# osmocom/osmo-trx

Measured on AMD Instinct MI355X. Metric: Mbursts/s detect+demod (156.25 sym, 4 SPS), higher is better.
Workload: dtype f32

## Files before the change

osmo_trx_amd/csrc/trx_kernel_nb.hip:

```cpp
#include "trx_k4_common.h"
#include "trx_nb_asm.inc"

#define NB_D_LEN    160
#define NB_CZ_LEN   (TRX_CZ_PAD + TRX_CORR_NARROW + TRX_CZ_PAD)
#define NB_SLICE    (K4_XS + NB_D_LEN + NB_CZ_LEN)
#define NB_COMP_ROWS (TRX_DELAY_FILTS + 1)
#define NB_TABLES_FLOATS (TRX_SINCV_LDS + 16 * WAVE + NB_COMP_ROWS * 36 + 16 + 8 * 8 + 5 * WAVE + 5 * WAVE + 2 * 8 * 16)
#define NB_TABLES_BYTES (NB_TABLES_FLOATS * 4)
#define NB_WPB 16
#define NB_POOL_RING 64
#define NB_POOL_UNSET (-1)
#define NB_POOL_END (-2)
#define NB_NO_BURST 0xffffffffu
#define NB_LDS_TAIL (16 + 4 * NB_POOL_RING)
#define NB_LDS_BYTES (NB_TABLES_BYTES + NB_WPB * NB_SLICE * 8 + NB_LDS_TAIL)
#define NB_MAX_TOA 32



typedef float v3f __attribute__((ext_vector_type(3)));
typedef int v4i __attribute__((ext_vector_type(4)));

template <typename T>
__device__ __forceinline__ unsigned lds_addr(const T *p)
{
	return (unsigned)(uintptr_t)(const __attribute__((address_space(3))) T *)p;
}

__global__ void __launch_bounds__(NB_WPB * WAVE)
nb_pull4_kernel(const uint32_t *__restrict__ iq, const trxhip_burst_params *__restrict__ params,
		trxhip_burst_result *__restrict__ results, float *__restrict__ soft, const trx_tables *__restrict__ tab,
		unsigned n_bursts, float thresh, float full_scale, unsigned *__restrict__ pool_ctr, unsigned *__restrict__ redo,
		float gk5, float gk6, float gk7, float gk8)
{
	static_assert(NB_TABLES_BYTES % 16 == 0 && (NB_SLICE * 8) % 16 == 0 && (K4_XS * 8) % 16 == 0 && (NB_D_LEN * 8) % 16 == 0, "16-byte LDS accesses");
	static_assert(NB_LDS_BYTES <= 160 * 1024, "LDS");
	static_assert(NB_ASM_GDEC_OFF == (TRX_SINCV_LDS + 16 * WAVE + NB_COMP_ROWS * 36) * 4, "tools/gen_nb_asm.py: LDS offset of the decimator taps");
	static_assert(NB_ASM_LSEQ_OFF == (NB_TABLES_FLOATS - 2 * 8 * 16) * 4, "tools/gen_nb_asm.py: LDS offset of the training-sequence taps");
	constexpr int NLD = 10;
	extern __shared__ __attribute__((aligned(16))) char smem[];
	const int lane0 = threadIdx.x & (WAVE - 1);
	const int wave = uni((int)(threadIdx.x >> 6));

	float *const sincv = reinterpret_cast<float *>(smem);
	float *const wa4f = sincv + TRX_SINCV_LDS;
	const float4 *const wa4 = reinterpret_cast<const float4 *>(wa4f);
	float *const comp = wa4f + 16 * WAVE;
	float *const gdec = comp + NB_COMP_ROWS * 36;
	float *const lhdr = gdec + 16;
	int *const pkcl = reinterpret_cast<int *>(lhdr + 8 * 8);
	int *const lcn = pkcl + 5 * WAVE;
	c32 *const lseq = reinterpret_cast<c32 *>(lcn + 5 * WAVE);
	c32 *const wbase = reinterpret_cast<c32 *>(smem + NB_TABLES_BYTES) + (size_t)wave * NB_SLICE;
	int *const wg_next = reinterpret_cast<int *>(reinterpret_cast<c32 *>(smem + NB_TABLES_BYTES) + (size_t)NB_WPB * NB_SLICE);
	int *const pool_g = wg_next + 4;
	c32 *const P = wbase;
	c32 *const D = wbase + K4_XS;
	c32 *const cz = D + NB_D_LEN + TRX_CZ_PAD;

	for (int i = threadIdx.x; i < TRX_SINCV_LDS; i += blockDim.x)
		sincv[i] = (i < TRX_SINCV_LEN) ? tab->sincv[i] : 0.0f;
	for (int i = threadIdx.x; i < 16 * WAVE; i += blockDim.x) {
		const int l = i & (WAVE - 1), u = i >> 6;
		const PeakConst pcl = peak_const(l);
		const int q = (u < 8) ? pcl.loA + 512 * (7 - u) : pcl.hiA + 512 * (u - 8);
		wa4f[((u >> 2) * WAVE + l) * 4 + (u & 3)] = (q < TRX_SINCV_LEN) ? tab->sincv[q] : 0.0f;
	}
	for (int i = threadIdx.x; i < NB_COMP_ROWS * 36; i += blockDim.x) {
		const int f = i / 36, j = i % 36;
		comp[i] = (j >= TRX_FUSED_SH) ? tab->comp_filt[f][j - TRX_FUSED_SH] : 0.0f;
	}
	if (threadIdx.x < 16)
		gdec[threadIdx.x] = tab->dec_taps[threadIdx.x];
	if (threadIdx.x < 128)
		lseq[threadIdx.x] = make_float2(tab->seq[TRX_SEQ_TSC0 + (threadIdx.x >> 4)].taps[threadIdx.x & 15].re,
						tab->seq[TRX_SEQ_TSC0 + (threadIdx.x >> 4)].taps[threadIdx.x & 15].im);
	if (threadIdx.x < 64)
		lhdr[threadIdx.x] = reinterpret_cast<const float *>(&tab->seq[TRX_SEQ_TSC0 + (threadIdx.x >> 3)].gain)[threadIdx.x & 7];
	if (threadIdx.x < WAVE) {
		const PeakConst pc0 = peak_const(threadIdx.x);
		pkcl[0 * WAVE + threadIdx.x] = pc0.flA;
		pkcl[1 * WAVE + threadIdx.x] = pc0.loA;
		pkcl[2 * WAVE + threadIdx.x] = pc0.hiA;
		pkcl[3 * WAVE + threadIdx.x] = pc0.offB;
		pkcl[4 * WAVE + threadIdx.x] = pc0.ratio_off;
		lcn[0 * WAVE + threadIdx.x] = pc0.ratio_off * 8;
		lcn[1 * WAVE + threadIdx.x] = (pc0.flA - 8) * 8;
		lcn[2 * WAVE + threadIdx.x] = pc0.offB;
		const int l = threadIdx.x, e = (-l) & 3;
		const bool sp = l >= 52 && l < 60;
		lcn[3 * WAVE + l] = 8 * (sp ? (l < 56 ? e : e - 2) : (l < 48 ? 4 + 3 * l : 148));
		lcn[4 * WAVE + l] = sp ? (e + (l >= 56 ? 4 : 0)) * K4_NTP * 4 : -1;
	}
	for (int i = lane0; i < NB_SLICE; i += WAVE)
		wbase[i] = make_float2(0.0f, 0.0f);
	if (threadIdx.x == 0) {
		wg_next[0] = NB_WPB;
		wg_next[1] = 0;
	}
	if (threadIdx.x < NB_POOL_RING)
		pool_g[threadIdx.x] = NB_POOL_UNSET;
	__syncthreads();

	const float fs_db = 6.02059991f * __log2f(full_scale);
	const float thr2 = thresh * thresh;
	const float gc0 = thr2 * 1.0001e-5f;
	int t5pk = 0;
	bool t5_ok = true;
	for (int t = 0; t < 8; t++) {
		const int v = (int)(lhdr[8 * t + 5] * 512.0f);
		t5_ok = t5_ok && v >= -8 && v <= 7 && (float)v == lhdr[8 * t + 5] * 512.0f;
		t5pk |= (v & 15) << (4 * t);
	}
	t5pk = uni(t5pk);
	const unsigned long long e8_addr = reinterpret_cast<unsigned long long>(&tab->edge8[0][0][0]);
	const unsigned n_wg = gridDim.x;
	const unsigned n_groups = (n_bursts + 15u) >> 4;
	const bool pooled = pool_ctr != nullptr;
	const unsigned n_static_groups = pooled ? ((n_groups - (n_groups >> 3)) / n_wg) * n_wg : n_groups;
	const unsigned n_pool_groups = n_groups - n_static_groups;
	const unsigned gq = n_static_groups / n_wg, gr = n_static_groups % n_wg;
	const unsigned my_groups = gq + (blockIdx.x < gr ? 1u : 0u);
	const unsigned base16 = (blockIdx.x * gq + (blockIdx.x < gr ? blockIdx.x : gr)) << 4;
	unsigned items = my_groups << 4;
	if (base16 + items > n_bursts)
		items = (base16 < n_bursts) ? n_bursts - base16 : 0u;
	auto burst_of = [&](unsigned jj) -> unsigned {
		if (jj < items)
			return base16 + jj;
		if (!pooled)
			return NB_NO_BURST;
		const unsigned k = (jj - items) >> 4;
		volatile int *slot = pool_g + (k & (NB_POOL_RING - 1));
		int g;
		while ((g = *slot) == NB_POOL_UNSET)
			__builtin_amdgcn_s_sleep(2);
		g = uni(g);
		if (g < 0)
			return NB_NO_BURST;
		const unsigned bb = ((n_static_groups + (unsigned)g) << 4) + (jj & 15u);
		return bb < n_bursts ? bb : NB_NO_BURST;
	};
	auto pool_draw = [&](unsigned jj, bool ended, int lane) {
		const unsigned k = (jj + 16u - items) >> 4;
		int g = NB_POOL_END;
		if (!ended) {
			unsigned p = 0;
			if (lane == 0)
				p = __hip_atomic_fetch_add(pool_ctr, 1u, __ATOMIC_RELAXED, __HIP_MEMORY_SCOPE_AGENT);
			p = (unsigned)uni((int)p);
			g = (p < n_pool_groups) ? (int)p : NB_POOL_END;
		}
		if (lane == 0) {
			pool_g[(k + NB_POOL_RING / 2) & (NB_POOL_RING - 1)] = NB_POOL_UNSET;
			pool_g[k & (NB_POOL_RING - 1)] = g;
		}
	};

	uint32_t pre_i[NLD];
	uint32_t pre_prm = 0u;
	auto prefetch = [&](unsigned bb, int lane) {
		pre_prm = reinterpret_cast<const uint32_t *>(params)[2 * (size_t)bb];
		const uint32_t *src = iq + (size_t)bb * 625;
		const unsigned ul = (unsigned)lane & 63u;
#pragma unroll
		for (int r = 0; r < NLD - 1; r++)
			pre_i[r] = __builtin_nontemporal_load(src + (unsigned)(r * WAVE) + ul);
		pre_i[NLD - 1] = __builtin_nontemporal_load(src + (unsigned)((NLD - 1) * WAVE) + min(ul, 48u));
	};
	const unsigned b_first = burst_of((unsigned)wave);
	if (b_first != NB_NO_BURST)
		prefetch(b_first, lane0);

	v3f o = { 0.0f, 0.0f, 0.0f };
	int recw = 0;
	bool pend_any = false;
	bool pend_rec = false;
	unsigned pend_b = 0;
	bool left_any = false;
	int q_xr = 0, q_xi = 0, q_es = 0, q_toa = 0, q_s = 0, q_fl = 0, q_b = 0;
	int q_n = 0;
	auto flush_records = [&](const int lane) {
		if (lane < q_n) {
			const float *const h = lhdr + 8 * (q_fl & 0xff);
			const float xr = __int_as_float(q_xr), xi = __int_as_float(q_xi);
			const float a0 = xr * h[2], a1 = xr * h[3], a2 = xi * h[3], a3 = xi * h[2];
			const float amp_re = a0 - a2, amp_im = a1 + a3;
			const float toa = (float)q_toa * 0.001953125f;
			const float energy = __int_as_float(q_es) * 0.0125f;
			const float rssi = fs_db - 3.01029996f * __log2f(energy);
			const float p2 = xi * xi + xr * xr;
			const float C = p2 * h[7];
			const float S = __int_as_float(q_s);
			const float ci = 3.0103f * __log2f(C * __builtin_amdgcn_rcpf(S - C));
			const v4i r0 = { 1, __float_as_int(toa), __float_as_int(amp_re), __float_as_int(amp_im) };
			const v4i r1 = { __float_as_int(ci), __float_as_int(energy), __float_as_int(rssi), q_fl };
			asm volatile("global_store_dwordx4 %0, %1, off\n\t"
				     "global_store_dwordx4 %0, %2, off offset:16\n\t"
				     "s_nop 1"
				     :: "v"(results + (unsigned)q_b), "v"(r0), "v"(r1) : "memory");
		}
		q_n = 0;
	};

	auto demod_general = [&](const int nk, const c32 ampv, const int lane) -> bool {
		constexpr int L = 625, nwrite = 148;
		c32 *const dec = D;
		const trx_tables *tabc = tab;
		asm volatile("" : "+s"(tabc));
		const int w = nk >> 7, fr = nk & 127;
		const int fidx = (fr >= 2) ? (fr >> 1) : TRX_DELAY_FILTS;
		const float ian = __builtin_amdgcn_rcpf(norm2(ampv));
		const c32 scale = make_float2(ampv.x * ian, -ampv.y * ian);
		const int n_lo = w > 0 ? w : 0;
		const int n_hi = (L - 1 + w < 623) ? L - 1 + w : 623;
		const int i_full_lo = cdiv4(n_lo + 15), i_full_hi = fdiv4(n_hi);
		const int i0l = cdiv4(n_lo), i0h = i_full_hi + 1;
		const bool need_lo = (n_hi >= n_lo) && (i0l < i_full_lo) && (i0l < nwrite);
		const bool need_hi = (n_hi >= n_lo) && (i0h <= fdiv4(n_hi + 15)) && (i0h < nwrite);
		const bool lo_tab = need_lo && (n_hi >= 4 * (i_full_lo - 1));
		float ct0 = 0.0f, ct1 = 0.0f, ct2 = 0.0f;
		const int le = lane >> 4, lt = lane & 15;
		const int li = i0l + le;
		const int lt0 = n_lo + 15 - 4 * li;
		const bool lact = lt0 >= 1;
		if (lo_tab) {
			const float *row = &tabc->edge_lo[fidx][(lact ? lt0 : 1) - 1][lt];
			ct0 = row[0];
			ct1 = row[16];
			ct2 = (lt < 4) ? row[32] : 0.0f;
		}
		const bool hi_tab = need_hi && (w <= -2) && (n_lo <= 4 * i0h - 15);
		if ((need_lo && !lo_tab) || (need_hi && !hi_tab))
			return false;
		float ch0 = 0.0f, ch1 = 0.0f, ch2 = 0.0f;
		const int hi_i = i0h + le;
		const int htm = n_hi + 15 - 4 * hi_i;
		const bool hact = htm >= 0;
		if (hi_tab) {
			const float *row = &tabc->edge_hi[fidx][hact ? htm : 0][lt];
			ch0 = row[0];
			ch1 = row[16];
			ch2 = (lt < 4) ? row[32] : 0.0f;
		}
		{
			const int c_full = -24 - w;
			const int i_min = cdiv4(-36 - c_full), i_max = fdiv4(L + 1 - c_full);
			int ic = 3 * lane;
			if (ic < i_min) ic = i_min;
			if (ic > i_max - 2) ic = i_max - 2;
			v2f acc[3];
			asm volatile(NB_ASM_FIRG
				     : [a0] "=&v"(acc[0]), [a1] "=&v"(acc[1]), [a2] "=&v"(acc[2])
				     : [nk] "s"(nk), [pb] "s"(lds_addr(P)), [cb] "s"(lds_addr(comp) + 4u * (K4_U0 + TRX_FUSED_SH)), [kic] "v"(8 * ic)
				     : NB_ASM_CLOBBERS);
			if (n_lo == 0 && lo_tab && i_full_hi >= nwrite - 1) {
				if (lane < 52) {
#pragma unroll
					for (int j = 0; j < 3; j++)
						dec[3 * lane + j] = cmul(make_float2(acc[j].x, acc[j].y), scale);
				}
			} else {
#pragma unroll
				for (int j = 0; j < 3; j++) {
					const int i = 3 * lane + j;
					const bool full = (i >= i_full_lo) && (i <= i_full_hi);
					const c32 d = full ? cmul(make_float2(acc[j].x, acc[j].y), scale) : make_float2(0.0f, 0.0f);
					if (i < 156)
						dec[i] = d;
				}
			}
		}
		if (lo_tab) {
			const int s0 = 4 * li - 24 - w + lt;
			const c32 *pp = P + ((s0 & 3) * PH_A + PH_M0 + (s0 >> 2));
			const c32 x0 = lds_c32(pp), x1 = lds_c32(pp + 4), x2 = lds_c32(pp + 8);
			float ar = x0.x * ct0, ai = x0.y * ct0;
			ar = fmaf(x1.x, ct1, ar); ai = fmaf(x1.y, ct1, ai);
			ar = fmaf(x2.x, ct2, ar); ai = fmaf(x2.y, ct2, ai);
			const float sr = row_sum(ar), si = row_sum(ai);
			if (lt == 0 && lact)
				dec[li] = cmul(make_float2(sr, si), scale);
		}
		if (hi_tab) {
			const int s0 = 4 * hi_i - 24 - w + lt;
			const c32 *pp = P + ((s0 & 3) * PH_A + PH_M0 + (s0 >> 2));
			const c32 x0 = lds_c32(pp), x1 = lds_c32(pp + 4), x2 = lds_c32(pp + 8);
			float ar = x0.x * ch0, ai = x0.y * ch0;
			ar = fmaf(x1.x, ch1, ar); ai = fmaf(x1.y, ch1, ai);
			ar = fmaf(x2.x, ch2, ar); ai = fmaf(x2.y, ch2, ai);
			const float sr = row_sum(ar), si = row_sum(ai);
			if (lt == 0 && hact && hi_i < 156)
				dec[hi_i] = cmul(make_float2(sr, si), scale);
		}
		wave_sync();
		auto pick = [&](int i) {
			const float d = reinterpret_cast<const float *>(dec + i)[i & 1];
			return __builtin_amdgcn_fmed3f(fmaf((i & 2) ? -0.5f : 0.5f, d, 0.5f), 0.0f, 1.0f);
		};
		const int i0 = (lane < 48) ? 4 + 3 * lane : ((-lane) & 3);
		o.x = pick(i0);
		o.y = pick(lane < 48 ? i0 + 1 : 0);
		o.z = pick(lane < 48 ? i0 + 2 : 0);
		wave_sync();
		return true;
	};

	DIAG_DECL;
	unsigned j_next = 0, b_next = NB_NO_BURST;
	for (unsigned b = b_first; b != NB_NO_BURST; b = b_next) {
		int lane;
		asm volatile("v_mbcnt_lo_u32_b32 %0, -1, 0\n\tv_mbcnt_hi_u32_b32 %0, -1, %0" : "=v"(lane));
		const int ticket = claim_issue(wg_next);
		const unsigned prm0 = (unsigned)uni((int)pre_prm);
		const unsigned max_toa = prm0 >> 16;
		const int tsc = (prm0 >> 8) & 0xff;
		bool leave = ((prm0 & 0xf8ffu) != (unsigned)TRXHIP_TSC) || (max_toa > NB_MAX_TOA) || !t5_ok;

		c32 *const pload = P + (lane & 3) * PH_A + PH_M0 + (lane >> 2);
		float amax = 0.0f, epart = 0.0f;
#ifdef TRX_DIAG
		DIAG_MARK(12);
		asm volatile("s_waitcnt vmcnt(0)" ::: "memory");
		DIAG_MARK(13);
#endif
		if (!leave) {
#pragma unroll
			for (int r = 0; r < NLD; r++) {
				const int i = r * WAVE + lane;
				if (r < NLD - 1 || i < 625) {
					const c32 v = make_float2((float)(int16_t)(pre_i[r] & 0xffffu), (float)(int16_t)(pre_i[r] >> 16));
					pload[16 * r] = v;
					asm("v_max3_f32 %0, %0, |%1|, |%2|" : "+v"(amax) : "v"(v.x), "v"(v.y));
					if (r < 5)
						epart = fmaf(v.x, v.x, fmaf(v.y, v.y, epart));
				}
			}
		} else {
#pragma unroll
			for (int r = 0; r < NLD; r++)
				asm volatile("" :: "v"(pre_i[r]));
		}
		DIAG_MARK(14);
		if (pend_any) {
			float *const so = soft + (size_t)pend_b * 148;
			int *const rp = reinterpret_cast<int *>(results + pend_b);
			const float oe = o.x;
			asm volatile("s_bfm_b64 exec, 48, 0\n\t"
				     "global_store_dwordx3 %0, %1, %2 offset:16\n\t"
				     "s_bfm_b64 exec, 4, 52\n\t"
				     "global_store_dword %3, %4, %2\n\t"
				     "s_mov_b64 exec, %8\n\t"
				     "global_store_dword %5, %6, %7\n\t"
				     "s_mov_b64 exec, -1\n\t"
				     "s_nop 0"
				     :: "v"(lane * 12), "v"(o), "s"(so), "v"(((-lane) & 3) * 4), "v"(oe), "v"(lane * 4), "v"(recw), "s"(rp),
				        "s"(pend_rec ? 0xffull : 0ull)
				     : "memory");
		}
		pend_any = false;
		DIAG_MARK(16);
		j_next = (unsigned)(leave ? claim_take(ticket) : claim_take_behind<5>(ticket));
		b_next = burst_of(j_next);
		if (pooled && (j_next & 15u) == 0u && j_next + 16u >= items)
			pool_draw(j_next, b_next == NB_NO_BURST && j_next >= items, lane);
		DIAG_MARK(17);
		if (b_next != NB_NO_BURST)
			prefetch(b_next, lane);
		DIAG_MARK(15);

		int clip = 0;
		if (!leave) {
			clip = __ballot(amax > TRX_CLIP_THRESH) != 0ull;

			const int len = 16 + (int)max_toa;
			__builtin_assume(len >= 16 && len <= 16 + NB_MAX_TOA);
			const unsigned vd_addr = lds_addr(D) + 8u * (unsigned)lane, vcz_addr = lds_addr(cz) + 8u * (unsigned)lane;
			unsigned long long bad;
			asm volatile(NB_ASM_DEC
				     : [bad] "=s"(bad)
				     : [pd] "v"(lds_addr(P + PH_M0 + 52) + 8u * (unsigned)lane), [vd] "v"(vd_addr), [zero] "v"(0), [nact] "s"(15 + len)
				     : NB_ASM_CLOBBERS);
			DIAG_MARK(2);
			{
				float v;
				asm volatile(NB_ASM_CORR
					     : [nrm] "=&v"(v)
					     : [vd] "v"(vd_addr), [vcz] "v"(vcz_addr), [len] "s"(len), [tsc] "s"(tsc), [bad] "s"(bad)
					     : NB_ASM_CLOBBERS);
				DIAG_MARK(3);
				int m_bits, es_bits, bidx;
				int kr, ka, kb, kic, ktp;
				asm volatile(NB_ASM_AMAX("ds_read_b32 %[kr], %[l4] offset:%c[lc]", "ds_read_b32 %[ka], %[l4] offset:%c[lc]+256",
							 "ds_read_b32 %[kb], %[l4] offset:%c[lc]+512", "ds_read_b32 %[kic], %[l4] offset:%c[lc]+768",
							 "ds_read_b32 %[ktp], %[l4] offset:%c[lc]+1024", "s_nop 0", "s_nop 0", "s_nop 0")
					     "s_waitcnt lgkmcnt(0)"
					     : [m] "=s"(m_bits), [es] "=s"(es_bits), [bidx] "=s"(bidx), [kr] "=&v"(kr), [ka] "=&v"(ka), [kb] "=&v"(kb),
					       [kic] "=&v"(kic), [ktp] "=&v"(ktp)
					     : [nrm] "v"(v), [ep] "v"(epart), [l4] "v"(4 * lane),
					       [lc] "n"((TRX_SINCV_LDS + 16 * WAVE + NB_COMP_ROWS * 36 + 16 + 64 + 5 * WAVE) * 4)
					     : NB_ASM_CLOBBERS);
				DIAG_MARK(4);
				int hit = 0;
				int toa512 = 0;
				if (m_bits != 0) {
					int st, e512;
					float km;
					asm volatile(NB_ASM_DETA
						     : [st] "=&s"(st), [e] "=&s"(e512), [km] "=&v"(km)
						     : [bidx] "s"(bidx), [len] "s"(len), [czb] "s"(lds_addr(cz)), [kr] "v"(kr), [ka] "v"(ka), [l16] "v"(16 * lane),
						       [k5] "s"(gk5), [k6] "s"(gk6), [k7] "s"(gk7), [k8] "s"(gk8), [c0] "v"(gc0)
						     : NB_ASM_CLOBBERS);
					DIAG_MARK(5);
					int xr_bits = 0, xi_bits = 0;
					if (st == 1) {
						asm volatile(NB_ASM_DETB
							     : [st] "=&s"(st), [toa] "=&s"(toa512), [xr] "=&s"(xr_bits), [xi] "=&s"(xi_bits)
							     : [e] "s"(e512), [kb] "v"(kb), [czb] "s"(lds_addr(cz)), [km] "v"(km)
							     : NB_ASM_CLOBBERS);
						DIAG_MARK(6);
					}
					if (st == 3) {
						if (lane == 0)
							atomicAdd(&g_trx_fast_stats[0], 1ull);
						PeakConst pkc;
						pkc.flA = pkcl[0 * WAVE + lane]; pkc.loA = pkcl[1 * WAVE + lane]; pkc.hiA = pkcl[2 * WAVE + lane];
						pkc.offB = pkcl[3 * WAVE + lane]; pkc.ratio_off = pkcl[4 * WAVE + lane];
						c32 xcorr;
						peak_detect_spec(cz, bidx, sincv, pkc, lane, &toa512, &xcorr, wa4);
						toa512 = uni(toa512);
						xr_bits = uni(__float_as_int(xcorr.x));
						xi_bits = uni(__float_as_int(xcorr.y));
						st = 1;
					}
					if (st == 2) {
						leave = true;
						if (lane == 0) atomicAdd(&g_trx_fast_stats[2], 1ull);
					}
					if (st == 1) {
						hit = 1;
						int ok, s_bits;
						float d0, d1, d2;
						const int t5 = (t5pk << (28 - 4 * tsc)) >> 28;
						asm volatile("s_setprio 0");
						asm volatile(NB_ASM_TAIL
							     : [ok] "=&s"(ok), [ssum] "=&s"(s_bits), [d0] "=&v"(d0), [d1] "=&v"(d1), [d2] "=&v"(d2)
							     : [toa] "s"(toa512), [xr] "s"(xr_bits), [xi] "s"(xi_bits), [t5] "s"(t5), [hdrb] "s"(lds_addr(lhdr) + 32u * (unsigned)tsc),
							       [e8lo] "s"((unsigned)e8_addr), [e8hi] "s"((unsigned)(e8_addr >> 32)), [l16] "v"(16 * lane),
							       [vd] "v"(vd_addr), [pb] "s"(lds_addr(P)), [cb] "s"(lds_addr(comp) + 4u * (K4_U0 + TRX_FUSED_SH)), [db] "s"(lds_addr(D)),
							       [kic] "v"(kic), [ktp] "v"(ktp)
							     : NB_ASM_CLOBBERS);
						DIAG_MARK(10);
						asm volatile("s_setprio 2");
						if (!ok) {
							if (lane == 0) atomicAdd(&g_trx_fast_stats[3], 1ull);
							const float *const h = lhdr + 8 * tsc;
							const float xr = __int_as_float(xr_bits), xi = __int_as_float(xi_bits);
							const float a0 = xr * h[2], a1 = xr * h[3], a2 = xi * h[3], a3 = xi * h[2];
							const c32 ampv = make_float2(unif(a0 - a2), unif(a1 + a3));
							if (!demod_general(t5 + 10 * 512 - toa512, ampv, lane))
								leave = true;
						}
						if (!leave) {
							asm("s_lshl_b64 exec, 1, %[n]\n\t"
						    "v_mov_b32_e32 %[qxr], %[xr]\n\t"
						    "v_mov_b32_e32 %[qxi], %[xi]\n\t"
						    "v_mov_b32_e32 %[qes], %[es]\n\t"
						    "v_mov_b32_e32 %[qtoa], %[toa]\n\t"
						    "v_mov_b32_e32 %[qs], %[ss]\n\t"
						    "v_mov_b32_e32 %[qfl], %[fl]\n\t"
						    "v_mov_b32_e32 %[qb], %[b]\n\t"
						    "s_mov_b64 exec, -1"
						    : [qxr] "+v"(q_xr), [qxi] "+v"(q_xi), [qes] "+v"(q_es), [qtoa] "+v"(q_toa), [qs] "+v"(q_s), [qfl] "+v"(q_fl),
						      [qb] "+v"(q_b)
						    : [n] "s"(uni(q_n)), [xr] "s"(xr_bits), [xi] "s"(xi_bits), [es] "s"(es_bits), [toa] "s"(toa512 - t5 - 10 * 512),
						      [ss] "s"(s_bits), [fl] "s"((int)((uint32_t)tsc | ((uint32_t)clip << 8) | (37u << 24))), [b] "s"((int)b));
						q_n++;
						}
						if (ok) {
							o.x = __builtin_amdgcn_fmed3f(fmaf(0.5f, d0, 0.5f), 0.0f, 1.0f);
							o.y = __builtin_amdgcn_fmed3f(fmaf(0.5f, d1, 0.5f), 0.0f, 1.0f);
							o.z = __builtin_amdgcn_fmed3f(fmaf(0.5f, d2, 0.5f), 0.0f, 1.0f);
						}
					}
				}
				if (!hit && !leave) {
					const float energy = __int_as_float(es_bits) * 0.0125f;
					const float rssi = fs_db - 3.01029996f * __log2f(energy);
					const uint32_t flags = ((uint32_t)clip << 8) | (1u << 16);
					int word = clip ? -TRXHIP_SIGERR_CLIP : 0;
					word = put_lane<1>(word, 0.0f);
					word = put_lane<2>(word, 0.0f);
					word = put_lane<3>(word, 0.0f);
					word = put_lane<4>(word, 0.0f);
					word = put_lane<5>(word, energy);
					word = put_lane<6>(word, rssi);
					word = write_lane<7>(word, (int)flags);
					recw = word;
					o = (v3f){ 0.0f, 0.0f, 0.0f };
				}
				pend_rec = !hit;
			}
		}
		if (leave) {
			if (lane == 0) {
				reinterpret_cast<uint8_t *>(redo + TRX_REDO_HDR)[b] = 1;
				if (!left_any)
					__hip_atomic_store(redo, 1u, __ATOMIC_RELAXED, __HIP_MEMORY_SCOPE_AGENT);
			}
			left_any = true;
			continue;
		}
		pend_b = b;
		pend_any = true;
		if (q_n == WAVE)
			flush_records(lane);
		DIAG_MARK(11);
	}
	if (pend_any) {
		int lane;
		asm volatile("v_mbcnt_lo_u32_b32 %0, -1, 0\n\tv_mbcnt_hi_u32_b32 %0, -1, %0" : "=v"(lane));
		float *const so = soft + (size_t)pend_b * 148;
		int *const rp = reinterpret_cast<int *>(results + pend_b);
		const float oe = o.x;
		asm volatile("s_bfm_b64 exec, 48, 0\n\t"
			     "global_store_dwordx3 %0, %1, %2 offset:16\n\t"
			     "s_bfm_b64 exec, 4, 52\n\t"
			     "global_store_dword %3, %4, %2\n\t"
			     "s_mov_b64 exec, %8\n\t"
			     "global_store_dword %5, %6, %7\n\t"
			     "s_mov_b64 exec, -1\n\t"
			     "s_nop 0"
			     :: "v"(lane * 12), "v"(o), "s"(so), "v"(((-lane) & 3) * 4), "v"(oe), "v"(lane * 4), "v"(recw), "s"(rp),
			        "s"(pend_rec ? 0xffull : 0ull)
			     : "memory");
	}
	{
		int lane;
		asm volatile("v_mbcnt_lo_u32_b32 %0, -1, 0\n\tv_mbcnt_hi_u32_b32 %0, -1, %0" : "=v"(lane));
		flush_records(lane);
	}
	DIAG_FLUSH();
	if (pooled) {
		__syncthreads();
		int tid0;
		asm volatile("v_mbcnt_lo_u32_b32 %0, -1, 0\n\tv_mbcnt_hi_u32_b32 %0, -1, %0" : "=v"(tid0));
		if (tid0 == 0 && atomicAdd(wg_next + 1, 1) == 0) {
			const unsigned d = __hip_atomic_fetch_add(pool_ctr + 1, 1u, __ATOMIC_ACQ_REL, __HIP_MEMORY_SCOPE_AGENT);
			if (d == gridDim.x - 1u) {
				__hip_atomic_store(pool_ctr, 0u, __ATOMIC_RELAXED, __HIP_MEMORY_SCOPE_AGENT);
				__hip_atomic_store(pool_ctr + 1, 0u, __ATOMIC_RELEASE, __HIP_MEMORY_SCOPE_AGENT);
			}
		}
	}
}
```

osmo_trx_amd/csrc/trx_nb_asm.inc:

```
#define NB_ASM_GDEC_OFF 29968
#define NB_ASM_LSEQ_OFF 32848
#define NB_ASM_CLOBBERS "v64", "v65", "v66", "v67", "v68", "v69", "v70", "v71", "v72", "v73", "v74", "v75", "v76", "v77", "v78", "v79", "v80", "v81", "v82", "v83", "v84", "v85", "v86", "v87", "v88", "v89", "v90", "v91", "v92", "v93", "v94", "v95", "v96", "v97", "v98", "v99", "v100", "v101", "v102", "v103", "v104", "v105", "v106", "v107", "v108", "v109", "v110", "v111", "v112", "v113", "v114", "v115", "v116", "v117", "v118", "v119", "v120", "v121", "v122", "v123", "v124", "v125", "v126", "v127", "s87", "s88", "s89", "s90", "s91", "s92", "s93", "s94", "s95", "s96", "s97", "s98", "s99", "vcc", "scc", "memory"
#define NB_ASM_DEC \
	"s_bfm_b64 exec, %[nact], 0\n\t" \
	"ds_read_b128 v[120:123], %[zero] offset:29968\n\t" \
	"ds_read_b128 v[124:127], %[zero] offset:29984\n\t" \
	"ds_read_b64 v[88:89], %[pd] offset:1440\n\t" \
	"ds_read_b64 v[90:91], %[pd] offset:2880\n\t" \
	"ds_read_b64 v[92:93], %[pd] offset:4320\n\t" \
	"ds_read_b64 v[94:95], %[pd] offset:8\n\t" \
	"ds_read_b64 v[96:97], %[pd] offset:1448\n\t" \
	"ds_read_b64 v[98:99], %[pd] offset:2888\n\t" \
	"ds_read_b64 v[100:101], %[pd] offset:4328\n\t" \
	"ds_read_b64 v[102:103], %[pd] offset:16\n\t" \
	"ds_read_b64 v[104:105], %[pd] offset:1456\n\t" \
	"ds_read_b64 v[106:107], %[pd] offset:2896\n\t" \
	"ds_read_b64 v[108:109], %[pd] offset:4336\n\t" \
	"ds_read_b64 v[110:111], %[pd] offset:24\n\t" \
	"ds_read_b64 v[112:113], %[pd] offset:1464\n\t" \
	"ds_read_b64 v[114:115], %[pd] offset:2904\n\t" \
	"ds_read_b64 v[116:117], %[pd] offset:4344\n\t" \
	"ds_read_b64 v[118:119], %[pd] offset:32\n\t" \
	"s_waitcnt lgkmcnt(12)\n\t" \
	"v_pk_mul_f32 v[88:89], v[88:89], v[120:121] op_sel:[0,0] op_sel_hi:[1,0]\n\t" \
	"v_pk_mul_f32 v[90:91], v[90:91], v[120:121] op_sel:[0,1] op_sel_hi:[1,1]\n\t" \
	"v_pk_mul_f32 v[92:93], v[92:93], v[122:123] op_sel:[0,0] op_sel_hi:[1,0]\n\t" \
	"v_pk_add_f32 v[88:89], v[88:89], v[90:91]\n\t" \
	"v_pk_mul_f32 v[94:95], v[94:95], v[122:123] op_sel:[0,1] op_sel_hi:[1,1]\n\t" \
	"v_pk_add_f32 v[88:89], v[88:89], v[92:93]\n\t" \
	"s_waitcnt lgkmcnt(8)\n\t" \
	"v_pk_mul_f32 v[96:97], v[96:97], v[124:125] op_sel:[0,0] op_sel_hi:[1,0]\n\t" \
	"v_pk_add_f32 v[88:89], v[88:89], v[94:95]\n\t" \
	"v_pk_mul_f32 v[98:99], v[98:99], v[124:125] op_sel:[0,1] op_sel_hi:[1,1]\n\t" \
	"v_pk_add_f32 v[88:89], v[88:89], v[96:97]\n\t" \
	"v_pk_mul_f32 v[100:101], v[100:101], v[126:127] op_sel:[0,0] op_sel_hi:[1,0]\n\t" \
	"v_pk_add_f32 v[88:89], v[88:89], v[98:99]\n\t" \
	"v_pk_mul_f32 v[102:103], v[102:103], v[126:127] op_sel:[0,1] op_sel_hi:[1,1]\n\t" \
	"v_pk_add_f32 v[88:89], v[88:89], v[100:101]\n\t" \
	"s_waitcnt lgkmcnt(4)\n\t" \
	"v_pk_mul_f32 v[104:105], v[104:105], v[126:127] op_sel:[0,1] op_sel_hi:[1,1]\n\t" \
	"v_pk_add_f32 v[88:89], v[88:89], v[102:103]\n\t" \
	"v_pk_mul_f32 v[106:107], v[106:107], v[126:127] op_sel:[0,0] op_sel_hi:[1,0]\n\t" \
	"v_pk_add_f32 v[88:89], v[88:89], v[104:105]\n\t" \
	"v_pk_mul_f32 v[108:109], v[108:109], v[124:125] op_sel:[0,1] op_sel_hi:[1,1]\n\t" \
	"v_pk_add_f32 v[88:89], v[88:89], v[106:107]\n\t" \
	"v_pk_mul_f32 v[110:111], v[110:111], v[124:125] op_sel:[0,0] op_sel_hi:[1,0]\n\t" \
	"v_pk_add_f32 v[88:89], v[88:89], v[108:109]\n\t" \
	"s_waitcnt lgkmcnt(0)\n\t" \
	"v_pk_mul_f32 v[112:113], v[112:113], v[122:123] op_sel:[0,1] op_sel_hi:[1,1]\n\t" \
	"v_pk_add_f32 v[88:89], v[88:89], v[110:111]\n\t" \
	"v_pk_mul_f32 v[114:115], v[114:115], v[122:123] op_sel:[0,0] op_sel_hi:[1,0]\n\t" \
	"v_pk_add_f32 v[88:89], v[88:89], v[112:113]\n\t" \
	"v_pk_mul_f32 v[116:117], v[116:117], v[120:121] op_sel:[0,1] op_sel_hi:[1,1]\n\t" \
	"v_pk_add_f32 v[88:89], v[88:89], v[114:115]\n\t" \
	"v_pk_mul_f32 v[118:119], v[118:119], v[120:121] op_sel:[0,0] op_sel_hi:[1,0]\n\t" \
	"v_pk_add_f32 v[88:89], v[88:89], v[116:117]\n\t" \
	"s_nop 0\n\t" \
	"v_pk_add_f32 v[88:89], v[88:89], v[118:119]\n\t" \
	"ds_write_b64 %[vd], v[88:89]\n\t" \
	"v_min_f32_e64 v90, |v88|, |v89|\n\t" \
	"v_max_f32_e64 v91, |v88|, |v89|\n\t" \
	"v_ldexp_f32 v90, v90, 17\n\t" \
	"v_cmp_lt_f32_e32 vcc, v90, v91\n\t" \
	"s_mov_b64 exec, -1\n\t" \
	"s_mov_b64 %[bad], vcc\n\t" \
	"s_waitcnt lgkmcnt(0)\n\t"
#define NB_ASM_CORR \
	"v_mov_b64_e32 v[120:121], 0\n\t" \
	"s_bfm_b64 exec, %[len], 0\n\t" \
	"ds_read_b64 v[88:89], %[vd] offset:0\n\t" \
	"ds_read_b64 v[90:91], %[vd] offset:8\n\t" \
	"ds_read_b64 v[92:93], %[vd] offset:16\n\t" \
	"ds_read_b64 v[94:95], %[vd] offset:24\n\t" \
	"ds_read_b64 v[96:97], %[vd] offset:32\n\t" \
	"ds_read_b64 v[98:99], %[vd] offset:40\n\t" \
	"ds_read_b64 v[100:101], %[vd] offset:48\n\t" \
	"ds_read_b64 v[102:103], %[vd] offset:56\n\t" \
	"ds_read_b64 v[104:105], %[vd] offset:64\n\t" \
	"ds_read_b64 v[106:107], %[vd] offset:72\n\t" \
	"ds_read_b64 v[108:109], %[vd] offset:80\n\t" \
	"ds_read_b64 v[110:111], %[vd] offset:88\n\t" \
	"ds_read_b64 v[112:113], %[vd] offset:96\n\t" \
	"ds_read_b64 v[114:115], %[vd] offset:104\n\t" \
	"ds_read_b64 v[116:117], %[vd] offset:112\n\t" \
	"ds_read_b64 v[118:119], %[vd] offset:120\n\t" \
	"s_cmp_lg_u64 %[bad], 0\n\t" \
	"s_cbranch_scc1 .Lnb_corr_mul\n\t" \
	"s_getpc_b64 s[88:89]\n\t" \
	".Lnb_corr_pc:\n\t" \
	"s_mul_i32 s90, %[tsc], .Lnb_corr_v1-.Lnb_corr_v0\n\t" \
	"s_add_u32 s88, s88, s90\n\t" \
	"s_addc_u32 s89, s89, 0\n\t" \
	"s_add_u32 s88, s88, .Lnb_corr_v0-.Lnb_corr_pc\n\t" \
	"s_addc_u32 s89, s89, 0\n\t" \
	"s_setpc_b64 s[88:89]\n\t" \
	".Lnb_corr_v0:\n\t" \
	"s_waitcnt lgkmcnt(15)\n\t" \
	"v_pk_add_f32 v[120:121], v[120:121], v[88:89] neg_lo:[0,1] neg_hi:[0,1]\n\t" \
	"s_waitcnt lgkmcnt(14)\n\t" \
	"v_pk_add_f32 v[120:121], v[120:121], v[90:91] op_sel:[0,1] op_sel_hi:[1,0] neg_lo:[0,0] neg_hi:[0,1]\n\t" \
	"s_waitcnt lgkmcnt(13)\n\t" \
	"v_pk_add_f32 v[120:121], v[120:121], v[92:93]\n\t" \
	"s_waitcnt lgkmcnt(12)\n\t" \
	"v_pk_add_f32 v[120:121], v[120:121], v[94:95] op_sel:[0,1] op_sel_hi:[1,0] neg_lo:[0,0] neg_hi:[0,1]\n\t" \
	"s_waitcnt lgkmcnt(11)\n\t" \
	"v_pk_add_f32 v[120:121], v[120:121], v[96:97] neg_lo:[0,1] neg_hi:[0,1]\n\t" \
	"s_waitcnt lgkmcnt(10)\n\t" \
	"v_pk_add_f32 v[120:121], v[120:121], v[98:99] op_sel:[0,1] op_sel_hi:[1,0] neg_lo:[0,0] neg_hi:[0,1]\n\t" \
	"s_waitcnt lgkmcnt(9)\n\t" \
	"v_pk_add_f32 v[120:121], v[120:121], v[100:101] neg_lo:[0,1] neg_hi:[0,1]\n\t" \
	"s_waitcnt lgkmcnt(8)\n\t" \
	"v_pk_add_f32 v[120:121], v[120:121], v[102:103] op_sel:[0,1] op_sel_hi:[1,0] neg_lo:[0,1] neg_hi:[0,0]\n\t" \
	"s_waitcnt lgkmcnt(7)\n\t" \
	"v_pk_add_f32 v[120:121], v[120:121], v[104:105]\n\t" \
	"s_waitcnt lgkmcnt(6)\n\t" \
	"v_pk_add_f32 v[120:121], v[120:121], v[106:107] op_sel:[0,1] op_sel_hi:[1,0] neg_lo:[0,1] neg_hi:[0,0]\n\t" \
	"s_waitcnt lgkmcnt(5)\n\t" \
	"v_pk_add_f32 v[120:121], v[120:121], v[108:109] neg_lo:[0,1] neg_hi:[0,1]\n\t" \
	"s_waitcnt lgkmcnt(4)\n\t" \
	"v_pk_add_f32 v[120:121], v[120:121], v[110:111] op_sel:[0,1] op_sel_hi:[1,0] neg_lo:[0,1] neg_hi:[0,0]\n\t" \
	"s_waitcnt lgkmcnt(3)\n\t" \
	"v_pk_add_f32 v[120:121], v[120:121], v[112:113]\n\t" \
	"s_waitcnt lgkmcnt(2)\n\t" \
	"v_pk_add_f32 v[120:121], v[120:121], v[114:115] op_sel:[0,1] op_sel_hi:[1,0] neg_lo:[0,1] neg_hi:[0,0]\n\t" \
	"s_waitcnt lgkmcnt(1)\n\t" \
	"v_pk_add_f32 v[120:121], v[120:121], v[116:117] neg_lo:[0,1] neg_hi:[0,1]\n\t" \
	"s_waitcnt lgkmcnt(0)\n\t" \
	"v_pk_add_f32 v[120:121], v[120:121], v[118:119] op_sel:[0,1] op_sel_hi:[1,0] neg_lo:[0,1] neg_hi:[0,0]\n\t" \
	"s_branch .Lnb_corr_join\n\t" \
	".Lnb_corr_v1:\n\t" \
	"s_waitcnt lgkmcnt(15)\n\t" \
	"v_pk_add_f32 v[120:121], v[120:121], v[88:89] neg_lo:[0,1] neg_hi:[0,1]\n\t" \
	"s_waitcnt lgkmcnt(14)\n\t" \
	"v_pk_add_f32 v[120:121], v[120:121], v[90:91] op_sel:[0,1] op_sel_hi:[1,0] neg_lo:[0,0] neg_hi:[0,1]\n\t" \
	"s_waitcnt lgkmcnt(13)\n\t" \
	"v_pk_add_f32 v[120:121], v[120:121], v[92:93]\n\t" \
	"s_waitcnt lgkmcnt(12)\n\t" \
	"v_pk_add_f32 v[120:121], v[120:121], v[94:95] op_sel:[0,1] op_sel_hi:[1,0] neg_lo:[0,0] neg_hi:[0,1]\n\t" \
	"s_waitcnt lgkmcnt(11)\n\t" \
	"v_pk_add_f32 v[120:121], v[120:121], v[96:97] neg_lo:[0,1] neg_hi:[0,1]\n\t" \
	"s_waitcnt lgkmcnt(10)\n\t" \
	"v_pk_add_f32 v[120:121], v[120:121], v[98:99] op_sel:[0,1] op_sel_hi:[1,0] neg_lo:[0,0] neg_hi:[0,1]\n\t" \
	"s_waitcnt lgkmcnt(9)\n\t" \
	"v_pk_add_f32 v[120:121], v[120:121], v[100:101]\n\t" \
	"s_waitcnt lgkmcnt(8)\n\t" \
	"v_pk_add_f32 v[120:121], v[120:121], v[102:103] op_sel:[0,1] op_sel_hi:[1,0] neg_lo:[0,0] neg_hi:[0,1]\n\t" \
	"s_waitcnt lgkmcnt(7)\n\t" \
	"v_pk_add_f32 v[120:121], v[120:121], v[104:105] neg_lo:[0,1] neg_hi:[0,1]\n\t" \
	"s_waitcnt lgkmcnt(6)\n\t" \
	"v_pk_add_f32 v[120:121], v[120:121], v[106:107] op_sel:[0,1] op_sel_hi:[1,0] neg_lo:[0,1] neg_hi:[0,0]\n\t" \
	"s_waitcnt lgkmcnt(5)\n\t" \
	"v_pk_add_f32 v[120:121], v[120:121], v[108:109] neg_lo:[0,1] neg_hi:[0,1]\n\t" \
	"s_waitcnt lgkmcnt(4)\n\t" \
	"v_pk_add_f32 v[120:121], v[120:121], v[110:111] op_sel:[0,1] op_sel_hi:[1,0] neg_lo:[0,1] neg_hi:[0,0]\n\t" \
	"s_waitcnt lgkmcnt(3)\n\t" \
	"v_pk_add_f32 v[120:121], v[120:121], v[112:113]\n\t" \
	"s_waitcnt lgkmcnt(2)\n\t" \
	"v_pk_add_f32 v[120:121], v[120:121], v[114:115] op_sel:[0,1] op_sel_hi:[1,0] neg_lo:[0,1] neg_hi:[0,0]\n\t" \
	"s_waitcnt lgkmcnt(1)\n\t" \
	"v_pk_add_f32 v[120:121], v[120:121], v[116:117] neg_lo:[0,1] neg_hi:[0,1]\n\t" \
	"s_waitcnt lgkmcnt(0)\n\t" \
	"v_pk_add_f32 v[120:121], v[120:121], v[118:119] op_sel:[0,1] op_sel_hi:[1,0] neg_lo:[0,0] neg_hi:[0,1]\n\t" \
	"s_branch .Lnb_corr_join\n\t" \
	".Lnb_corr_v2:\n\t" \
	"s_waitcnt lgkmcnt(15)\n\t" \
	"v_pk_add_f32 v[120:121], v[120:121], v[88:89]\n\t" \
	"s_waitcnt lgkmcnt(14)\n\t" \
	"v_pk_add_f32 v[120:121], v[120:121], v[90:91] op_sel:[0,1] op_sel_hi:[1,0] neg_lo:[0,1] neg_hi:[0,0]\n\t" \
	"s_waitcnt lgkmcnt(13)\n\t" \
	"v_pk_add_f32 v[120:121], v[120:121], v[92:93]\n\t" \
	"s_waitcnt lgkmcnt(12)\n\t" \
	"v_pk_add_f32 v[120:121], v[120:121], v[94:95] op_sel:[0,1] op_sel_hi:[1,0] neg_lo:[0,0] neg_hi:[0,1]\n\t" \
	"s_waitcnt lgkmcnt(11)\n\t" \
	"v_pk_add_f32 v[120:121], v[120:121], v[96:97]\n\t" \
	"s_waitcnt lgkmcnt(10)\n\t" \
	"v_pk_add_f32 v[120:121], v[120:121], v[98:99] op_sel:[0,1] op_sel_hi:[1,0] neg_lo:[0,1] neg_hi:[0,0]\n\t" \
	"s_waitcnt lgkmcnt(9)\n\t" \
	"v_pk_add_f32 v[120:121], v[120:121], v[100:101]\n\t" \
	"s_waitcnt lgkmcnt(8)\n\t" \
	"v_pk_add_f32 v[120:121], v[120:121], v[102:103] op_sel:[0,1] op_sel_hi:[1,0] neg_lo:[0,0] neg_hi:[0,1]\n\t" \
	"s_waitcnt lgkmcnt(7)\n\t" \
	"v_pk_add_f32 v[120:121], v[120:121], v[104:105]\n\t" \
	"s_waitcnt lgkmcnt(6)\n\t" \
	"v_pk_add_f32 v[120:121], v[120:121], v[106:107] op_sel:[0,1] op_sel_hi:[1,0] neg_lo:[0,1] neg_hi:[0,0]\n\t" \
	"s_waitcnt lgkmcnt(5)\n\t" \
	"v_pk_add_f32 v[120:121], v[120:121], v[108:109] neg_lo:[0,1] neg_hi:[0,1]\n\t" \
	"s_waitcnt lgkmcnt(4)\n\t" \
	"v_pk_add_f32 v[120:121], v[120:121], v[110:111] op_sel:[0,1] op_sel_hi:[1,0] neg_lo:[0,1] neg_hi:[0,0]\n\t" \
	"s_waitcnt lgkmcnt(3)\n\t" \
	"v_pk_add_f32 v[120:121], v[120:121], v[112:113] neg_lo:[0,1] neg_hi:[0,1]\n\t" \
	"s_waitcnt lgkmcnt(2)\n\t" \
	"v_pk_add_f32 v[120:121], v[120:121], v[114:115] op_sel:[0,1] op_sel_hi:[1,0] neg_lo:[0,0] neg_hi:[0,1]\n\t" \
	"s_waitcnt lgkmcnt(1)\n\t" \
	"v_pk_add_f32 v[120:121], v[120:121], v[116:117] neg_lo:[0,1] neg_hi:[0,1]\n\t" \
	"s_waitcnt lgkmcnt(0)\n\t" \
	"v_pk_add_f32 v[120:121], v[120:121], v[118:119] op_sel:[0,1] op_sel_hi:[1,0] neg_lo:[0,1] neg_hi:[0,0]\n\t" \
	"s_branch .Lnb_corr_join\n\t" \
	".Lnb_corr_v3:\n\t" \
	"s_waitcnt lgkmcnt(15)\n\t" \
	"v_pk_add_f32 v[120:121], v[120:121], v[88:89] neg_lo:[0,1] neg_hi:[0,1]\n\t" \
	"s_waitcnt lgkmcnt(14)\n\t" \
	"v_pk_add_f32 v[120:121], v[120:121], v[90:91] op_sel:[0,1] op_sel_hi:[1,0] neg_lo:[0,1] neg_hi:[0,0]\n\t" \
	"s_waitcnt lgkmcnt(13)\n\t" \
	"v_pk_add_f32 v[120:121], v[120:121], v[92:93]\n\t" \
	"s_waitcnt lgkmcnt(12)\n\t" \
	"v_pk_add_f32 v[120:121], v[120:121], v[94:95] op_sel:[0,1] op_sel_hi:[1,0] neg_lo:[0,0] neg_hi:[0,1]\n\t" \
	"s_waitcnt lgkmcnt(11)\n\t" \
	"v_pk_add_f32 v[120:121], v[120:121], v[96:97]\n\t" \
	"s_waitcnt lgkmcnt(10)\n\t" \
	"v_pk_add_f32 v[120:121], v[120:121], v[98:99] op_sel:[0,1] op_sel_hi:[1,0] neg_lo:[0,1] neg_hi:[0,0]\n\t" \
	"s_waitcnt lgkmcnt(9)\n\t" \
	"v_pk_add_f32 v[120:121], v[120:121], v[100:101]\n\t" \
	"s_waitcnt lgkmcnt(8)\n\t" \
	"v_pk_add_f32 v[120:121], v[120:121], v[102:103] op_sel:[0,1] op_sel_hi:[1,0] neg_lo:[0,1] neg_hi:[0,0]\n\t" \
	"s_waitcnt lgkmcnt(7)\n\t" \
	"v_pk_add_f32 v[120:121], v[120:121], v[104:105] neg_lo:[0,1] neg_hi:[0,1]\n\t" \
	"s_waitcnt lgkmcnt(6)\n\t" \
	"v_pk_add_f32 v[120:121], v[120:121], v[106:107] op_sel:[0,1] op_sel_hi:[1,0] neg_lo:[0,0] neg_hi:[0,1]\n\t" \
	"s_waitcnt lgkmcnt(5)\n\t" \
	"v_pk_add_f32 v[120:121], v[120:121], v[108:109] neg_lo:[0,1] neg_hi:[0,1]\n\t" \
	"s_waitcnt lgkmcnt(4)\n\t" \
	"v_pk_add_f32 v[120:121], v[120:121], v[110:111] op_sel:[0,1] op_sel_hi:[1,0] neg_lo:[0,1] neg_hi:[0,0]\n\t" \
	"s_waitcnt lgkmcnt(3)\n\t" \
	"v_pk_add_f32 v[120:121], v[120:121], v[112:113] neg_lo:[0,1] neg_hi:[0,1]\n\t" \
	"s_waitcnt lgkmcnt(2)\n\t" \
	"v_pk_add_f32 v[120:121], v[120:121], v[114:115] op_sel:[0,1] op_sel_hi:[1,0] neg_lo:[0,0] neg_hi:[0,1]\n\t" \
	"s_waitcnt lgkmcnt(1)\n\t" \
	"v_pk_add_f32 v[120:121], v[120:121], v[116:117] neg_lo:[0,1] neg_hi:[0,1]\n\t" \
	"s_waitcnt lgkmcnt(0)\n\t" \
	"v_pk_add_f32 v[120:121], v[120:121], v[118:119] op_sel:[0,1] op_sel_hi:[1,0] neg_lo:[0,1] neg_hi:[0,0]\n\t" \
	"s_branch .Lnb_corr_join\n\t" \
	".Lnb_corr_v4:\n\t" \
	"s_waitcnt lgkmcnt(15)\n\t" \
	"v_pk_add_f32 v[120:121], v[120:121], v[88:89]\n\t" \
	"s_waitcnt lgkmcnt(14)\n\t" \
	"v_pk_add_f32 v[120:121], v[120:121], v[90:91] op_sel:[0,1] op_sel_hi:[1,0] neg_lo:[0,1] neg_hi:[0,0]\n\t" \
	"s_waitcnt lgkmcnt(13)\n\t" \
	"v_pk_add_f32 v[120:121], v[120:121], v[92:93] neg_lo:[0,1] neg_hi:[0,1]\n\t" \
	"s_waitcnt lgkmcnt(12)\n\t" \
	"v_pk_add_f32 v[120:121], v[120:121], v[94:95] op_sel:[0,1] op_sel_hi:[1,0] neg_lo:[0,0] neg_hi:[0,1]\n\t" \
	"s_waitcnt lgkmcnt(11)\n\t" \
	"v_pk_add_f32 v[120:121], v[120:121], v[96:97] neg_lo:[0,1] neg_hi:[0,1]\n\t" \
	"s_waitcnt lgkmcnt(10)\n\t" \
	"v_pk_add_f32 v[120:121], v[120:121], v[98:99] op_sel:[0,1] op_sel_hi:[1,0] neg_lo:[0,1] neg_hi:[0,0]\n\t" \
	"s_waitcnt lgkmcnt(9)\n\t" \
	"v_pk_add_f32 v[120:121], v[120:121], v[100:101] neg_lo:[0,1] neg_hi:[0,1]\n\t" \
	"s_waitcnt lgkmcnt(8)\n\t" \
	"v_pk_add_f32 v[120:121], v[120:121], v[102:103] op_sel:[0,1] op_sel_hi:[1,0] neg_lo:[0,1] neg_hi:[0,0]\n\t" \
	"s_waitcnt lgkmcnt(7)\n\t" \
	"v_pk_add_f32 v[120:121], v[120:121], v[104:105] neg_lo:[0,1] neg_hi:[0,1]\n\t" \
	"s_waitcnt lgkmcnt(6)\n\t" \
	"v_pk_add_f32 v[120:121], v[120:121], v[106:107] op_sel:[0,1] op_sel_hi:[1,0] neg_lo:[0,0] neg_hi:[0,1]\n\t" \
	"s_waitcnt lgkmcnt(5)\n\t" \
	"v_pk_add_f32 v[120:121], v[120:121], v[108:109] neg_lo:[0,1] neg_hi:[0,1]\n\t" \
	"s_waitcnt lgkmcnt(4)\n\t" \
	"v_pk_add_f32 v[120:121], v[120:121], v[110:111] op_sel:[0,1] op_sel_hi:[1,0] neg_lo:[0,1] neg_hi:[0,0]\n\t" \
	"s_waitcnt lgkmcnt(3)\n\t" \
	"v_pk_add_f32 v[120:121], v[120:121], v[112:113]\n\t" \
	"s_waitcnt lgkmcnt(2)\n\t" \
	"v_pk_add_f32 v[120:121], v[120:121], v[114:115] op_sel:[0,1] op_sel_hi:[1,0] neg_lo:[0,0] neg_hi:[0,1]\n\t" \
	"s_waitcnt lgkmcnt(1)\n\t" \
	"v_pk_add_f32 v[120:121], v[120:121], v[116:117]\n\t" \
	"s_waitcnt lgkmcnt(0)\n\t" \
	"v_pk_add_f32 v[120:121], v[120:121], v[118:119] op_sel:[0,1] op_sel_hi:[1,0] neg_lo:[0,0] neg_hi:[0,1]\n\t" \
	"s_branch .Lnb_corr_join\n\t" \
	".Lnb_corr_v5:\n\t" \
	"s_waitcnt lgkmcnt(15)\n\t" \
	"v_pk_add_f32 v[120:121], v[120:121], v[88:89] neg_lo:[0,1] neg_hi:[0,1]\n\t" \
	"s_waitcnt lgkmcnt(14)\n\t" \
	"v_pk_add_f32 v[120:121], v[120:121], v[90:91] op_sel:[0,1] op_sel_hi:[1,0] neg_lo:[0,1] neg_hi:[0,0]\n\t" \
	"s_waitcnt lgkmcnt(13)\n\t" \
	"v_pk_add_f32 v[120:121], v[120:121], v[92:93] neg_lo:[0,1] neg_hi:[0,1]\n\t" \
	"s_waitcnt lgkmcnt(12)\n\t" \
	"v_pk_add_f32 v[120:121], v[120:121], v[94:95] op_sel:[0,1] op_sel_hi:[1,0] neg_lo:[0,0] neg_hi:[0,1]\n\t" \
	"s_waitcnt lgkmcnt(11)\n\t" \
	"v_pk_add_f32 v[120:121], v[120:121], v[96:97]\n\t" \
	"s_waitcnt lgkmcnt(10)\n\t" \
	"v_pk_add_f32 v[120:121], v[120:121], v[98:99] op_sel:[0,1] op_sel_hi:[1,0] neg_lo:[0,1] neg_hi:[0,0]\n\t" \
	"s_waitcnt lgkmcnt(9)\n\t" \
	"v_pk_add_f32 v[120:121], v[120:121], v[100:101]\n\t" \
	"s_waitcnt lgkmcnt(8)\n\t" \
	"v_pk_add_f32 v[120:121], v[120:121], v[102:103] op_sel:[0,1] op_sel_hi:[1,0] neg_lo:[0,1] neg_hi:[0,0]\n\t" \
	"s_waitcnt lgkmcnt(7)\n\t" \
	"v_pk_add_f32 v[120:121], v[120:121], v[104:105]\n\t" \
	"s_waitcnt lgkmcnt(6)\n\t" \
	"v_pk_add_f32 v[120:121], v[120:121], v[106:107] op_sel:[0,1] op_sel_hi:[1,0] neg_lo:[0,0] neg_hi:[0,1]\n\t" \
	"s_waitcnt lgkmcnt(5)\n\t" \
	"v_pk_add_f32 v[120:121], v[120:121], v[108:109] neg_lo:[0,1] neg_hi:[0,1]\n\t" \
	"s_waitcnt lgkmcnt(4)\n\t" \
	"v_pk_add_f32 v[120:121], v[120:121], v[110:111] op_sel:[0,1] op_sel_hi:[1,0] neg_lo:[0,1] neg_hi:[0,0]\n\t" \
	"s_waitcnt lgkmcnt(3)\n\t" \
	"v_pk_add_f32 v[120:121], v[120:121], v[112:113] neg_lo:[0,1] neg_hi:[0,1]\n\t" \
	"s_waitcnt lgkmcnt(2)\n\t" \
	"v_pk_add_f32 v[120:121], v[120:121], v[114:115] op_sel:[0,1] op_sel_hi:[1,0] neg_lo:[0,0] neg_hi:[0,1]\n\t" \
	"s_waitcnt lgkmcnt(1)\n\t" \
	"v_pk_add_f32 v[120:121], v[120:121], v[116:117] neg_lo:[0,1] neg_hi:[0,1]\n\t" \
	"s_waitcnt lgkmcnt(0)\n\t" \
	"v_pk_add_f32 v[120:121], v[120:121], v[118:119] op_sel:[0,1] op_sel_hi:[1,0] neg_lo:[0,0] neg_hi:[0,1]\n\t" \
	"s_branch .Lnb_corr_join\n\t" \
	".Lnb_corr_v6:\n\t" \
	"s_waitcnt lgkmcnt(15)\n\t" \
	"v_pk_add_f32 v[120:121], v[120:121], v[88:89] neg_lo:[0,1] neg_hi:[0,1]\n\t" \
	"s_waitcnt lgkmcnt(14)\n\t" \
	"v_pk_add_f32 v[120:121], v[120:121], v[90:91] op_sel:[0,1] op_sel_hi:[1,0] neg_lo:[0,1] neg_hi:[0,0]\n\t" \
	"s_waitcnt lgkmcnt(13)\n\t" \
	"v_pk_add_f32 v[120:121], v[120:121], v[92:93]\n\t" \
	"s_waitcnt lgkmcnt(12)\n\t" \
	"v_pk_add_f32 v[120:121], v[120:121], v[94:95] op_sel:[0,1] op_sel_hi:[1,0] neg_lo:[0,0] neg_hi:[0,1]\n\t" \
	"s_waitcnt lgkmcnt(11)\n\t" \
	"v_pk_add_f32 v[120:121], v[120:121], v[96:97] neg_lo:[0,1] neg_hi:[0,1]\n\t" \
	"s_waitcnt lgkmcnt(10)\n\t" \
	"v_pk_add_f32 v[120:121], v[120:121], v[98:99] op_sel:[0,1] op_sel_hi:[1,0] neg_lo:[0,0] neg_hi:[0,1]\n\t" \
	"s_waitcnt lgkmcnt(9)\n\t" \
	"v_pk_add_f32 v[120:121], v[120:121], v[100:101]\n\t" \
	"s_waitcnt lgkmcnt(8)\n\t" \
	"v_pk_add_f32 v[120:121], v[120:121], v[102:103] op_sel:[0,1] op_sel_hi:[1,0] neg_lo:[0,0] neg_hi:[0,1]\n\t" \
	"s_waitcnt lgkmcnt(7)\n\t" \
	"v_pk_add_f32 v[120:121], v[120:121], v[104:105]\n\t" \
	"s_waitcnt lgkmcnt(6)\n\t" \
	"v_pk_add_f32 v[120:121], v[120:121], v[106:107] op_sel:[0,1] op_sel_hi:[1,0] neg_lo:[0,0] neg_hi:[0,1]\n\t" \
	"s_waitcnt lgkmcnt(5)\n\t" \
	"v_pk_add_f32 v[120:121], v[120:121], v[108:109] neg_lo:[0,1] neg_hi:[0,1]\n\t" \
	"s_waitcnt lgkmcnt(4)\n\t" \
	"v_pk_add_f32 v[120:121], v[120:121], v[110:111] op_sel:[0,1] op_sel_hi:[1,0] neg_lo:[0,0] neg_hi:[0,1]\n\t" \
	"s_waitcnt lgkmcnt(3)\n\t" \
	"v_pk_add_f32 v[120:121], v[120:121], v[112:113]\n\t" \
	"s_waitcnt lgkmcnt(2)\n\t" \
	"v_pk_add_f32 v[120:121], v[120:121], v[114:115] op_sel:[0,1] op_sel_hi:[1,0] neg_lo:[0,1] neg_hi:[0,0]\n\t" \
	"s_waitcnt lgkmcnt(1)\n\t" \
	"v_pk_add_f32 v[120:121], v[120:121], v[116:117] neg_lo:[0,1] neg_hi:[0,1]\n\t" \
	"s_waitcnt lgkmcnt(0)\n\t" \
	"v_pk_add_f32 v[120:121], v[120:121], v[118:119] op_sel:[0,1] op_sel_hi:[1,0] neg_lo:[0,1] neg_hi:[0,0]\n\t" \
	"s_branch .Lnb_corr_join\n\t" \
	".Lnb_corr_v7:\n\t" \
	"s_waitcnt lgkmcnt(15)\n\t" \
	"v_pk_add_f32 v[120:121], v[120:121], v[88:89] neg_lo:[0,1] neg_hi:[0,1]\n\t" \
	"s_waitcnt lgkmcnt(14)\n\t" \
	"v_pk_add_f32 v[120:121], v[120:121], v[90:91] op_sel:[0,1] op_sel_hi:[1,0] neg_lo:[0,1] neg_hi:[0,0]\n\t" \
	"s_waitcnt lgkmcnt(13)\n\t" \
	"v_pk_add_f32 v[120:121], v[120:121], v[92:93]\n\t" \
	"s_waitcnt lgkmcnt(12)\n\t" \
	"v_pk_add_f32 v[120:121], v[120:121], v[94:95] op_sel:[0,1] op_sel_hi:[1,0] neg_lo:[0,1] neg_hi:[0,0]\n\t" \
	"s_waitcnt lgkmcnt(11)\n\t" \
	"v_pk_add_f32 v[120:121], v[120:121], v[96:97]\n\t" \
	"s_waitcnt lgkmcnt(10)\n\t" \
	"v_pk_add_f32 v[120:121], v[120:121], v[98:99] op_sel:[0,1] op_sel_hi:[1,0] neg_lo:[0,0] neg_hi:[0,1]\n\t" \
	"s_waitcnt lgkmcnt(9)\n\t" \
	"v_pk_add_f32 v[120:121], v[120:121], v[100:101]\n\t" \
	"s_waitcnt lgkmcnt(8)\n\t" \
	"v_pk_add_f32 v[120:121], v[120:121], v[102:103] op_sel:[0,1] op_sel_hi:[1,0] neg_lo:[0,1] neg_hi:[0,0]\n\t" \
	"s_waitcnt lgkmcnt(7)\n\t" \
	"v_pk_add_f32 v[120:121], v[120:121], v[104:105]\n\t" \
	"s_waitcnt lgkmcnt(6)\n\t" \
	"v_pk_add_f32 v[120:121], v[120:121], v[106:107] op_sel:[0,1] op_sel_hi:[1,0] neg_lo:[0,1] neg_hi:[0,0]\n\t" \
	"s_waitcnt lgkmcnt(5)\n\t" \
	"v_pk_add_f32 v[120:121], v[120:121], v[108:109] neg_lo:[0,1] neg_hi:[0,1]\n\t" \
	"s_waitcnt lgkmcnt(4)\n\t" \
	"v_pk_add_f32 v[120:121], v[120:121], v[110:111] op_sel:[0,1] op_sel_hi:[1,0] neg_lo:[0,0] neg_hi:[0,1]\n\t" \
	"s_waitcnt lgkmcnt(3)\n\t" \
	"v_pk_add_f32 v[120:121], v[120:121], v[112:113] neg_lo:[0,1] neg_hi:[0,1]\n\t" \
	"s_waitcnt lgkmcnt(2)\n\t" \
	"v_pk_add_f32 v[120:121], v[120:121], v[114:115] op_sel:[0,1] op_sel_hi:[1,0] neg_lo:[0,1] neg_hi:[0,0]\n\t" \
	"s_waitcnt lgkmcnt(1)\n\t" \
	"v_pk_add_f32 v[120:121], v[120:121], v[116:117] neg_lo:[0,1] neg_hi:[0,1]\n\t" \
	"s_waitcnt lgkmcnt(0)\n\t" \
	"v_pk_add_f32 v[120:121], v[120:121], v[118:119] op_sel:[0,1] op_sel_hi:[1,0] neg_lo:[0,0] neg_hi:[0,1]\n\t" \
	"s_branch .Lnb_corr_join\n\t" \
	".Lnb_corr_join:\n\t" \
	"s_add_u32 s90, %[len], 12\n\t" \
	"s_bfm_b64 exec, s90, 0\n\t" \
	"ds_write_b64 %[vcz], v[120:121]\n\t" \
	"s_mov_b64 exec, -1\n\t" \
	"v_pk_mul_f32 v[122:123], v[120:121], v[120:121]\n\t" \
	"s_waitcnt lgkmcnt(0)\n\t" \
	"v_add_f32_e32 %[nrm], v123, v122\n\t" \
	"s_branch .Lnb_corr_end\n\t" \
	".Lnb_corr_mul:\n\t" \
	"s_lshl_b32 s90, %[tsc], 7\n\t" \
	"v_mov_b32_e32 v64, s90\n\t" \
	"ds_read_b128 v[66:69], v64 offset:32848\n\t" \
	"ds_read_b128 v[70:73], v64 offset:32864\n\t" \
	"ds_read_b128 v[74:77], v64 offset:32880\n\t" \
	"ds_read_b128 v[78:81], v64 offset:32896\n\t" \
	"s_waitcnt lgkmcnt(0)\n\t" \
	"v_pk_mul_f32 v[82:83], v[88:89], v[66:67] op_sel:[0,0] op_sel_hi:[0,1]\n\t" \
	"v_pk_mul_f32 v[84:85], v[88:89], v[66:67] op_sel:[1,1] op_sel_hi:[1,0]\n\t" \
	"s_nop 0\n\t" \
	"v_pk_add_f32 v[86:87], v[82:83], v[84:85] neg_lo:[0,1] neg_hi:[0,0]\n\t" \
	"s_nop 0\n\t" \
	"v_pk_add_f32 v[120:121], v[120:121], v[86:87]\n\t" \
	"v_pk_mul_f32 v[82:83], v[90:91], v[68:69] op_sel:[0,0] op_sel_hi:[0,1]\n\t" \
	"v_pk_mul_f32 v[84:85], v[90:91], v[68:69] op_sel:[1,1] op_sel_hi:[1,0]\n\t" \
	"s_nop 0\n\t" \
	"v_pk_add_f32 v[86:87], v[82:83], v[84:85] neg_lo:[0,1] neg_hi:[0,0]\n\t" \
	"s_nop 0\n\t" \
	"v_pk_add_f32 v[120:121], v[120:121], v[86:87]\n\t" \
	"v_pk_mul_f32 v[82:83], v[92:93], v[70:71] op_sel:[0,0] op_sel_hi:[0,1]\n\t" \
	"v_pk_mul_f32 v[84:85], v[92:93], v[70:71] op_sel:[1,1] op_sel_hi:[1,0]\n\t" \
	"s_nop 0\n\t" \
	"v_pk_add_f32 v[86:87], v[82:83], v[84:85] neg_lo:[0,1] neg_hi:[0,0]\n\t" \
	"s_nop 0\n\t" \
	"v_pk_add_f32 v[120:121], v[120:121], v[86:87]\n\t" \
	"v_pk_mul_f32 v[82:83], v[94:95], v[72:73] op_sel:[0,0] op_sel_hi:[0,1]\n\t" \
	"v_pk_mul_f32 v[84:85], v[94:95], v[72:73] op_sel:[1,1] op_sel_hi:[1,0]\n\t" \
	"s_nop 0\n\t" \
	"v_pk_add_f32 v[86:87], v[82:83], v[84:85] neg_lo:[0,1] neg_hi:[0,0]\n\t" \
	"s_nop 0\n\t" \
	"v_pk_add_f32 v[120:121], v[120:121], v[86:87]\n\t" \
	"v_pk_mul_f32 v[82:83], v[96:97], v[74:75] op_sel:[0,0] op_sel_hi:[0,1]\n\t" \
	"v_pk_mul_f32 v[84:85], v[96:97], v[74:75] op_sel:[1,1] op_sel_hi:[1,0]\n\t" \
	"s_nop 0\n\t" \
	"v_pk_add_f32 v[86:87], v[82:83], v[84:85] neg_lo:[0,1] neg_hi:[0,0]\n\t" \
	"s_nop 0\n\t" \
	"v_pk_add_f32 v[120:121], v[120:121], v[86:87]\n\t" \
	"v_pk_mul_f32 v[82:83], v[98:99], v[76:77] op_sel:[0,0] op_sel_hi:[0,1]\n\t" \
	"v_pk_mul_f32 v[84:85], v[98:99], v[76:77] op_sel:[1,1] op_sel_hi:[1,0]\n\t" \
	"s_nop 0\n\t" \
	"v_pk_add_f32 v[86:87], v[82:83], v[84:85] neg_lo:[0,1] neg_hi:[0,0]\n\t" \
	"s_nop 0\n\t" \
	"v_pk_add_f32 v[120:121], v[120:121], v[86:87]\n\t" \
	"v_pk_mul_f32 v[82:83], v[100:101], v[78:79] op_sel:[0,0] op_sel_hi:[0,1]\n\t" \
	"v_pk_mul_f32 v[84:85], v[100:101], v[78:79] op_sel:[1,1] op_sel_hi:[1,0]\n\t" \
	"s_nop 0\n\t" \
	"v_pk_add_f32 v[86:87], v[82:83], v[84:85] neg_lo:[0,1] neg_hi:[0,0]\n\t" \
	"s_nop 0\n\t" \
	"v_pk_add_f32 v[120:121], v[120:121], v[86:87]\n\t" \
	"v_pk_mul_f32 v[82:83], v[102:103], v[80:81] op_sel:[0,0] op_sel_hi:[0,1]\n\t" \
	"v_pk_mul_f32 v[84:85], v[102:103], v[80:81] op_sel:[1,1] op_sel_hi:[1,0]\n\t" \
	"s_nop 0\n\t" \
	"v_pk_add_f32 v[86:87], v[82:83], v[84:85] neg_lo:[0,1] neg_hi:[0,0]\n\t" \
	"s_nop 0\n\t" \
	"v_pk_add_f32 v[120:121], v[120:121], v[86:87]\n\t" \
	"ds_read_b128 v[66:69], v64 offset:32912\n\t" \
	"ds_read_b128 v[70:73], v64 offset:32928\n\t" \
	"ds_read_b128 v[74:77], v64 offset:32944\n\t" \
	"ds_read_b128 v[78:81], v64 offset:32960\n\t" \
	"s_waitcnt lgkmcnt(0)\n\t" \
	"v_pk_mul_f32 v[82:83], v[104:105], v[66:67] op_sel:[0,0] op_sel_hi:[0,1]\n\t" \
	"v_pk_mul_f32 v[84:85], v[104:105], v[66:67] op_sel:[1,1] op_sel_hi:[1,0]\n\t" \
	"s_nop 0\n\t" \
	"v_pk_add_f32 v[86:87], v[82:83], v[84:85] neg_lo:[0,1] neg_hi:[0,0]\n\t" \
	"s_nop 0\n\t" \
	"v_pk_add_f32 v[120:121], v[120:121], v[86:87]\n\t" \
	"v_pk_mul_f32 v[82:83], v[106:107], v[68:69] op_sel:[0,0] op_sel_hi:[0,1]\n\t" \
	"v_pk_mul_f32 v[84:85], v[106:107], v[68:69] op_sel:[1,1] op_sel_hi:[1,0]\n\t" \
	"s_nop 0\n\t" \
	"v_pk_add_f32 v[86:87], v[82:83], v[84:85] neg_lo:[0,1] neg_hi:[0,0]\n\t" \
	"s_nop 0\n\t" \
	"v_pk_add_f32 v[120:121], v[120:121], v[86:87]\n\t" \
	"v_pk_mul_f32 v[82:83], v[108:109], v[70:71] op_sel:[0,0] op_sel_hi:[0,1]\n\t" \
	"v_pk_mul_f32 v[84:85], v[108:109], v[70:71] op_sel:[1,1] op_sel_hi:[1,0]\n\t" \
	"s_nop 0\n\t" \
	"v_pk_add_f32 v[86:87], v[82:83], v[84:85] neg_lo:[0,1] neg_hi:[0,0]\n\t" \
	"s_nop 0\n\t" \
	"v_pk_add_f32 v[120:121], v[120:121], v[86:87]\n\t" \
	"v_pk_mul_f32 v[82:83], v[110:111], v[72:73] op_sel:[0,0] op_sel_hi:[0,1]\n\t" \
	"v_pk_mul_f32 v[84:85], v[110:111], v[72:73] op_sel:[1,1] op_sel_hi:[1,0]\n\t" \
	"s_nop 0\n\t" \
	"v_pk_add_f32 v[86:87], v[82:83], v[84:85] neg_lo:[0,1] neg_hi:[0,0]\n\t" \
	"s_nop 0\n\t" \
	"v_pk_add_f32 v[120:121], v[120:121], v[86:87]\n\t" \
	"v_pk_mul_f32 v[82:83], v[112:113], v[74:75] op_sel:[0,0] op_sel_hi:[0,1]\n\t" \
	"v_pk_mul_f32 v[84:85], v[112:113], v[74:75] op_sel:[1,1] op_sel_hi:[1,0]\n\t" \
	"s_nop 0\n\t" \
	"v_pk_add_f32 v[86:87], v[82:83], v[84:85] neg_lo:[0,1] neg_hi:[0,0]\n\t" \
	"s_nop 0\n\t" \
	"v_pk_add_f32 v[120:121], v[120:121], v[86:87]\n\t" \
	"v_pk_mul_f32 v[82:83], v[114:115], v[76:77] op_sel:[0,0] op_sel_hi:[0,1]\n\t" \
	"v_pk_mul_f32 v[84:85], v[114:115], v[76:77] op_sel:[1,1] op_sel_hi:[1,0]\n\t" \
	"s_nop 0\n\t" \
	"v_pk_add_f32 v[86:87], v[82:83], v[84:85] neg_lo:[0,1] neg_hi:[0,0]\n\t" \
	"s_nop 0\n\t" \
	"v_pk_add_f32 v[120:121], v[120:121], v[86:87]\n\t" \
	"v_pk_mul_f32 v[82:83], v[116:117], v[78:79] op_sel:[0,0] op_sel_hi:[0,1]\n\t" \
	"v_pk_mul_f32 v[84:85], v[116:117], v[78:79] op_sel:[1,1] op_sel_hi:[1,0]\n\t" \
	"s_nop 0\n\t" \
	"v_pk_add_f32 v[86:87], v[82:83], v[84:85] neg_lo:[0,1] neg_hi:[0,0]\n\t" \
	"s_nop 0\n\t" \
	"v_pk_add_f32 v[120:121], v[120:121], v[86:87]\n\t" \
	"v_pk_mul_f32 v[82:83], v[118:119], v[80:81] op_sel:[0,0] op_sel_hi:[0,1]\n\t" \
	"v_pk_mul_f32 v[84:85], v[118:119], v[80:81] op_sel:[1,1] op_sel_hi:[1,0]\n\t" \
	"s_nop 0\n\t" \
	"v_pk_add_f32 v[86:87], v[82:83], v[84:85] neg_lo:[0,1] neg_hi:[0,0]\n\t" \
	"s_nop 0\n\t" \
	"v_pk_add_f32 v[120:121], v[120:121], v[86:87]\n\t" \
	"s_branch .Lnb_corr_join\n\t" \
	".Lnb_corr_end:\n\t"
#define NB_ASM_DETA \
	"s_mov_b32 %[st], 0\n\t" \
	"s_cmp_lt_i32 %[bidx], 3\n\t" \
	"s_cbranch_scc1 .Lnb_da_end\n\t" \
	"s_sub_u32 s88, %[len], 3\n\t" \
	"s_cmp_gt_i32 %[bidx], s88\n\t" \
	"s_cbranch_scc1 .Lnb_da_end\n\t" \
	"s_lshl3_add_u32 s89, %[bidx], %[czb]\n\t" \
	"s_add_u32 s90, %[len], -1\n\t" \
	"v_mov_b32_e32 v64, s89\n\t" \
	"v_add_u32_e32 v65, s89, %[kr]\n\t" \
	"s_lshl3_add_u32 s90, s90, %[czb]\n\t" \
	"v_add_u32_e32 v66, s89, %[ka]\n\t" \
	"ds_read_b64 v[68:69], v64\n\t" \
	"v_mov_b32_e32 v67, s90\n\t" \
	"v_mov_b64_e32 v[72:73], 0\n\t" \
	"s_bfm_b64 exec, 8, 0\n\t" \
	"ds_read_b64 v[70:71], v65\n\t" \
	"s_mov_b64 exec, 1\n\t" \
	"ds_write_b64 v67, v[72:73]\n\t" \
	"s_mov_b64 exec, -1\n\t" \
	"ds_read_b128 v[76:79], %[l16] offset:16512\n\t" \
	"ds_read_b128 v[80:83], %[l16] offset:17536\n\t" \
	"ds_read_b64 v[88:89], v66 offset:0\n\t" \
	"ds_read_b64 v[90:91], v66 offset:8\n\t" \
	"ds_read_b64 v[92:93], v66 offset:16\n\t" \
	"ds_read_b64 v[94:95], v66 offset:24\n\t" \
	"ds_read_b64 v[96:97], v66 offset:32\n\t" \
	"ds_read_b64 v[98:99], v66 offset:40\n\t" \
	"ds_read_b64 v[100:101], v66 offset:48\n\t" \
	"ds_read_b64 v[102:103], v66 offset:56\n\t" \
	"v_mov_b64_e32 v[84:85], 0\n\t" \
	"v_mov_b64_e32 v[86:87], 0\n\t" \
	"s_add_u32 s91, %[bidx], -1\n\t" \
	"s_sub_u32 s92, %[len], %[bidx]\n\t" \
	"s_min_u32 s91, s91, 4\n\t" \
	"s_waitcnt lgkmcnt(11)\n\t" \
	"v_pk_mul_f32 v[68:69], v[68:69], v[68:69]\n\t" \
	"s_add_u32 s92, s92, -2\n\t" \
	"v_add_f32_e32 v74, v69, v68\n\t" \
	"v_mul_f32_e32 %[km], 0x36c9539c, v74\n\t" \
	"s_bfm_b64 exec, 8, 0\n\t" \
	"v_pk_mul_f32 v[70:71], v[70:71], v[70:71]\n\t" \
	"s_min_u32 s92, s92, 4\n\t" \
	"v_add_f32_e32 v75, v71, v70\n\t" \
	"s_add_u32 s91, s91, s92\n\t" \
	"s_cmp_eq_u32 s91, 8\n\t" \
	"v_add_f32_dpp v75, v75, v75 quad_perm:[1,0,3,2] row_mask:0xf bank_mask:0xf\n\t" \
	"s_cselect_b32 s92, %[k8], %[k7]\n\t" \
	"s_cmp_eq_u32 s91, 6\n\t" \
	"v_add_f32_dpp v75, v75, v75 quad_perm:[2,3,0,1] row_mask:0xf bank_mask:0xf\n\t" \
	"s_cselect_b32 s93, %[k6], %[k5]\n\t" \
	"s_cmp_ge_u32 s91, 7\n\t" \
	"v_add_f32_dpp v75, v75, v75 row_half_mirror row_mask:0xf bank_mask:0xf\n\t" \
	"s_cselect_b32 s92, s92, s93\n\t" \
	"v_mul_f32_e32 v112, s92, v75\n\t" \
	"v_mul_f32_e32 v113, 0x3f7fff37, v112\n\t" \
	"v_fmamk_f32 v114, v112, 0x3f8000c9, %[c0]\n\t" \
	"v_cmp_lt_f32_e32 vcc, v74, v113\n\t" \
	"s_cbranch_vccnz .Lnb_da_wait_end\n\t" \
	"v_cmp_gt_f32_e32 vcc, v74, v114\n\t" \
	"s_mov_b32 %[st], 2\n\t" \
	"s_cbranch_vccz .Lnb_da_wait_end\n\t" \
	"s_mov_b64 exec, -1\n\t" \
	"ds_read_b128 v[104:107], %[l16] offset:18560\n\t" \
	"ds_read_b128 v[108:111], %[l16] offset:19584\n\t" \
	"ds_read_b64 v[112:113], v66 offset:64\n\t" \
	"ds_read_b64 v[114:115], v66 offset:72\n\t" \
	"ds_read_b64 v[116:117], v66 offset:80\n\t" \
	"ds_read_b64 v[118:119], v66 offset:88\n\t" \
	"ds_read_b64 v[120:121], v66 offset:96\n\t" \
	"ds_read_b64 v[122:123], v66 offset:104\n\t" \
	"ds_read_b64 v[124:125], v66 offset:112\n\t" \
	"ds_read_b64 v[126:127], v66 offset:120\n\t" \
	"s_waitcnt lgkmcnt(10)\n\t" \
	"v_pk_fma_f32 v[84:85], v[88:89], v[76:77], v[84:85] op_sel:[0,0,0] op_sel_hi:[1,0,1]\n\t" \
	"v_pk_fma_f32 v[86:87], v[90:91], v[76:77], v[86:87] op_sel:[0,1,0] op_sel_hi:[1,1,1]\n\t" \
	"v_pk_fma_f32 v[84:85], v[92:93], v[78:79], v[84:85] op_sel:[0,0,0] op_sel_hi:[1,0,1]\n\t" \
	"v_pk_fma_f32 v[86:87], v[94:95], v[78:79], v[86:87] op_sel:[0,1,0] op_sel_hi:[1,1,1]\n\t" \
	"v_pk_fma_f32 v[84:85], v[96:97], v[80:81], v[84:85] op_sel:[0,0,0] op_sel_hi:[1,0,1]\n\t" \
	"v_pk_fma_f32 v[86:87], v[98:99], v[80:81], v[86:87] op_sel:[0,1,0] op_sel_hi:[1,1,1]\n\t" \
	"v_pk_fma_f32 v[84:85], v[100:101], v[82:83], v[84:85] op_sel:[0,0,0] op_sel_hi:[1,0,1]\n\t" \
	"v_pk_fma_f32 v[86:87], v[102:103], v[82:83], v[86:87] op_sel:[0,1,0] op_sel_hi:[1,1,1]\n\t" \
	"s_waitcnt lgkmcnt(0)\n\t" \
	"v_pk_fma_f32 v[84:85], v[112:113], v[104:105], v[84:85] op_sel:[0,0,0] op_sel_hi:[1,0,1]\n\t" \
	"v_pk_fma_f32 v[86:87], v[114:115], v[104:105], v[86:87] op_sel:[0,1,0] op_sel_hi:[1,1,1]\n\t" \
	"v_pk_fma_f32 v[84:85], v[116:117], v[106:107], v[84:85] op_sel:[0,0,0] op_sel_hi:[1,0,1]\n\t" \
	"v_pk_fma_f32 v[86:87], v[118:119], v[106:107], v[86:87] op_sel:[0,1,0] op_sel_hi:[1,1,1]\n\t" \
	"v_pk_fma_f32 v[84:85], v[120:121], v[108:109], v[84:85] op_sel:[0,0,0] op_sel_hi:[1,0,1]\n\t" \
	"v_pk_fma_f32 v[86:87], v[122:123], v[108:109], v[86:87] op_sel:[0,1,0] op_sel_hi:[1,1,1]\n\t" \
	"v_pk_fma_f32 v[84:85], v[124:125], v[110:111], v[84:85] op_sel:[0,0,0] op_sel_hi:[1,0,1]\n\t" \
	"v_pk_fma_f32 v[86:87], v[126:127], v[110:111], v[86:87] op_sel:[0,1,0] op_sel_hi:[1,1,1]\n\t" \
	"s_nop 0\n\t" \
	"v_pk_add_f32 v[84:85], v[84:85], v[86:87]\n\t" \
	"s_nop 0\n\t" \
	"v_pk_mul_f32 v[84:85], v[84:85], v[84:85]\n\t" \
	"s_nop 0\n\t" \
	"v_add_f32_e32 v88, v85, v84\n\t" \
	"v_fmamk_f32 v89, v88, 0x36c9539c, %[km]\n\t" \
	"v_sub_f32_e32 v90, v88, v89\n\t" \
	"v_add_f32_e32 v91, v88, v89\n\t" \
	"s_lshl_b32 s94, %[bidx], 9\n\t" \
	"v_mov_b32_dpp v90, v90 quad_perm:[1,0,3,2] row_mask:0xf bank_mask:0xf\n\t" \
	"v_cmp_lt_f32_e64 s[88:89], v91, v90\n\t" \
	"s_mov_b32 %[st], 1\n\t" \
	"s_lshr_b64 s[90:91], s[88:89], 1\n\t" \
	"s_or_b64 s[90:91], s[90:91], s[88:89]\n\t" \
	"s_mov_b32 s96, 0x55555555\n\t" \
	"s_mov_b32 s97, 0x15555555\n\t" \
	"s_and_b64 s[92:93], s[90:91], s[96:97]\n\t" \
	"s_cmp_eq_u64 s[92:93], s[96:97]\n\t" \
	"s_cbranch_scc0 .Lnb_da_careful\n\t" \
	"s_mov_b32 s95, 0\n\t" \
	"s_lshl1_add_u32 s96, s95, 0\n\t" \
	"s_bitcmp1_b64 s[88:89], s96\n\t" \
	"s_addc_u32 s95, s95, s95\n\t" \
	"s_lshl1_add_u32 s96, s95, 2\n\t" \
	"s_bitcmp1_b64 s[88:89], s96\n\t" \
	"s_addc_u32 s95, s95, s95\n\t" \
	"s_lshl1_add_u32 s96, s95, 6\n\t" \
	"s_bitcmp1_b64 s[88:89], s96\n\t" \
	"s_addc_u32 s95, s95, s95\n\t" \
	"s_lshl1_add_u32 s96, s95, 14\n\t" \
	"s_bitcmp1_b64 s[88:89], s96\n\t" \
	"s_addc_u32 s95, s95, s95\n\t" \
	"s_lshl1_add_u32 s96, s95, 30\n\t" \
	"s_bitcmp1_b64 s[88:89], s96\n\t" \
	"s_addc_u32 s95, s95, s95\n\t" \
	".Lnb_da_walked:\n\t" \
	"s_lshl_b32 s95, s95, 5\n\t" \
	"s_add_u32 s94, s94, s95\n\t" \
	"s_add_u32 %[e], s94, -1008\n\t" \
	"s_branch .Lnb_da_end\n\t" \
	".Lnb_da_careful:\n\t" \
	"s_mov_b32 s95, 0\n\t" \
	"s_lshl1_add_u32 s96, s95, 0\n\t" \
	"s_bitcmp0_b64 s[90:91], s96\n\t" \
	"s_cbranch_scc1 .Lnb_da_unsure\n\t" \
	"s_bitcmp1_b64 s[88:89], s96\n\t" \
	"s_addc_u32 s95, s95, s95\n\t" \
	"s_lshl1_add_u32 s96, s95, 2\n\t" \
	"s_bitcmp0_b64 s[90:91], s96\n\t" \
	"s_cbranch_scc1 .Lnb_da_unsure\n\t" \
	"s_bitcmp1_b64 s[88:89], s96\n\t" \
	"s_addc_u32 s95, s95, s95\n\t" \
	"s_lshl1_add_u32 s96, s95, 6\n\t" \
	"s_bitcmp0_b64 s[90:91], s96\n\t" \
	"s_cbranch_scc1 .Lnb_da_unsure\n\t" \
	"s_bitcmp1_b64 s[88:89], s96\n\t" \
	"s_addc_u32 s95, s95, s95\n\t" \
	"s_lshl1_add_u32 s96, s95, 14\n\t" \
	"s_bitcmp0_b64 s[90:91], s96\n\t" \
	"s_cbranch_scc1 .Lnb_da_unsure\n\t" \
	"s_bitcmp1_b64 s[88:89], s96\n\t" \
	"s_addc_u32 s95, s95, s95\n\t" \
	"s_lshl1_add_u32 s96, s95, 30\n\t" \
	"s_bitcmp0_b64 s[90:91], s96\n\t" \
	"s_cbranch_scc1 .Lnb_da_unsure\n\t" \
	"s_bitcmp1_b64 s[88:89], s96\n\t" \
	"s_addc_u32 s95, s95, s95\n\t" \
	"s_branch .Lnb_da_walked\n\t" \
	".Lnb_da_unsure:\n\t" \
	"s_mov_b32 %[st], 3\n\t" \
	"s_branch .Lnb_da_end\n\t" \
	".Lnb_da_wait_end:\n\t" \
	"s_mov_b64 exec, -1\n\t" \
	"s_waitcnt lgkmcnt(0)\n\t" \
	".Lnb_da_end:\n\t"
#define NB_ASM_DETB \
	"v_mov_b64_e32 v[64:65], 0\n\t" \
	"v_mov_b64_e32 v[66:67], 0\n\t" \
	"v_add_u32_e32 v68, %[e], %[kb]\n\t" \
	"s_add_u32 s88, %[czb], -56\n\t" \
	"s_mov_b32 exec_lo, 0x3fffffff\n\t" \
	"s_mov_b32 exec_hi, 0xffff\n\t" \
	"v_ashrrev_i32_e32 v69, 9, v68\n\t" \
	"v_and_b32_e32 v70, 0x1ff, v68\n\t" \
	"v_lshl_add_u32 v69, v69, 3, s88\n\t" \
	"v_bfe_u32 v71, v70, 4, 5\n\t" \
	"v_sub_u32_e32 v72, 0x200, v70\n\t" \
	"v_xor_b32_e32 v71, v71, v70\n\t" \
	"v_bfe_u32 v73, v72, 4, 5\n\t" \
	"v_lshlrev_b32_e32 v71, 2, v71\n\t" \
	"v_xor_b32_e32 v72, v73, v72\n\t" \
	"v_lshlrev_b32_e32 v72, 2, v72\n\t" \
	"ds_read_b64 v[80:81], v69 offset:0\n\t" \
	"ds_read_b32 v96, v71 offset:14336\n\t" \
	"ds_read_b64 v[82:83], v69 offset:8\n\t" \
	"ds_read_b32 v97, v71 offset:12288\n\t" \
	"ds_read_b64 v[84:85], v69 offset:16\n\t" \
	"ds_read_b32 v98, v71 offset:10240\n\t" \
	"ds_read_b64 v[86:87], v69 offset:24\n\t" \
	"ds_read_b32 v99, v71 offset:8192\n\t" \
	"ds_read_b64 v[88:89], v69 offset:32\n\t" \
	"ds_read_b32 v100, v71 offset:6144\n\t" \
	"ds_read_b64 v[90:91], v69 offset:40\n\t" \
	"ds_read_b32 v101, v71 offset:4096\n\t" \
	"ds_read_b64 v[92:93], v69 offset:48\n\t" \
	"ds_read_b32 v102, v71 offset:2048\n\t" \
	"ds_read_b64 v[94:95], v69 offset:56\n\t" \
	"ds_read_b32 v103, v71 offset:0\n\t" \
	"s_waitcnt lgkmcnt(12)\n\t" \
	"v_pk_fma_f32 v[64:65], v[80:81], v[96:97], v[64:65] op_sel:[0,0,0] op_sel_hi:[1,0,1]\n\t" \
	"v_pk_fma_f32 v[66:67], v[82:83], v[96:97], v[66:67] op_sel:[0,1,0] op_sel_hi:[1,1,1]\n\t" \
	"ds_read_b64 v[104:105], v69 offset:64\n\t" \
	"ds_read_b32 v120, v72 offset:0\n\t" \
	"ds_read_b64 v[106:107], v69 offset:72\n\t" \
	"ds_read_b32 v121, v72 offset:2048\n\t" \
	"s_waitcnt lgkmcnt(12)\n\t" \
	"v_pk_fma_f32 v[64:65], v[84:85], v[98:99], v[64:65] op_sel:[0,0,0] op_sel_hi:[1,0,1]\n\t" \
	"v_pk_fma_f32 v[66:67], v[86:87], v[98:99], v[66:67] op_sel:[0,1,0] op_sel_hi:[1,1,1]\n\t" \
	"ds_read_b64 v[108:109], v69 offset:80\n\t" \
	"ds_read_b32 v122, v72 offset:4096\n\t" \
	"ds_read_b64 v[110:111], v69 offset:88\n\t" \
	"ds_read_b32 v123, v72 offset:6144\n\t" \
	"s_waitcnt lgkmcnt(12)\n\t" \
	"v_pk_fma_f32 v[64:65], v[88:89], v[100:101], v[64:65] op_sel:[0,0,0] op_sel_hi:[1,0,1]\n\t" \
	"v_pk_fma_f32 v[66:67], v[90:91], v[100:101], v[66:67] op_sel:[0,1,0] op_sel_hi:[1,1,1]\n\t" \
	"ds_read_b64 v[112:113], v69 offset:96\n\t" \
	"ds_read_b32 v124, v72 offset:8192\n\t" \
	"ds_read_b64 v[114:115], v69 offset:104\n\t" \
	"ds_read_b32 v125, v72 offset:10240\n\t" \
	"s_waitcnt lgkmcnt(12)\n\t" \
	"v_pk_fma_f32 v[64:65], v[92:93], v[102:103], v[64:65] op_sel:[0,0,0] op_sel_hi:[1,0,1]\n\t" \
	"v_pk_fma_f32 v[66:67], v[94:95], v[102:103], v[66:67] op_sel:[0,1,0] op_sel_hi:[1,1,1]\n\t" \
	"ds_read_b64 v[116:117], v69 offset:112\n\t" \
	"ds_read_b32 v126, v72 offset:12288\n\t" \
	"ds_read_b64 v[118:119], v69 offset:120\n\t" \
	"ds_read_b32 v127, v72 offset:14336\n\t" \
	"s_waitcnt lgkmcnt(12)\n\t" \
	"v_pk_fma_f32 v[64:65], v[104:105], v[120:121], v[64:65] op_sel:[0,0,0] op_sel_hi:[1,0,1]\n\t" \
	"v_pk_fma_f32 v[66:67], v[106:107], v[120:121], v[66:67] op_sel:[0,1,0] op_sel_hi:[1,1,1]\n\t" \
	"s_waitcnt lgkmcnt(8)\n\t" \
	"v_pk_fma_f32 v[64:65], v[108:109], v[122:123], v[64:65] op_sel:[0,0,0] op_sel_hi:[1,0,1]\n\t" \
	"v_pk_fma_f32 v[66:67], v[110:111], v[122:123], v[66:67] op_sel:[0,1,0] op_sel_hi:[1,1,1]\n\t" \
	"s_waitcnt lgkmcnt(4)\n\t" \
	"v_pk_fma_f32 v[64:65], v[112:113], v[124:125], v[64:65] op_sel:[0,0,0] op_sel_hi:[1,0,1]\n\t" \
	"v_pk_fma_f32 v[66:67], v[114:115], v[124:125], v[66:67] op_sel:[0,1,0] op_sel_hi:[1,1,1]\n\t" \
	"s_waitcnt lgkmcnt(0)\n\t" \
	"v_pk_fma_f32 v[64:65], v[116:117], v[126:127], v[64:65] op_sel:[0,0,0] op_sel_hi:[1,0,1]\n\t" \
	"v_pk_fma_f32 v[66:67], v[118:119], v[126:127], v[66:67] op_sel:[0,1,0] op_sel_hi:[1,1,1]\n\t" \
	"s_mov_b64 exec, -1\n\t" \
	"v_pk_add_f32 v[74:75], v[64:65], v[66:67]\n\t" \
	"s_add_u32 s92, %[e], 497\n\t" \
	"v_pk_mul_f32 v[76:77], v[74:75], v[74:75]\n\t" \
	"s_mov_b32 %[st], 1\n\t" \
	"v_add_f32_e32 v78, v77, v76\n\t" \
	"v_fmamk_f32 v79, v78, 0x36c9539c, %[km]\n\t" \
	"v_sub_f32_e32 v96, v78, v79\n\t" \
	"v_add_f32_e32 v97, v78, v79\n\t" \
	"s_nop 0\n\t" \
	"v_mov_b32_dpp v96, v96 quad_perm:[1,0,3,2] row_mask:0xf bank_mask:0xf\n\t" \
	"v_cmp_lt_f32_e64 s[88:89], v97, v96\n\t" \
	"s_lshr_b32 s90, s88, 1\n\t" \
	"s_or_b32 s90, s90, s88\n\t" \
	"s_and_b32 s91, s90, 0x15555555\n\t" \
	"s_cmp_eq_u32 s91, 0x15555555\n\t" \
	"s_cbranch_scc0 .Lnb_db_careful\n\t" \
	"s_mov_b32 s94, 0\n\t" \
	"s_lshl1_add_u32 s95, s94, 0\n\t" \
	"s_bitcmp1_b32 s88, s95\n\t" \
	"s_addc_u32 s94, s94, s94\n\t" \
	"s_lshl1_add_u32 s95, s94, 2\n\t" \
	"s_bitcmp1_b32 s88, s95\n\t" \
	"s_addc_u32 s94, s94, s94\n\t" \
	"s_lshl1_add_u32 s95, s94, 6\n\t" \
	"s_bitcmp1_b32 s88, s95\n\t" \
	"s_addc_u32 s94, s94, s94\n\t" \
	"s_lshl1_add_u32 s95, s94, 14\n\t" \
	"s_bitcmp1_b32 s88, s95\n\t" \
	"s_addc_u32 s94, s94, s94\n\t" \
	".Lnb_db_walked:\n\t" \
	"s_add_u32 s93, s94, 32\n\t" \
	"s_lshl1_add_u32 %[toa], s94, s92\n\t" \
	"v_readlane_b32 %[xr], v74, s93\n\t" \
	"v_readlane_b32 %[xi], v75, s93\n\t" \
	"s_branch .Lnb_db_end\n\t" \
	".Lnb_db_careful:\n\t" \
	"s_mov_b32 s94, 0\n\t" \
	"s_lshl1_add_u32 s95, s94, 0\n\t" \
	"s_bitcmp0_b32 s90, s95\n\t" \
	"s_cbranch_scc1 .Lnb_db_unsure\n\t" \
	"s_bitcmp1_b32 s88, s95\n\t" \
	"s_addc_u32 s94, s94, s94\n\t" \
	"s_lshl1_add_u32 s95, s94, 2\n\t" \
	"s_bitcmp0_b32 s90, s95\n\t" \
	"s_cbranch_scc1 .Lnb_db_unsure\n\t" \
	"s_bitcmp1_b32 s88, s95\n\t" \
	"s_addc_u32 s94, s94, s94\n\t" \
	"s_lshl1_add_u32 s95, s94, 6\n\t" \
	"s_bitcmp0_b32 s90, s95\n\t" \
	"s_cbranch_scc1 .Lnb_db_unsure\n\t" \
	"s_bitcmp1_b32 s88, s95\n\t" \
	"s_addc_u32 s94, s94, s94\n\t" \
	"s_lshl1_add_u32 s95, s94, 14\n\t" \
	"s_bitcmp0_b32 s90, s95\n\t" \
	"s_cbranch_scc1 .Lnb_db_unsure\n\t" \
	"s_bitcmp1_b32 s88, s95\n\t" \
	"s_addc_u32 s94, s94, s94\n\t" \
	"s_branch .Lnb_db_walked\n\t" \
	".Lnb_db_unsure:\n\t" \
	"s_mov_b32 %[st], 3\n\t" \
	".Lnb_db_end:\n\t"
#define NB_ASM_TAIL \
	"v_mov_b32_e32 v65, %[hdrb]\n\t" \
	"ds_read_b128 v[68:71], v65\n\t" \
	"s_sub_u32 s88, %[t5], %[toa]\n\t" \
	"s_add_u32 s87, s88, 5120\n\t" \
	"s_mov_b32 %[ok], 0\n\t" \
	"s_and_b32 s91, s87, 127\n\t" \
	"s_lshr_b32 s92, s91, 1\n\t" \
	"s_cmp_ge_u32 s91, 2\n\t" \
	"s_cselect_b32 s92, s92, 64\n\t" \
	"s_mul_i32 s93, s92, 768\n\t" \
	"s_add_u32 s94, %[e8lo], s93\n\t" \
	"s_addc_u32 s95, %[e8hi], 0\n\t" \
	"s_abs_i32 s96, %[toa]\n\t" \
	"s_add_u32 s96, s96, 256\n\t" \
	"global_load_dwordx4 v[120:123], %[l16], s[94:95]\n\t" \
	"s_lshr_b32 s96, s96, 9\n\t" \
	"s_sub_u32 s97, 0, s96\n\t" \
	"s_cmp_lt_i32 %[toa], 0\n\t" \
	"s_cselect_b32 s96, s97, s96\n\t" \
	"s_lshl_b32 s96, s96, 3\n\t" \
	"v_add_u32_e32 v64, s96, %[vd]\n\t" \
	"s_bfm_b64 exec, 16, 0\n\t" \
	"ds_read_b64 v[66:67], v64\n\t" \
	"s_mov_b64 exec, -1\n\t" \
	"s_waitcnt lgkmcnt(1)\n\t" \
	"v_mul_f32_e32 v82, %[xr], v70\n\t" \
	"v_mul_f32_e32 v83, %[xr], v71\n\t" \
	"v_mul_f32_e32 v84, %[xi], v71\n\t" \
	"v_mul_f32_e32 v85, %[xi], v70\n\t" \
	"v_sub_f32_e32 v86, v82, v84\n\t" \
	"v_add_f32_e32 v87, v83, v85\n\t" \
	"v_mul_f32_e32 v90, v86, v86\n\t" \
	"v_mul_f32_e32 v89, v87, v87\n\t" \
	"v_add_f32_e32 v89, v89, v90\n\t" \
	"v_rcp_f32_e32 v89, v89\n\t" \
	"s_mov_b32 s88, 0xaaaaaaaa\n\t" \
	"s_mov_b32 s89, 0xaaaaaaaa\n\t" \
	"v_mul_f32_e32 v91, v86, v89\n\t" \
	"v_mul_f32_e64 v92, -v87, v89\n\t" \
	"v_cndmask_b32_e64 v119, v91, v92, s[88:89]\n\t" \
	"s_mov_b32 s88, 0xcccccccc\n\t" \
	"s_mov_b32 s89, 0xcccccccc\n\t" \
	"v_cndmask_b32_e64 v119, v119, -v119, s[88:89]\n\t" \
	"s_bfm_b64 exec, 16, 0\n\t" \
	"s_waitcnt lgkmcnt(0)\n\t" \
	"v_pk_mul_f32 v[66:67], v[66:67], v[66:67]\n\t" \
	"s_ashr_i32 s88, s87, 7\n\t" \
	"v_add_f32_e32 v81, v67, v66\n\t" \
	"s_and_b32 s89, s87, 127\n\t" \
	"s_lshr_b32 s90, s89, 1\n\t" \
	"v_add_f32_dpp v81, v81, v81 quad_perm:[1,0,3,2] row_mask:0xf bank_mask:0xf\n\t" \
	"s_cmp_ge_u32 s89, 2\n\t" \
	"s_cselect_b32 s90, s90, 64\n\t" \
	"v_add_f32_dpp v81, v81, v81 quad_perm:[2,3,0,1] row_mask:0xf bank_mask:0xf\n\t" \
	"s_sub_u32 s91, -18, s88\n\t" \
	"s_and_b32 s92, s91, 3\n\t" \
	"v_add_f32_dpp v81, v81, v81 row_half_mirror row_mask:0xf bank_mask:0xf\n\t" \
	"s_ashr_i32 s93, s91, 2\n\t" \
	"s_mul_i32 s94, s92, 180\n\t" \
	"v_add_f32_dpp v81, v81, v81 row_mirror row_mask:0xf bank_mask:0xf\n\t" \
	"s_add_u32 s94, s94, s93\n\t" \
	"s_lshl3_add_u32 s94, s94, %[pb]\n\t" \
	"v_mul_f32_e32 v81, 0x3d800000, v81\n\t" \
	"s_mul_i32 s95, s90, 144\n\t" \
	"s_add_u32 s95, s95, %[cb]\n\t" \
	"v_readlane_b32 %[ssum], v81, 0\n\t" \
	"s_mov_b64 exec, -1\n\t" \
	"s_sub_u32 s96, 0, s88\n\t" \
	"s_cmp_gt_u32 s96, 36\n\t" \
	"s_cbranch_scc1 .Lnb_tl_wait_end\n\t" \
	"s_mov_b32 %[ok], 1\n\t" \
	"v_add_u32_e32 v112, s94, %[kic]\n\t" \
	"s_add_u32 s96, s92, 1\n\t" \
	"s_lshr_b32 s96, s96, 2\n\t" \
	"s_mul_i32 s96, s96, -5752\n\t" \
	"s_add_u32 s96, s96, 1440\n\t" \
	"v_add_u32_e32 v113, s96, v112\n\t" \
	"s_add_u32 s96, s92, 2\n\t" \
	"s_lshr_b32 s96, s96, 2\n\t" \
	"s_mul_i32 s96, s96, -5752\n\t" \
	"s_add_u32 s96, s96, 2880\n\t" \
	"v_add_u32_e32 v114, s96, v112\n\t" \
	"s_add_u32 s96, s92, 3\n\t" \
	"s_lshr_b32 s96, s96, 2\n\t" \
	"s_mul_i32 s96, s96, -5752\n\t" \
	"s_add_u32 s96, s96, 4320\n\t" \
	"v_add_u32_e32 v115, s96, v112\n\t" \
	"s_mov_b32 exec_hi, 0x0ff0ffff\n\t" \
	"ds_read_b64 v[72:73], v112 offset:96\n\t" \
	"ds_read_b64 v[74:75], v113 offset:96\n\t" \
	"ds_read_b64 v[76:77], v114 offset:96\n\t" \
	"ds_read_b64 v[78:79], v115 offset:96\n\t" \
	"ds_read_b64 v[80:81], v112 offset:104\n\t" \
	"ds_read_b64 v[82:83], v113 offset:104\n\t" \
	"ds_read_b64 v[84:85], v114 offset:104\n\t" \
	"ds_read_b64 v[86:87], v115 offset:104\n\t" \
	"ds_read_b64 v[88:89], v112 offset:112\n\t" \
	"ds_read_b64 v[90:91], v113 offset:112\n\t" \
	"ds_read_b64 v[92:93], v114 offset:112\n\t" \
	"ds_read_b64 v[94:95], v115 offset:112\n\t" \
	"v_add_u32_e32 v116, %[db], %[l16]\n\t" \
	"v_cmp_lt_i32_e32 vcc, -1, %[ktp]\n\t" \
	"v_add_u32_e32 v117, %[db], %[ktp]\n\t" \
	"v_mov_b32_e32 v118, s95\n\t" \
	"v_mov_b64_e32 v[64:65], 0\n\t" \
	"v_mov_b64_e32 v[66:67], 0\n\t" \
	"v_mov_b64_e32 v[68:69], 0\n\t" \
	"v_cndmask_b32_e32 v117, v118, v117, vcc\n\t" \
	"s_waitcnt vmcnt(0)\n\t" \
	"ds_write_b128 v116, v[120:123]\n\t" \
	"ds_read_b128 v[104:107], v117\n\t" \
	"ds_read_b128 v[108:111], v117 offset:16\n\t" \
	"ds_read_b64 v[96:97], v112 offset:120\n\t" \
	"ds_read_b64 v[98:99], v113 offset:120\n\t" \
	"ds_read_b64 v[100:101], v114 offset:120\n\t" \
	"ds_read_b64 v[102:103], v115 offset:120\n\t" \
	"s_waitcnt lgkmcnt(5)\n\t" \
	"v_pk_fma_f32 v[64:65], v[72:73], v[104:105], v[64:65] op_sel:[0,0,0] op_sel_hi:[1,0,1]\n\t" \
	"v_pk_fma_f32 v[66:67], v[80:81], v[104:105], v[66:67] op_sel:[0,0,0] op_sel_hi:[1,0,1]\n\t" \
	"v_pk_fma_f32 v[68:69], v[88:89], v[104:105], v[68:69] op_sel:[0,0,0] op_sel_hi:[1,0,1]\n\t" \
	"v_pk_fma_f32 v[64:65], v[74:75], v[104:105], v[64:65] op_sel:[0,1,0] op_sel_hi:[1,1,1]\n\t" \
	"v_pk_fma_f32 v[66:67], v[82:83], v[104:105], v[66:67] op_sel:[0,1,0] op_sel_hi:[1,1,1]\n\t" \
	"v_pk_fma_f32 v[68:69], v[90:91], v[104:105], v[68:69] op_sel:[0,1,0] op_sel_hi:[1,1,1]\n\t" \
	"v_pk_fma_f32 v[64:65], v[76:77], v[106:107], v[64:65] op_sel:[0,0,0] op_sel_hi:[1,0,1]\n\t" \
	"v_pk_fma_f32 v[66:67], v[84:85], v[106:107], v[66:67] op_sel:[0,0,0] op_sel_hi:[1,0,1]\n\t" \
	"v_pk_fma_f32 v[68:69], v[92:93], v[106:107], v[68:69] op_sel:[0,0,0] op_sel_hi:[1,0,1]\n\t" \
	"v_pk_fma_f32 v[64:65], v[78:79], v[106:107], v[64:65] op_sel:[0,1,0] op_sel_hi:[1,1,1]\n\t" \
	"v_pk_fma_f32 v[66:67], v[86:87], v[106:107], v[66:67] op_sel:[0,1,0] op_sel_hi:[1,1,1]\n\t" \
	"v_pk_fma_f32 v[68:69], v[94:95], v[106:107], v[68:69] op_sel:[0,1,0] op_sel_hi:[1,1,1]\n\t" \
	"ds_read_b128 v[104:107], v117 offset:32\n\t" \
	"ds_read_b64 v[72:73], v112 offset:128\n\t" \
	"ds_read_b64 v[74:75], v113 offset:128\n\t" \
	"ds_read_b64 v[76:77], v114 offset:128\n\t" \
	"ds_read_b64 v[78:79], v115 offset:128\n\t" \
	"s_waitcnt lgkmcnt(5)\n\t" \
	"v_pk_fma_f32 v[64:65], v[80:81], v[108:109], v[64:65] op_sel:[0,0,0] op_sel_hi:[1,0,1]\n\t" \
	"v_pk_fma_f32 v[66:67], v[88:89], v[108:109], v[66:67] op_sel:[0,0,0] op_sel_hi:[1,0,1]\n\t" \
	"v_pk_fma_f32 v[68:69], v[96:97], v[108:109], v[68:69] op_sel:[0,0,0] op_sel_hi:[1,0,1]\n\t" \
	"v_pk_fma_f32 v[64:65], v[82:83], v[108:109], v[64:65] op_sel:[0,1,0] op_sel_hi:[1,1,1]\n\t" \
	"v_pk_fma_f32 v[66:67], v[90:91], v[108:109], v[66:67] op_sel:[0,1,0] op_sel_hi:[1,1,1]\n\t" \
	"v_pk_fma_f32 v[68:69], v[98:99], v[108:109], v[68:69] op_sel:[0,1,0] op_sel_hi:[1,1,1]\n\t" \
	"v_pk_fma_f32 v[64:65], v[84:85], v[110:111], v[64:65] op_sel:[0,0,0] op_sel_hi:[1,0,1]\n\t" \
	"v_pk_fma_f32 v[66:67], v[92:93], v[110:111], v[66:67] op_sel:[0,0,0] op_sel_hi:[1,0,1]\n\t" \
	"v_pk_fma_f32 v[68:69], v[100:101], v[110:111], v[68:69] op_sel:[0,0,0] op_sel_hi:[1,0,1]\n\t" \
	"v_pk_fma_f32 v[64:65], v[86:87], v[110:111], v[64:65] op_sel:[0,1,0] op_sel_hi:[1,1,1]\n\t" \
	"v_pk_fma_f32 v[66:67], v[94:95], v[110:111], v[66:67] op_sel:[0,1,0] op_sel_hi:[1,1,1]\n\t" \
	"v_pk_fma_f32 v[68:69], v[102:103], v[110:111], v[68:69] op_sel:[0,1,0] op_sel_hi:[1,1,1]\n\t" \
	"ds_read_b128 v[108:111], v117 offset:48\n\t" \
	"ds_read_b64 v[80:81], v112 offset:136\n\t" \
	"ds_read_b64 v[82:83], v113 offset:136\n\t" \
	"ds_read_b64 v[84:85], v114 offset:136\n\t" \
	"ds_read_b64 v[86:87], v115 offset:136\n\t" \
	"s_waitcnt lgkmcnt(5)\n\t" \
	"v_pk_fma_f32 v[64:65], v[88:89], v[104:105], v[64:65] op_sel:[0,0,0] op_sel_hi:[1,0,1]\n\t" \
	"v_pk_fma_f32 v[66:67], v[96:97], v[104:105], v[66:67] op_sel:[0,0,0] op_sel_hi:[1,0,1]\n\t" \
	"v_pk_fma_f32 v[68:69], v[72:73], v[104:105], v[68:69] op_sel:[0,0,0] op_sel_hi:[1,0,1]\n\t" \
	"v_pk_fma_f32 v[64:65], v[90:91], v[104:105], v[64:65] op_sel:[0,1,0] op_sel_hi:[1,1,1]\n\t" \
	"v_pk_fma_f32 v[66:67], v[98:99], v[104:105], v[66:67] op_sel:[0,1,0] op_sel_hi:[1,1,1]\n\t" \
	"v_pk_fma_f32 v[68:69], v[74:75], v[104:105], v[68:69] op_sel:[0,1,0] op_sel_hi:[1,1,1]\n\t" \
	"v_pk_fma_f32 v[64:65], v[92:93], v[106:107], v[64:65] op_sel:[0,0,0] op_sel_hi:[1,0,1]\n\t" \
	"v_pk_fma_f32 v[66:67], v[100:101], v[106:107], v[66:67] op_sel:[0,0,0] op_sel_hi:[1,0,1]\n\t" \
	"v_pk_fma_f32 v[68:69], v[76:77], v[106:107], v[68:69] op_sel:[0,0,0] op_sel_hi:[1,0,1]\n\t" \
	"v_pk_fma_f32 v[64:65], v[94:95], v[106:107], v[64:65] op_sel:[0,1,0] op_sel_hi:[1,1,1]\n\t" \
	"v_pk_fma_f32 v[66:67], v[102:103], v[106:107], v[66:67] op_sel:[0,1,0] op_sel_hi:[1,1,1]\n\t" \
	"v_pk_fma_f32 v[68:69], v[78:79], v[106:107], v[68:69] op_sel:[0,1,0] op_sel_hi:[1,1,1]\n\t" \
	"ds_read_b128 v[104:107], v117 offset:64\n\t" \
	"ds_read_b64 v[88:89], v112 offset:144\n\t" \
	"ds_read_b64 v[90:91], v113 offset:144\n\t" \
	"ds_read_b64 v[92:93], v114 offset:144\n\t" \
	"ds_read_b64 v[94:95], v115 offset:144\n\t" \
	"s_waitcnt lgkmcnt(5)\n\t" \
	"v_pk_fma_f32 v[64:65], v[96:97], v[108:109], v[64:65] op_sel:[0,0,0] op_sel_hi:[1,0,1]\n\t" \
	"v_pk_fma_f32 v[66:67], v[72:73], v[108:109], v[66:67] op_sel:[0,0,0] op_sel_hi:[1,0,1]\n\t" \
	"v_pk_fma_f32 v[68:69], v[80:81], v[108:109], v[68:69] op_sel:[0,0,0] op_sel_hi:[1,0,1]\n\t" \
	"v_pk_fma_f32 v[64:65], v[98:99], v[108:109], v[64:65] op_sel:[0,1,0] op_sel_hi:[1,1,1]\n\t" \
	"v_pk_fma_f32 v[66:67], v[74:75], v[108:109], v[66:67] op_sel:[0,1,0] op_sel_hi:[1,1,1]\n\t" \
	"v_pk_fma_f32 v[68:69], v[82:83], v[108:109], v[68:69] op_sel:[0,1,0] op_sel_hi:[1,1,1]\n\t" \
	"v_pk_fma_f32 v[64:65], v[100:101], v[110:111], v[64:65] op_sel:[0,0,0] op_sel_hi:[1,0,1]\n\t" \
	"v_pk_fma_f32 v[66:67], v[76:77], v[110:111], v[66:67] op_sel:[0,0,0] op_sel_hi:[1,0,1]\n\t" \
	"v_pk_fma_f32 v[68:69], v[84:85], v[110:111], v[68:69] op_sel:[0,0,0] op_sel_hi:[1,0,1]\n\t" \
	"v_pk_fma_f32 v[64:65], v[102:103], v[110:111], v[64:65] op_sel:[0,1,0] op_sel_hi:[1,1,1]\n\t" \
	"v_pk_fma_f32 v[66:67], v[78:79], v[110:111], v[66:67] op_sel:[0,1,0] op_sel_hi:[1,1,1]\n\t" \
	"v_pk_fma_f32 v[68:69], v[86:87], v[110:111], v[68:69] op_sel:[0,1,0] op_sel_hi:[1,1,1]\n\t" \
	"ds_read_b128 v[108:111], v117 offset:80\n\t" \
	"ds_read_b64 v[96:97], v112 offset:152\n\t" \
	"ds_read_b64 v[98:99], v113 offset:152\n\t" \
	"ds_read_b64 v[100:101], v114 offset:152\n\t" \
	"ds_read_b64 v[102:103], v115 offset:152\n\t" \
	"s_waitcnt lgkmcnt(5)\n\t" \
	"v_pk_fma_f32 v[64:65], v[72:73], v[104:105], v[64:65] op_sel:[0,0,0] op_sel_hi:[1,0,1]\n\t" \
	"v_pk_fma_f32 v[66:67], v[80:81], v[104:105], v[66:67] op_sel:[0,0,0] op_sel_hi:[1,0,1]\n\t" \
	"v_pk_fma_f32 v[68:69], v[88:89], v[104:105], v[68:69] op_sel:[0,0,0] op_sel_hi:[1,0,1]\n\t" \
	"v_pk_fma_f32 v[64:65], v[74:75], v[104:105], v[64:65] op_sel:[0,1,0] op_sel_hi:[1,1,1]\n\t" \
	"v_pk_fma_f32 v[66:67], v[82:83], v[104:105], v[66:67] op_sel:[0,1,0] op_sel_hi:[1,1,1]\n\t" \
	"v_pk_fma_f32 v[68:69], v[90:91], v[104:105], v[68:69] op_sel:[0,1,0] op_sel_hi:[1,1,1]\n\t" \
	"v_pk_fma_f32 v[64:65], v[76:77], v[106:107], v[64:65] op_sel:[0,0,0] op_sel_hi:[1,0,1]\n\t" \
	"v_pk_fma_f32 v[66:67], v[84:85], v[106:107], v[66:67] op_sel:[0,0,0] op_sel_hi:[1,0,1]\n\t" \
	"v_pk_fma_f32 v[68:69], v[92:93], v[106:107], v[68:69] op_sel:[0,0,0] op_sel_hi:[1,0,1]\n\t" \
	"v_pk_fma_f32 v[64:65], v[78:79], v[106:107], v[64:65] op_sel:[0,1,0] op_sel_hi:[1,1,1]\n\t" \
	"v_pk_fma_f32 v[66:67], v[86:87], v[106:107], v[66:67] op_sel:[0,1,0] op_sel_hi:[1,1,1]\n\t" \
	"v_pk_fma_f32 v[68:69], v[94:95], v[106:107], v[68:69] op_sel:[0,1,0] op_sel_hi:[1,1,1]\n\t" \
	"s_waitcnt lgkmcnt(0)\n\t" \
	"v_pk_fma_f32 v[64:65], v[80:81], v[108:109], v[64:65] op_sel:[0,0,0] op_sel_hi:[1,0,1]\n\t" \
	"v_pk_fma_f32 v[66:67], v[88:89], v[108:109], v[66:67] op_sel:[0,0,0] op_sel_hi:[1,0,1]\n\t" \
	"v_pk_fma_f32 v[68:69], v[96:97], v[108:109], v[68:69] op_sel:[0,0,0] op_sel_hi:[1,0,1]\n\t" \
	"v_pk_fma_f32 v[64:65], v[82:83], v[108:109], v[64:65] op_sel:[0,1,0] op_sel_hi:[1,1,1]\n\t" \
	"v_pk_fma_f32 v[66:67], v[90:91], v[108:109], v[66:67] op_sel:[0,1,0] op_sel_hi:[1,1,1]\n\t" \
	"v_pk_fma_f32 v[68:69], v[98:99], v[108:109], v[68:69] op_sel:[0,1,0] op_sel_hi:[1,1,1]\n\t" \
	"v_pk_fma_f32 v[64:65], v[84:85], v[110:111], v[64:65] op_sel:[0,0,0] op_sel_hi:[1,0,1]\n\t" \
	"v_pk_fma_f32 v[66:67], v[92:93], v[110:111], v[66:67] op_sel:[0,0,0] op_sel_hi:[1,0,1]\n\t" \
	"v_pk_fma_f32 v[68:69], v[100:101], v[110:111], v[68:69] op_sel:[0,0,0] op_sel_hi:[1,0,1]\n\t" \
	"v_pk_fma_f32 v[64:65], v[86:87], v[110:111], v[64:65] op_sel:[0,1,0] op_sel_hi:[1,1,1]\n\t" \
	"v_pk_fma_f32 v[66:67], v[94:95], v[110:111], v[66:67] op_sel:[0,1,0] op_sel_hi:[1,1,1]\n\t" \
	"v_pk_fma_f32 v[68:69], v[102:103], v[110:111], v[68:69] op_sel:[0,1,0] op_sel_hi:[1,1,1]\n\t" \
	"s_nop 0\n\t" \
	"v_add_f32_dpp v64, v64, v64 row_shl:4 row_mask:0x8 bank_mask:0xf\n\t" \
	"v_add_f32_dpp v65, v65, v65 row_shl:4 row_mask:0x8 bank_mask:0xf\n\t" \
	"v_mul_f32_dpp %[d1], v119, v66 quad_perm:[1,0,3,2] row_mask:0xf bank_mask:0xf\n\t" \
	"v_mul_f32_dpp %[d2], v119, v68 quad_perm:[2,1,0,3] row_mask:0xf bank_mask:0xf\n\t" \
	"v_mul_f32_dpp %[d0], v119, v64 quad_perm:[0,3,2,1] row_mask:0xf bank_mask:0xf\n\t" \
	"v_fmac_f32_dpp %[d1], v119, v67 quad_perm:[0,3,2,1] row_mask:0xf bank_mask:0xf\n\t" \
	"v_fmac_f32_dpp %[d2], v119, v69 quad_perm:[1,0,3,2] row_mask:0xf bank_mask:0xf\n\t" \
	"v_fmac_f32_dpp %[d0], v119, v65 quad_perm:[3,2,1,0] row_mask:0xf bank_mask:0xf\n\t" \
	"s_mov_b64 exec, -1\n\t" \
	"s_branch .Lnb_tl_end\n\t" \
	".Lnb_tl_wait_end:\n\t" \
	"s_waitcnt vmcnt(0)\n\t" \
	".Lnb_tl_end:\n\t"
#define NB_ASM_FIRG \
	"s_ashr_i32 s88, %[nk], 7\n\t" \
	"s_and_b32 s89, %[nk], 127\n\t" \
	"s_lshr_b32 s90, s89, 1\n\t" \
	"s_cmp_ge_u32 s89, 2\n\t" \
	"s_cselect_b32 s90, s90, 64\n\t" \
	"s_sub_u32 s91, -18, s88\n\t" \
	"s_and_b32 s92, s91, 3\n\t" \
	"s_ashr_i32 s93, s91, 2\n\t" \
	"s_mul_i32 s94, s92, 180\n\t" \
	"s_add_u32 s94, s94, s93\n\t" \
	"s_lshl3_add_u32 s94, s94, %[pb]\n\t" \
	"s_mul_i32 s95, s90, 144\n\t" \
	"s_add_u32 s95, s95, %[cb]\n\t" \
	"v_add_u32_e32 v112, s94, %[kic]\n\t" \
	"s_add_u32 s96, s92, 1\n\t" \
	"s_lshr_b32 s96, s96, 2\n\t" \
	"s_mul_i32 s96, s96, -5752\n\t" \
	"s_add_u32 s96, s96, 1440\n\t" \
	"v_add_u32_e32 v113, s96, v112\n\t" \
	"s_add_u32 s96, s92, 2\n\t" \
	"s_lshr_b32 s96, s96, 2\n\t" \
	"s_mul_i32 s96, s96, -5752\n\t" \
	"s_add_u32 s96, s96, 2880\n\t" \
	"v_add_u32_e32 v114, s96, v112\n\t" \
	"s_add_u32 s96, s92, 3\n\t" \
	"s_lshr_b32 s96, s96, 2\n\t" \
	"s_mul_i32 s96, s96, -5752\n\t" \
	"s_add_u32 s96, s96, 4320\n\t" \
	"v_add_u32_e32 v115, s96, v112\n\t" \
	"v_mov_b64_e32 %[a0], 0\n\t" \
	"v_mov_b64_e32 %[a1], 0\n\t" \
	"v_mov_b64_e32 %[a2], 0\n\t" \
	"v_mov_b32_e32 v117, s95\n\t" \
	"s_bfm_b64 exec, 52, 0\n\t" \
	"ds_read_b64 v[72:73], v112 offset:96\n\t" \
	"ds_read_b64 v[74:75], v113 offset:96\n\t" \
	"ds_read_b64 v[76:77], v114 offset:96\n\t" \
	"ds_read_b64 v[78:79], v115 offset:96\n\t" \
	"ds_read_b64 v[80:81], v112 offset:104\n\t" \
	"ds_read_b64 v[82:83], v113 offset:104\n\t" \
	"ds_read_b64 v[84:85], v114 offset:104\n\t" \
	"ds_read_b64 v[86:87], v115 offset:104\n\t" \
	"ds_read_b64 v[88:89], v112 offset:112\n\t" \
	"ds_read_b64 v[90:91], v113 offset:112\n\t" \
	"ds_read_b64 v[92:93], v114 offset:112\n\t" \
	"ds_read_b64 v[94:95], v115 offset:112\n\t" \
	"ds_read_b128 v[104:107], v117\n\t" \
	"ds_read_b128 v[108:111], v117 offset:16\n\t" \
	"ds_read_b64 v[96:97], v112 offset:120\n\t" \
	"ds_read_b64 v[98:99], v113 offset:120\n\t" \
	"ds_read_b64 v[100:101], v114 offset:120\n\t" \
	"ds_read_b64 v[102:103], v115 offset:120\n\t" \
	"s_waitcnt lgkmcnt(5)\n\t" \
	"v_pk_fma_f32 %[a0], v[72:73], v[104:105], %[a0] op_sel:[0,0,0] op_sel_hi:[1,0,1]\n\t" \
	"v_pk_fma_f32 %[a1], v[80:81], v[104:105], %[a1] op_sel:[0,0,0] op_sel_hi:[1,0,1]\n\t" \
	"v_pk_fma_f32 %[a2], v[88:89], v[104:105], %[a2] op_sel:[0,0,0] op_sel_hi:[1,0,1]\n\t" \
	"v_pk_fma_f32 %[a0], v[74:75], v[104:105], %[a0] op_sel:[0,1,0] op_sel_hi:[1,1,1]\n\t" \
	"v_pk_fma_f32 %[a1], v[82:83], v[104:105], %[a1] op_sel:[0,1,0] op_sel_hi:[1,1,1]\n\t" \
	"v_pk_fma_f32 %[a2], v[90:91], v[104:105], %[a2] op_sel:[0,1,0] op_sel_hi:[1,1,1]\n\t" \
	"v_pk_fma_f32 %[a0], v[76:77], v[106:107], %[a0] op_sel:[0,0,0] op_sel_hi:[1,0,1]\n\t" \
	"v_pk_fma_f32 %[a1], v[84:85], v[106:107], %[a1] op_sel:[0,0,0] op_sel_hi:[1,0,1]\n\t" \
	"v_pk_fma_f32 %[a2], v[92:93], v[106:107], %[a2] op_sel:[0,0,0] op_sel_hi:[1,0,1]\n\t" \
	"v_pk_fma_f32 %[a0], v[78:79], v[106:107], %[a0] op_sel:[0,1,0] op_sel_hi:[1,1,1]\n\t" \
	"v_pk_fma_f32 %[a1], v[86:87], v[106:107], %[a1] op_sel:[0,1,0] op_sel_hi:[1,1,1]\n\t" \
	"v_pk_fma_f32 %[a2], v[94:95], v[106:107], %[a2] op_sel:[0,1,0] op_sel_hi:[1,1,1]\n\t" \
	"ds_read_b128 v[104:107], v117 offset:32\n\t" \
	"ds_read_b64 v[72:73], v112 offset:128\n\t" \
	"ds_read_b64 v[74:75], v113 offset:128\n\t" \
	"ds_read_b64 v[76:77], v114 offset:128\n\t" \
	"ds_read_b64 v[78:79], v115 offset:128\n\t" \
	"s_waitcnt lgkmcnt(5)\n\t" \
	"v_pk_fma_f32 %[a0], v[80:81], v[108:109], %[a0] op_sel:[0,0,0] op_sel_hi:[1,0,1]\n\t" \
	"v_pk_fma_f32 %[a1], v[88:89], v[108:109], %[a1] op_sel:[0,0,0] op_sel_hi:[1,0,1]\n\t" \
	"v_pk_fma_f32 %[a2], v[96:97], v[108:109], %[a2] op_sel:[0,0,0] op_sel_hi:[1,0,1]\n\t" \
	"v_pk_fma_f32 %[a0], v[82:83], v[108:109], %[a0] op_sel:[0,1,0] op_sel_hi:[1,1,1]\n\t" \
	"v_pk_fma_f32 %[a1], v[90:91], v[108:109], %[a1] op_sel:[0,1,0] op_sel_hi:[1,1,1]\n\t" \
	"v_pk_fma_f32 %[a2], v[98:99], v[108:109], %[a2] op_sel:[0,1,0] op_sel_hi:[1,1,1]\n\t" \
	"v_pk_fma_f32 %[a0], v[84:85], v[110:111], %[a0] op_sel:[0,0,0] op_sel_hi:[1,0,1]\n\t" \
	"v_pk_fma_f32 %[a1], v[92:93], v[110:111], %[a1] op_sel:[0,0,0] op_sel_hi:[1,0,1]\n\t" \
	"v_pk_fma_f32 %[a2], v[100:101], v[110:111], %[a2] op_sel:[0,0,0] op_sel_hi:[1,0,1]\n\t" \
	"v_pk_fma_f32 %[a0], v[86:87], v[110:111], %[a0] op_sel:[0,1,0] op_sel_hi:[1,1,1]\n\t" \
	"v_pk_fma_f32 %[a1], v[94:95], v[110:111], %[a1] op_sel:[0,1,0] op_sel_hi:[1,1,1]\n\t" \
	"v_pk_fma_f32 %[a2], v[102:103], v[110:111], %[a2] op_sel:[0,1,0] op_sel_hi:[1,1,1]\n\t" \
	"ds_read_b128 v[108:111], v117 offset:48\n\t" \
	"ds_read_b64 v[80:81], v112 offset:136\n\t" \
	"ds_read_b64 v[82:83], v113 offset:136\n\t" \
	"ds_read_b64 v[84:85], v114 offset:136\n\t" \
	"ds_read_b64 v[86:87], v115 offset:136\n\t" \
	"s_waitcnt lgkmcnt(5)\n\t" \
	"v_pk_fma_f32 %[a0], v[88:89], v[104:105], %[a0] op_sel:[0,0,0] op_sel_hi:[1,0,1]\n\t" \
	"v_pk_fma_f32 %[a1], v[96:97], v[104:105], %[a1] op_sel:[0,0,0] op_sel_hi:[1,0,1]\n\t" \
	"v_pk_fma_f32 %[a2], v[72:73], v[104:105], %[a2] op_sel:[0,0,0] op_sel_hi:[1,0,1]\n\t" \
	"v_pk_fma_f32 %[a0], v[90:91], v[104:105], %[a0] op_sel:[0,1,0] op_sel_hi:[1,1,1]\n\t" \
	"v_pk_fma_f32 %[a1], v[98:99], v[104:105], %[a1] op_sel:[0,1,0] op_sel_hi:[1,1,1]\n\t" \
	"v_pk_fma_f32 %[a2], v[74:75], v[104:105], %[a2] op_sel:[0,1,0] op_sel_hi:[1,1,1]\n\t" \
	"v_pk_fma_f32 %[a0], v[92:93], v[106:107], %[a0] op_sel:[0,0,0] op_sel_hi:[1,0,1]\n\t" \
	"v_pk_fma_f32 %[a1], v[100:101], v[106:107], %[a1] op_sel:[0,0,0] op_sel_hi:[1,0,1]\n\t" \
	"v_pk_fma_f32 %[a2], v[76:77], v[106:107], %[a2] op_sel:[0,0,0] op_sel_hi:[1,0,1]\n\t" \
	"v_pk_fma_f32 %[a0], v[94:95], v[106:107], %[a0] op_sel:[0,1,0] op_sel_hi:[1,1,1]\n\t" \
	"v_pk_fma_f32 %[a1], v[102:103], v[106:107], %[a1] op_sel:[0,1,0] op_sel_hi:[1,1,1]\n\t" \
	"v_pk_fma_f32 %[a2], v[78:79], v[106:107], %[a2] op_sel:[0,1,0] op_sel_hi:[1,1,1]\n\t" \
	"ds_read_b128 v[104:107], v117 offset:64\n\t" \
	"ds_read_b64 v[88:89], v112 offset:144\n\t" \
	"ds_read_b64 v[90:91], v113 offset:144\n\t" \
	"ds_read_b64 v[92:93], v114 offset:144\n\t" \
	"ds_read_b64 v[94:95], v115 offset:144\n\t" \
	"s_waitcnt lgkmcnt(5)\n\t" \
	"v_pk_fma_f32 %[a0], v[96:97], v[108:109], %[a0] op_sel:[0,0,0] op_sel_hi:[1,0,1]\n\t" \
	"v_pk_fma_f32 %[a1], v[72:73], v[108:109], %[a1] op_sel:[0,0,0] op_sel_hi:[1,0,1]\n\t" \
	"v_pk_fma_f32 %[a2], v[80:81], v[108:109], %[a2] op_sel:[0,0,0] op_sel_hi:[1,0,1]\n\t" \
	"v_pk_fma_f32 %[a0], v[98:99], v[108:109], %[a0] op_sel:[0,1,0] op_sel_hi:[1,1,1]\n\t" \
	"v_pk_fma_f32 %[a1], v[74:75], v[108:109], %[a1] op_sel:[0,1,0] op_sel_hi:[1,1,1]\n\t" \
	"v_pk_fma_f32 %[a2], v[82:83], v[108:109], %[a2] op_sel:[0,1,0] op_sel_hi:[1,1,1]\n\t" \
	"v_pk_fma_f32 %[a0], v[100:101], v[110:111], %[a0] op_sel:[0,0,0] op_sel_hi:[1,0,1]\n\t" \
	"v_pk_fma_f32 %[a1], v[76:77], v[110:111], %[a1] op_sel:[0,0,0] op_sel_hi:[1,0,1]\n\t" \
	"v_pk_fma_f32 %[a2], v[84:85], v[110:111], %[a2] op_sel:[0,0,0] op_sel_hi:[1,0,1]\n\t" \
	"v_pk_fma_f32 %[a0], v[102:103], v[110:111], %[a0] op_sel:[0,1,0] op_sel_hi:[1,1,1]\n\t" \
	"v_pk_fma_f32 %[a1], v[78:79], v[110:111], %[a1] op_sel:[0,1,0] op_sel_hi:[1,1,1]\n\t" \
	"v_pk_fma_f32 %[a2], v[86:87], v[110:111], %[a2] op_sel:[0,1,0] op_sel_hi:[1,1,1]\n\t" \
	"ds_read_b128 v[108:111], v117 offset:80\n\t" \
	"ds_read_b64 v[96:97], v112 offset:152\n\t" \
	"ds_read_b64 v[98:99], v113 offset:152\n\t" \
	"ds_read_b64 v[100:101], v114 offset:152\n\t" \
	"ds_read_b64 v[102:103], v115 offset:152\n\t" \
	"s_waitcnt lgkmcnt(5)\n\t" \
	"v_pk_fma_f32 %[a0], v[72:73], v[104:105], %[a0] op_sel:[0,0,0] op_sel_hi:[1,0,1]\n\t" \
	"v_pk_fma_f32 %[a1], v[80:81], v[104:105], %[a1] op_sel:[0,0,0] op_sel_hi:[1,0,1]\n\t" \
	"v_pk_fma_f32 %[a2], v[88:89], v[104:105], %[a2] op_sel:[0,0,0] op_sel_hi:[1,0,1]\n\t" \
	"v_pk_fma_f32 %[a0], v[74:75], v[104:105], %[a0] op_sel:[0,1,0] op_sel_hi:[1,1,1]\n\t" \
	"v_pk_fma_f32 %[a1], v[82:83], v[104:105], %[a1] op_sel:[0,1,0] op_sel_hi:[1,1,1]\n\t" \
	"v_pk_fma_f32 %[a2], v[90:91], v[104:105], %[a2] op_sel:[0,1,0] op_sel_hi:[1,1,1]\n\t" \
	"v_pk_fma_f32 %[a0], v[76:77], v[106:107], %[a0] op_sel:[0,0,0] op_sel_hi:[1,0,1]\n\t" \
	"v_pk_fma_f32 %[a1], v[84:85], v[106:107], %[a1] op_sel:[0,0,0] op_sel_hi:[1,0,1]\n\t" \
	"v_pk_fma_f32 %[a2], v[92:93], v[106:107], %[a2] op_sel:[0,0,0] op_sel_hi:[1,0,1]\n\t" \
	"v_pk_fma_f32 %[a0], v[78:79], v[106:107], %[a0] op_sel:[0,1,0] op_sel_hi:[1,1,1]\n\t" \
	"v_pk_fma_f32 %[a1], v[86:87], v[106:107], %[a1] op_sel:[0,1,0] op_sel_hi:[1,1,1]\n\t" \
	"v_pk_fma_f32 %[a2], v[94:95], v[106:107], %[a2] op_sel:[0,1,0] op_sel_hi:[1,1,1]\n\t" \
	"s_waitcnt lgkmcnt(0)\n\t" \
	"v_pk_fma_f32 %[a0], v[80:81], v[108:109], %[a0] op_sel:[0,0,0] op_sel_hi:[1,0,1]\n\t" \
	"v_pk_fma_f32 %[a1], v[88:89], v[108:109], %[a1] op_sel:[0,0,0] op_sel_hi:[1,0,1]\n\t" \
	"v_pk_fma_f32 %[a2], v[96:97], v[108:109], %[a2] op_sel:[0,0,0] op_sel_hi:[1,0,1]\n\t" \
	"v_pk_fma_f32 %[a0], v[82:83], v[108:109], %[a0] op_sel:[0,1,0] op_sel_hi:[1,1,1]\n\t" \
	"v_pk_fma_f32 %[a1], v[90:91], v[108:109], %[a1] op_sel:[0,1,0] op_sel_hi:[1,1,1]\n\t" \
	"v_pk_fma_f32 %[a2], v[98:99], v[108:109], %[a2] op_sel:[0,1,0] op_sel_hi:[1,1,1]\n\t" \
	"v_pk_fma_f32 %[a0], v[84:85], v[110:111], %[a0] op_sel:[0,0,0] op_sel_hi:[1,0,1]\n\t" \
	"v_pk_fma_f32 %[a1], v[92:93], v[110:111], %[a1] op_sel:[0,0,0] op_sel_hi:[1,0,1]\n\t" \
	"v_pk_fma_f32 %[a2], v[100:101], v[110:111], %[a2] op_sel:[0,0,0] op_sel_hi:[1,0,1]\n\t" \
	"v_pk_fma_f32 %[a0], v[86:87], v[110:111], %[a0] op_sel:[0,1,0] op_sel_hi:[1,1,1]\n\t" \
	"v_pk_fma_f32 %[a1], v[94:95], v[110:111], %[a1] op_sel:[0,1,0] op_sel_hi:[1,1,1]\n\t" \
	"v_pk_fma_f32 %[a2], v[102:103], v[110:111], %[a2] op_sel:[0,1,0] op_sel_hi:[1,1,1]\n\t" \
	"s_mov_b64 exec, -1\n\t"
#define NB_ASM_AMAX(FILL0, FILL1, FILL2, FILL3, FILL4, FILL5, FILL6, FILL7) \
	"v_mov_b32_e32 v88, %[nrm]\n\t" \
	"v_mov_b32_dpp v89, %[ep] quad_perm:[0,0,0,0] row_mask:0xf bank_mask:0xf\n\t" \
	FILL0 "\n\t" \
	"v_max_f32_dpp v88, v88, v88 quad_perm:[1,0,3,2] row_mask:0xf bank_mask:0xf\n\t" \
	"v_add_f32_dpp v89, v89, v89 row_half_mirror row_mask:0xf bank_mask:0xf\n\t" \
	FILL1 "\n\t" \
	"v_max_f32_dpp v88, v88, v88 quad_perm:[2,3,0,1] row_mask:0xf bank_mask:0xf\n\t" \
	"v_add_f32_dpp v89, v89, v89 row_mirror row_mask:0xf bank_mask:0xf\n\t" \
	FILL2 "\n\t" \
	"v_max_f32_dpp v88, v88, v88 row_half_mirror row_mask:0xf bank_mask:0xf\n\t" \
	"v_add_f32_dpp v89, v89, v89 row_bcast:15 row_mask:0xa bank_mask:0xf\n\t" \
	FILL3 "\n\t" \
	"v_max_f32_dpp v88, v88, v88 row_mirror row_mask:0xf bank_mask:0xf\n\t" \
	"v_add_f32_dpp v89, v89, v89 row_bcast:31 row_mask:0xc bank_mask:0xf\n\t" \
	FILL4 "\n\t" \
	"v_max_f32_dpp v88, v88, v88 row_bcast:15 row_mask:0xa bank_mask:0xf\n\t" \
	FILL5 "\n\t" \
	"v_readlane_b32 %[es], v89, 63\n\t" \
	"v_max_f32_dpp v88, v88, v88 row_bcast:31 row_mask:0xc bank_mask:0xf\n\t" \
	FILL6 "\n\t" \
	FILL7 "\n\t" \
	"v_readlane_b32 %[m], v88, 63\n\t" \
	"s_nop 1\n\t" \
	"v_cmp_eq_f32_e32 vcc, %[m], %[nrm]\n\t" \
	"s_ff1_i32_b64 %[bidx], vcc\n\t"
```

Baseline: 1048.

## Keep decimated samples in registers and correlate via DPP lane shifts for short windows

For search windows up to a fixed length, the decimator now works on shifted lanes and combines taps with DPP wave shifts. It hands its outputs to the correlator in registers instead of having the correlator reload them from LDS. The correlator runs the training-sequence correlation as a chain of DPP-shifted adds with a lane offset, and the peak index is corrected by that offset afterwards. Longer windows keep the original LDS-based path. This removes LDS reads and waitcnt stalls on the hot path, but adds much larger unrolled code, a data-dependent branch, and a tight lane-indexing scheme that must match the old output exactly.

```diff
diff --git a/osmo_trx_amd/csrc/trx_kernel_nb.hip b/osmo_trx_amd/csrc/trx_kernel_nb.hip
--- a/osmo_trx_amd/csrc/trx_kernel_nb.hip
+++ b/osmo_trx_amd/csrc/trx_kernel_nb.hip
@@ -36,6 +36,7 @@
 	static_assert(NB_TABLES_BYTES % 16 == 0 && (NB_SLICE * 8) % 16 == 0 && (K4_XS * 8) % 16 == 0 && (NB_D_LEN * 8) % 16 == 0, "16-byte LDS accesses");
 	static_assert(NB_LDS_BYTES <= 160 * 1024, "LDS");
 	static_assert(NB_ASM_GDEC_OFF == (TRX_SINCV_LDS + 16 * WAVE + NB_COMP_ROWS * 36) * 4, "tools/gen_nb_asm.py: LDS offset of the decimator taps");
+	static_assert(NB_ASM_DEC_MAX_NACT == 15 + NB_ASM_CORR_MAX_LEN, "tools/gen_nb_asm.py: DEC and CORR change form at the same window");
 	static_assert(NB_ASM_LSEQ_OFF == (NB_TABLES_FLOATS - 2 * 8 * 16) * 4, "tools/gen_nb_asm.py: LDS offset of the training-sequence taps");
 	constexpr int NLD = 10;
 	extern __shared__ __attribute__((aligned(16))) char smem[];
@@ -377,16 +378,20 @@
 			__builtin_assume(len >= 16 && len <= 16 + NB_MAX_TOA);
 			const unsigned vd_addr = lds_addr(D) + 8u * (unsigned)lane, vcz_addr = lds_addr(cz) + 8u * (unsigned)lane;
 			unsigned long long bad;
+			float dr, di;
 			asm volatile(NB_ASM_DEC
-				     : [bad] "=s"(bad)
-				     : [pd] "v"(lds_addr(P + PH_M0 + 52) + 8u * (unsigned)lane), [vd] "v"(vd_addr), [zero] "v"(0), [nact] "s"(15 + len)
+				     : [bad] "=s"(bad), [dr] "=&v"(dr), [di] "=&v"(di)
+				     : [pd] "v"(lds_addr(P + PH_M0 + 52) + 8u * (unsigned)lane), [vd] "v"(vd_addr), [vd4] "v"(vd_addr - 32u), [zero] "v"(0),
+				       [nact] "s"(15 + len)
 				     : NB_ASM_CLOBBERS);
 			DIAG_MARK(2);
 			{
 				float v;
+				const int lag0 = (len <= NB_ASM_CORR_MAX_LEN) ? NB_ASM_CORR_LANE0 : 0;
 				asm volatile(NB_ASM_CORR
 					     : [nrm] "=&v"(v)
-					     : [vd] "v"(vd_addr), [vcz] "v"(vcz_addr), [len] "s"(len), [tsc] "s"(tsc), [bad] "s"(bad)
+					     : [vd] "v"(vd_addr), [vcz] "v"(vcz_addr), [vdm] "v"(vd_addr - 8u * NB_ASM_CORR_LANE0),
+					       [vczm] "v"(vcz_addr - 8u * NB_ASM_CORR_LANE0), [dr] "v"(dr), [di] "v"(di), [len] "s"(len), [tsc] "s"(tsc), [bad] "s"(bad)
 					     : NB_ASM_CLOBBERS);
 				DIAG_MARK(3);
 				int m_bits, es_bits, bidx;
@@ -394,10 +399,11 @@
 				asm volatile(NB_ASM_AMAX("ds_read_b32 %[kr], %[l4] offset:%c[lc]", "ds_read_b32 %[ka], %[l4] offset:%c[lc]+256",
 							 "ds_read_b32 %[kb], %[l4] offset:%c[lc]+512", "ds_read_b32 %[kic], %[l4] offset:%c[lc]+768",
 							 "ds_read_b32 %[ktp], %[l4] offset:%c[lc]+1024", "s_nop 0", "s_nop 0", "s_nop 0")
+					     "s_sub_u32 %[bidx], %[bidx], %[lag0]\n\t"
 					     "s_waitcnt lgkmcnt(0)"
-					     : [m] "=s"(m_bits), [es] "=s"(es_bits), [bidx] "=s"(bidx), [kr] "=&v"(kr), [ka] "=&v"(ka), [kb] "=&v"(kb),
+					     : [m] "=&s"(m_bits), [es] "=&s"(es_bits), [bidx] "=&s"(bidx), [kr] "=&v"(kr), [ka] "=&v"(ka), [kb] "=&v"(kb),
 					       [kic] "=&v"(kic), [ktp] "=&v"(ktp)
-					     : [nrm] "v"(v), [ep] "v"(epart), [l4] "v"(4 * lane),
+					     : [nrm] "v"(v), [ep] "v"(epart), [l4] "v"(4 * lane), [lag0] "s"(lag0),
 					       [lc] "n"((TRX_SINCV_LDS + 16 * WAVE + NB_COMP_ROWS * 36 + 16 + 64 + 5 * WAVE) * 4)
 					     : NB_ASM_CLOBBERS);
 				DIAG_MARK(4);
diff --git a/osmo_trx_amd/csrc/trx_nb_asm.inc b/osmo_trx_amd/csrc/trx_nb_asm.inc
--- a/osmo_trx_amd/csrc/trx_nb_asm.inc
+++ b/osmo_trx_amd/csrc/trx_nb_asm.inc
@@ -1,7 +1,73 @@
 #define NB_ASM_GDEC_OFF 29968
 #define NB_ASM_LSEQ_OFF 32848
+#define NB_ASM_DEC_MAX_NACT 60
+#define NB_ASM_CORR_LANE0 19
+#define NB_ASM_CORR_MAX_LEN 45
 #define NB_ASM_CLOBBERS "v64", "v65", "v66", "v67", "v68", "v69", "v70", "v71", "v72", "v73", "v74", "v75", "v76", "v77", "v78", "v79", "v80", "v81", "v82", "v83", "v84", "v85", "v86", "v87", "v88", "v89", "v90", "v91", "v92", "v93", "v94", "v95", "v96", "v97", "v98", "v99", "v100", "v101", "v102", "v103", "v104", "v105", "v106", "v107", "v108", "v109", "v110", "v111", "v112", "v113", "v114", "v115", "v116", "v117", "v118", "v119", "v120", "v121", "v122", "v123", "v124", "v125", "v126", "v127", "s87", "s88", "s89", "s90", "s91", "s92", "s93", "s94", "s95", "s96", "s97", "s98", "s99", "vcc", "scc", "memory"
 #define NB_ASM_DEC \
+	"s_cmp_gt_u32 %[nact], 60\n\t" \
+	"s_cbranch_scc1 .Lnb_dec_wide\n\t" \
+	"s_sub_u32 s88, 60, %[nact]\n\t" \
+	"s_lshr_b64 exec, -1, s88\n\t" \
+	"ds_read_b128 v[120:123], %[zero] offset:29968\n\t" \
+	"ds_read_b128 v[124:127], %[zero] offset:29984\n\t" \
+	"ds_read_b64 v[98:99], %[pd] offset:1440\n\t" \
+	"ds_read_b64 v[100:101], %[pd] offset:2880\n\t" \
+	"ds_read_b64 v[102:103], %[pd] offset:4320\n\t" \
+	"ds_read_b64 v[96:97], %[pd] offset:0\n\t" \
+	"s_waitcnt lgkmcnt(3)\n\t" \
+	"v_pk_mul_f32 v[64:65], v[98:99], v[120:121] op_sel:[0,0] op_sel_hi:[1,0]\n\t" \
+	"s_waitcnt lgkmcnt(2)\n\t" \
+	"v_pk_mul_f32 v[66:67], v[100:101], v[120:121] op_sel:[0,1] op_sel_hi:[1,1]\n\t" \
+	"s_waitcnt lgkmcnt(1)\n\t" \
+	"v_pk_mul_f32 v[68:69], v[102:103], v[122:123] op_sel:[0,0] op_sel_hi:[1,0]\n\t" \
+	"v_pk_add_f32 v[104:105], v[64:65], v[66:67]\n\t" \
+	"s_waitcnt lgkmcnt(0)\n\t" \
+	"v_pk_mul_f32 v[70:71], v[96:97], v[122:123] op_sel:[0,1] op_sel_hi:[1,1]\n\t" \
+	"v_pk_add_f32 v[104:105], v[104:105], v[68:69]\n\t" \
+	"v_pk_mul_f32 v[72:73], v[98:99], v[124:125] op_sel:[0,0] op_sel_hi:[1,0]\n\t" \
+	"v_pk_mul_f32 v[74:75], v[100:101], v[124:125] op_sel:[0,1] op_sel_hi:[1,1]\n\t" \
+	"v_add_f32_dpp v104, v104, v70 wave_shr:1 row_mask:0xf bank_mask:0xf bound_ctrl:0\n\t" \
+	"v_add_f32_dpp v105, v105, v71 wave_shr:1 row_mask:0xf bank_mask:0xf bound_ctrl:0\n\t" \
+	"v_pk_mul_f32 v[76:77], v[102:103], v[126:127] op_sel:[0,0] op_sel_hi:[1,0]\n\t" \
+	"v_pk_add_f32 v[104:105], v[104:105], v[72:73]\n\t" \
+	"v_pk_mul_f32 v[78:79], v[96:97], v[126:127] op_sel:[0,1] op_sel_hi:[1,1]\n\t" \
+	"v_pk_add_f32 v[104:105], v[104:105], v[74:75]\n\t" \
+	"v_pk_mul_f32 v[80:81], v[98:99], v[126:127] op_sel:[0,1] op_sel_hi:[1,1]\n\t" \
+	"v_pk_add_f32 v[104:105], v[104:105], v[76:77]\n\t" \
+	"v_pk_mul_f32 v[82:83], v[100:101], v[126:127] op_sel:[0,0] op_sel_hi:[1,0]\n\t" \
+	"v_pk_mul_f32 v[84:85], v[102:103], v[124:125] op_sel:[0,1] op_sel_hi:[1,1]\n\t" \
+	"v_add_f32_dpp v104, v104, v78 wave_shr:1 row_mask:0xf bank_mask:0xf bound_ctrl:0\n\t" \
+	"v_add_f32_dpp v105, v105, v79 wave_shr:1 row_mask:0xf bank_mask:0xf bound_ctrl:0\n\t" \
+	"v_pk_mul_f32 v[86:87], v[96:97], v[124:125] op_sel:[0,0] op_sel_hi:[1,0]\n\t" \
+	"v_pk_add_f32 v[104:105], v[104:105], v[80:81]\n\t" \
+	"v_pk_mul_f32 v[88:89], v[98:99], v[122:123] op_sel:[0,1] op_sel_hi:[1,1]\n\t" \
+	"v_pk_add_f32 v[104:105], v[104:105], v[82:83]\n\t" \
+	"v_pk_mul_f32 v[90:91], v[100:101], v[122:123] op_sel:[0,0] op_sel_hi:[1,0]\n\t" \
+	"v_pk_add_f32 v[104:105], v[104:105], v[84:85]\n\t" \
+	"v_pk_mul_f32 v[92:93], v[102:103], v[120:121] op_sel:[0,1] op_sel_hi:[1,1]\n\t" \
+	"v_pk_mul_f32 v[94:95], v[96:97], v[120:121] op_sel:[0,0] op_sel_hi:[1,0]\n\t" \
+	"v_add_f32_dpp v104, v104, v86 wave_shr:1 row_mask:0xf bank_mask:0xf bound_ctrl:0\n\t" \
+	"v_add_f32_dpp v105, v105, v87 wave_shr:1 row_mask:0xf bank_mask:0xf bound_ctrl:0\n\t" \
+	"v_pk_add_f32 v[104:105], v[104:105], v[88:89]\n\t" \
+	"s_nop 0\n\t" \
+	"v_pk_add_f32 v[104:105], v[104:105], v[90:91]\n\t" \
+	"s_nop 0\n\t" \
+	"v_pk_add_f32 v[104:105], v[104:105], v[92:93]\n\t" \
+	"s_nop 1\n\t" \
+	"v_add_f32_dpp %[dr], v104, v94 wave_shr:1 row_mask:0xf bank_mask:0xf bound_ctrl:0\n\t" \
+	"v_add_f32_dpp %[di], v105, v95 wave_shr:1 row_mask:0xf bank_mask:0xf bound_ctrl:0\n\t" \
+	"s_bfm_b64 exec, %[nact], 4\n\t" \
+	"ds_write2_b32 %[vd4], %[dr], %[di] offset1:1\n\t" \
+	"v_min_f32_e64 v106, |%[dr]|, |%[di]|\n\t" \
+	"v_max_f32_e64 v107, |%[dr]|, |%[di]|\n\t" \
+	"v_ldexp_f32 v106, v106, 17\n\t" \
+	"v_cmp_lt_f32_e32 vcc, v106, v107\n\t" \
+	"s_mov_b64 exec, -1\n\t" \
+	"s_mov_b64 %[bad], vcc\n\t" \
+	"s_waitcnt lgkmcnt(0)\n\t" \
+	"s_branch .Lnb_dec_end\n\t" \
+	".Lnb_dec_wide:\n\t" \
 	"s_bfm_b64 exec, %[nact], 0\n\t" \
 	"ds_read_b128 v[120:123], %[zero] offset:29968\n\t" \
 	"ds_read_b128 v[124:127], %[zero] offset:29984\n\t" \
@@ -64,8 +130,559 @@
 	"v_cmp_lt_f32_e32 vcc, v90, v91\n\t" \
 	"s_mov_b64 exec, -1\n\t" \
 	"s_mov_b64 %[bad], vcc\n\t" \
-	"s_waitcnt lgkmcnt(0)\n\t"
+	"s_waitcnt lgkmcnt(0)\n\t" \
+	".Lnb_dec_end:\n\t"
 #define NB_ASM_CORR \
+	"s_cmp_gt_u32 %[len], 45\n\t" \
+	"s_cbranch_scc1 .Lnb_corr_wide\n\t" \
+	"v_mov_b64_e32 v[120:121], 0\n\t" \
+	"v_mov_b64_e32 v[122:123], 0\n\t" \
+	"v_mov_b32_e32 %[nrm], 0\n\t" \
+	"s_lshl_b32 s90, %[len], 3\n\t" \
+	"s_sub_u32 s91, 45, %[len]\n\t" \
+	"v_add_u32_e32 v64, s90, %[vcz]\n\t" \
+	"s_lshr_b64 exec, -1, s91\n\t" \
+	"s_cmp_lg_u64 %[bad], 0\n\t" \
+	"s_cbranch_scc1 .Lnb_corrr_mul\n\t" \
+	"s_getpc_b64 s[88:89]\n\t" \
+	".Lnb_corrr_pc:\n\t" \
+	"s_mul_i32 s90, %[tsc], .Lnb_corrr_v1-.Lnb_corrr_v0\n\t" \
+	"s_add_u32 s88, s88, s90\n\t" \
+	"s_addc_u32 s89, s89, 0\n\t" \
+	"s_add_u32 s88, s88, .Lnb_corrr_v0-.Lnb_corrr_pc\n\t" \
+	"s_addc_u32 s89, s89, 0\n\t" \
+	"s_setpc_b64 s[88:89]\n\t" \
+	".Lnb_corrr_v0:\n\t" \
+	"v_sub_f32_e32 v120, 0, %[dr]\n\t" \
+	"v_sub_f32_e32 v121, 0, %[di]\n\t" \
+	"s_nop 0\n\t" \
+	"v_add_f32_dpp v120, v120, %[di] wave_shr:1 row_mask:0xf bank_mask:0xf bound_ctrl:0\n\t" \
+	"v_sub_f32_dpp v121, v121, %[dr] wave_shr:1 row_mask:0xf bank_mask:0xf bound_ctrl:0\n\t" \
+	"s_nop 0\n\t" \
+	"v_add_f32_dpp v120, v120, %[dr] wave_shr:1 row_mask:0xf bank_mask:0xf bound_ctrl:0\n\t" \
+	"v_add_f32_dpp v121, v121, %[di] wave_shr:1 row_mask:0xf bank_mask:0xf bound_ctrl:0\n\t" \
+	"s_nop 0\n\t" \
+	"v_add_f32_dpp v120, v120, %[di] wave_shr:1 row_mask:0xf bank_mask:0xf bound_ctrl:0\n\t" \
+	"v_sub_f32_dpp v121, v121, %[dr] wave_shr:1 row_mask:0xf bank_mask:0xf bound_ctrl:0\n\t" \
+	"s_nop 0\n\t" \
+	"v_sub_f32_dpp v120, v120, %[dr] wave_shr:1 row_mask:0xf bank_mask:0xf bound_ctrl:0\n\t" \
+	"v_sub_f32_dpp v121, v121, %[di] wave_shr:1 row_mask:0xf bank_mask:0xf bound_ctrl:0\n\t" \
+	"s_nop 0\n\t" \
+	"v_add_f32_dpp v120, v120, %[di] wave_shr:1 row_mask:0xf bank_mask:0xf bound_ctrl:0\n\t" \
+	"v_sub_f32_dpp v121, v121, %[dr] wave_shr:1 row_mask:0xf bank_mask:0xf bound_ctrl:0\n\t" \
+	"s_nop 0\n\t" \
+	"v_sub_f32_dpp v120, v120, %[dr] wave_shr:1 row_mask:0xf bank_mask:0xf bound_ctrl:0\n\t" \
+	"v_sub_f32_dpp v121, v121, %[di] wave_shr:1 row_mask:0xf bank_mask:0xf bound_ctrl:0\n\t" \
+	"s_nop 0\n\t" \
+	"v_sub_f32_dpp v120, v120, %[di] wave_shr:1 row_mask:0xf bank_mask:0xf bound_ctrl:0\n\t" \
+	"v_add_f32_dpp v121, v121, %[dr] wave_shr:1 row_mask:0xf bank_mask:0xf bound_ctrl:0\n\t" \
+	"s_nop 0\n\t" \
+	"v_add_f32_dpp v120, v120, %[dr] wave_shr:1 row_mask:0xf bank_mask:0xf bound_ctrl:0\n\t" \
+	"v_add_f32_dpp v121, v121, %[di] wave_shr:1 row_mask:0xf bank_mask:0xf bound_ctrl:0\n\t" \
+	"s_nop 0\n\t" \
+	"v_sub_f32_dpp v120, v120, %[di] wave_shr:1 row_mask:0xf bank_mask:0xf bound_ctrl:0\n\t" \
+	"v_add_f32_dpp v121, v121, %[dr] wave_shr:1 row_mask:0xf bank_mask:0xf bound_ctrl:0\n\t" \
+	"s_nop 0\n\t" \
+	"v_sub_f32_dpp v120, v120, %[dr] wave_shr:1 row_mask:0xf bank_mask:0xf bound_ctrl:0\n\t" \
+	"v_sub_f32_dpp v121, v121, %[di] wave_shr:1 row_mask:0xf bank_mask:0xf bound_ctrl:0\n\t" \
+	"s_nop 0\n\t" \
+	"v_sub_f32_dpp v120, v120, %[di] wave_shr:1 row_mask:0xf bank_mask:0xf bound_ctrl:0\n\t" \
+	"v_add_f32_dpp v121, v121, %[dr] wave_shr:1 row_mask:0xf bank_mask:0xf bound_ctrl:0\n\t" \
+	"s_nop 0\n\t" \
+	"v_add_f32_dpp v120, v120, %[dr] wave_shr:1 row_mask:0xf bank_mask:0xf bound_ctrl:0\n\t" \
+	"v_add_f32_dpp v121, v121, %[di] wave_shr:1 row_mask:0xf bank_mask:0xf bound_ctrl:0\n\t" \
+	"s_nop 0\n\t" \
+	"v_sub_f32_dpp v120, v120, %[di] wave_shr:1 row_mask:0xf bank_mask:0xf bound_ctrl:0\n\t" \
+	"v_add_f32_dpp v121, v121, %[dr] wave_shr:1 row_mask:0xf bank_mask:0xf bound_ctrl:0\n\t" \
+	"s_nop 0\n\t" \
+	"v_sub_f32_dpp v120, v120, %[dr] wave_shr:1 row_mask:0xf bank_mask:0xf bound_ctrl:0\n\t" \
+	"v_sub_f32_dpp v121, v121, %[di] wave_shr:1 row_mask:0xf bank_mask:0xf bound_ctrl:0\n\t" \
+	"s_nop 0\n\t" \
+	"v_sub_f32_dpp v120, v120, %[di] wave_shr:1 row_mask:0xf bank_mask:0xf bound_ctrl:0\n\t" \
+	"v_add_f32_dpp v121, v121, %[dr] wave_shr:1 row_mask:0xf bank_mask:0xf bound_ctrl:0\n\t" \
+	"s_branch .Lnb_corrr_join\n\t" \
+	".Lnb_corrr_v1:\n\t" \
+	"v_sub_f32_e32 v120, 0, %[dr]\n\t" \
+	"v_sub_f32_e32 v121, 0, %[di]\n\t" \
+	"s_nop 0\n\t" \
+	"v_add_f32_dpp v120, v120, %[di] wave_shr:1 row_mask:0xf bank_mask:0xf bound_ctrl:0\n\t" \
+	"v_sub_f32_dpp v121, v121, %[dr] wave_shr:1 row_mask:0xf bank_mask:0xf bound_ctrl:0\n\t" \
+	"s_nop 0\n\t" \
+	"v_add_f32_dpp v120, v120, %[dr] wave_shr:1 row_mask:0xf bank_mask:0xf bound_ctrl:0\n\t" \
+	"v_add_f32_dpp v121, v121, %[di] wave_shr:1 row_mask:0xf bank_mask:0xf bound_ctrl:0\n\t" \
+	"s_nop 0\n\t" \
+	"v_add_f32_dpp v120, v120, %[di] wave_shr:1 row_mask:0xf bank_mask:0xf bound_ctrl:0\n\t" \
+	"v_sub_f32_dpp v121, v121, %[dr] wave_shr:1 row_mask:0xf bank_mask:0xf bound_ctrl:0\n\t" \
+	"s_nop 0\n\t" \
+	"v_sub_f32_dpp v120, v120, %[dr] wave_shr:1 row_mask:0xf bank_mask:0xf bound_ctrl:0\n\t" \
+	"v_sub_f32_dpp v121, v121, %[di] wave_shr:1 row_mask:0xf bank_mask:0xf bound_ctrl:0\n\t" \
+	"s_nop 0\n\t" \
+	"v_add_f32_dpp v120, v120, %[di] wave_shr:1 row_mask:0xf bank_mask:0xf bound_ctrl:0\n\t" \
+	"v_sub_f32_dpp v121, v121, %[dr] wave_shr:1 row_mask:0xf bank_mask:0xf bound_ctrl:0\n\t" \
+	"s_nop 0\n\t" \
+	"v_add_f32_dpp v120, v120, %[dr] wave_shr:1 row_mask:0xf bank_mask:0xf bound_ctrl:0\n\t" \
+	"v_add_f32_dpp v121, v121, %[di] wave_shr:1 row_mask:0xf bank_mask:0xf bound_ctrl:0\n\t" \
+	"s_nop 0\n\t" \
+	"v_add_f32_dpp v120, v120, %[di] wave_shr:1 row_mask:0xf bank_mask:0xf bound_ctrl:0\n\t" \
+	"v_sub_f32_dpp v121, v121, %[dr] wave_shr:1 row_mask:0xf bank_mask:0xf bound_ctrl:0\n\t" \
+	"s_nop 0\n\t" \
+	"v_sub_f32_dpp v120, v120, %[dr] wave_shr:1 row_mask:0xf bank_mask:0xf bound_ctrl:0\n\t" \
+	"v_sub_f32_dpp v121, v121, %[di] wave_shr:1 row_mask:0xf bank_mask:0xf bound_ctrl:0\n\t" \
+	"s_nop 0\n\t" \
+	"v_sub_f32_dpp v120, v120, %[di] wave_shr:1 row_mask:0xf bank_mask:0xf bound_ctrl:0\n\t" \
+	"v_add_f32_dpp v121, v121, %[dr] wave_shr:1 row_mask:0xf bank_mask:0xf bound_ctrl:0\n\t" \
+	"s_nop 0\n\t" \
+	"v_sub_f32_dpp v120, v120, %[dr] wave_shr:1 row_mask:0xf bank_mask:0xf bound_ctrl:0\n\t" \
+	"v_sub_f32_dpp v121, v121, %[di] wave_shr:1 row_mask:0xf bank_mask:0xf bound_ctrl:0\n\t" \
+	"s_nop 0\n\t" \
+	"v_sub_f32_dpp v120, v120, %[di] wave_shr:1 row_mask:0xf bank_mask:0xf bound_ctrl:0\n\t" \
+	"v_add_f32_dpp v121, v121, %[dr] wave_shr:1 row_mask:0xf bank_mask:0xf bound_ctrl:0\n\t" \
+	"s_nop 0\n\t" \
+	"v_add_f32_dpp v120, v120, %[dr] wave_shr:1 row_mask:0xf bank_mask:0xf bound_ctrl:0\n\t" \
+	"v_add_f32_dpp v121, v121, %[di] wave_shr:1 row_mask:0xf bank_mask:0xf bound_ctrl:0\n\t" \
+	"s_nop 0\n\t" \
+	"v_sub_f32_dpp v120, v120, %[di] wave_shr:1 row_mask:0xf bank_mask:0xf bound_ctrl:0\n\t" \
+	"v_add_f32_dpp v121, v121, %[dr] wave_shr:1 row_mask:0xf bank_mask:0xf bound_ctrl:0\n\t" \
+	"s_nop 0\n\t" \
+	"v_sub_f32_dpp v120, v120, %[dr] wave_shr:1 row_mask:0xf bank_mask:0xf bound_ctrl:0\n\t" \
+	"v_sub_f32_dpp v121, v121, %[di] wave_shr:1 row_mask:0xf bank_mask:0xf bound_ctrl:0\n\t" \
+	"s_nop 0\n\t" \
+	"v_add_f32_dpp v120, v120, %[di] wave_shr:1 row_mask:0xf bank_mask:0xf bound_ctrl:0\n\t" \
+	"v_sub_f32_dpp v121, v121, %[dr] wave_shr:1 row_mask:0xf bank_mask:0xf bound_ctrl:0\n\t" \
+	"s_branch .Lnb_corrr_join\n\t" \
+	".Lnb_corrr_v2:\n\t" \
+	"v_add_f32_e32 v120, 0, %[dr]\n\t" \
+	"v_add_f32_e32 v121, 0, %[di]\n\t" \
+	"s_nop 0\n\t" \
+	"v_sub_f32_dpp v120, v120, %[di] wave_shr:1 row_mask:0xf bank_mask:0xf bound_ctrl:0\n\t" \
+	"v_add_f32_dpp v121, v121, %[dr] wave_shr:1 row_mask:0xf bank_mask:0xf bound_ctrl:0\n\t" \
+	"s_nop 0\n\t" \
+	"v_add_f32_dpp v120, v120, %[dr] wave_shr:1 row_mask:0xf bank_mask:0xf bound_ctrl:0\n\t" \
+	"v_add_f32_dpp v121, v121, %[di] wave_shr:1 row_mask:0xf bank_mask:0xf bound_ctrl:0\n\t" \
+	"s_nop 0\n\t" \
+	"v_add_f32_dpp v120, v120, %[di] wave_shr:1 row_mask:0xf bank_mask:0xf bound_ctrl:0\n\t" \
+	"v_sub_f32_dpp v121, v121, %[dr] wave_shr:1 row_mask:0xf bank_mask:0xf bound_ctrl:0\n\t" \
+	"s_nop 0\n\t" \
+	"v_add_f32_dpp v120, v120, %[dr] wave_shr:1 row_mask:0xf bank_mask:0xf bound_ctrl:0\n\t" \
+	"v_add_f32_dpp v121, v121, %[di] wave_shr:1 row_mask:0xf bank_mask:0xf bound_ctrl:0\n\t" \
+	"s_nop 0\n\t" \
+	"v_sub_f32_dpp v120, v120, %[di] wave_shr:1 row_mask:0xf bank_mask:0xf bound_ctrl:0\n\t" \
+	"v_add_f32_dpp v121, v121, %[dr] wave_shr:1 row_mask:0xf bank_mask:0xf bound_ctrl:0\n\t" \
+	"s_nop 0\n\t" \
+	"v_add_f32_dpp v120, v120, %[dr] wave_shr:1 row_mask:0xf bank_mask:0xf bound_ctrl:0\n\t" \
+	"v_add_f32_dpp v121, v121, %[di] wave_shr:1 row_mask:0xf bank_mask:0xf bound_ctrl:0\n\t" \
+	"s_nop 0\n\t" \
+	"v_add_f32_dpp v120, v120, %[di] wave_shr:1 row_mask:0xf bank_mask:0xf bound_ctrl:0\n\t" \
+	"v_sub_f32_dpp v121, v121, %[dr] wave_shr:1 row_mask:0xf bank_mask:0xf bound_ctrl:0\n\t" \
+	"s_nop 0\n\t" \
+	"v_add_f32_dpp v120, v120, %[dr] wave_shr:1 row_mask:0xf bank_mask:0xf bound_ctrl:0\n\t" \
+	"v_add_f32_dpp v121, v121, %[di] wave_shr:1 row_mask:0xf bank_mask:0xf bound_ctrl:0\n\t" \
+	"s_nop 0\n\t" \
+	"v_sub_f32_dpp v120, v120, %[di] wave_shr:1 row_mask:0xf bank_mask:0xf bound_ctrl:0\n\t" \
+	"v_add_f32_dpp v121, v121, %[dr] wave_shr:1 row_mask:0xf bank_mask:0xf bound_ctrl:0\n\t" \
+	"s_nop 0\n\t" \
+	"v_sub_f32_dpp v120, v120, %[dr] wave_shr:1 row_mask:0xf bank_mask:0xf bound_ctrl:0\n\t" \
+	"v_sub_f32_dpp v121, v121, %[di] wave_shr:1 row_mask:0xf bank_mask:0xf bound_ctrl:0\n\t" \
+	"s_nop 0\n\t" \
+	"v_sub_f32_dpp v120, v120, %[di] wave_shr:1 row_mask:0xf bank_mask:0xf bound_ctrl:0\n\t" \
+	"v_add_f32_dpp v121, v121, %[dr] wave_shr:1 row_mask:0xf bank_mask:0xf bound_ctrl:0\n\t" \
+	"s_nop 0\n\t" \
+	"v_sub_f32_dpp v120, v120, %[dr] wave_shr:1 row_mask:0xf bank_mask:0xf bound_ctrl:0\n\t" \
+	"v_sub_f32_dpp v121, v121, %[di] wave_shr:1 row_mask:0xf bank_mask:0xf bound_ctrl:0\n\t" \
+	"s_nop 0\n\t" \
+	"v_add_f32_dpp v120, v120, %[di] wave_shr:1 row_mask:0xf bank_mask:0xf bound_ctrl:0\n\t" \
+	"v_sub_f32_dpp v121, v121, %[dr] wave_shr:1 row_mask:0xf bank_mask:0xf bound_ctrl:0\n\t" \
+	"s_nop 0\n\t" \
+	"v_sub_f32_dpp v120, v120, %[dr] wave_shr:1 row_mask:0xf bank_mask:0xf bound_ctrl:0\n\t" \
+	"v_sub_f32_dpp v121, v121, %[di] wave_shr:1 row_mask:0xf bank_mask:0xf bound_ctrl:0\n\t" \
+	"s_nop 0\n\t" \
+	"v_sub_f32_dpp v120, v120, %[di] wave_shr:1 row_mask:0xf bank_mask:0xf bound_ctrl:0\n\t" \
+	"v_add_f32_dpp v121, v121, %[dr] wave_shr:1 row_mask:0xf bank_mask:0xf bound_ctrl:0\n\t" \
+	"s_branch .Lnb_corrr_join\n\t" \
+	".Lnb_corrr_v3:\n\t" \
+	"v_sub_f32_e32 v120, 0, %[dr]\n\t" \
+	"v_sub_f32_e32 v121, 0, %[di]\n\t" \
+	"s_nop 0\n\t" \
+	"v_sub_f32_dpp v120, v120, %[di] wave_shr:1 row_mask:0xf bank_mask:0xf bound_ctrl:0\n\t" \
+	"v_add_f32_dpp v121, v121, %[dr] wave_shr:1 row_mask:0xf bank_mask:0xf bound_ctrl:0\n\t" \
+	"s_nop 0\n\t" \
+	"v_add_f32_dpp v120, v120, %[dr] wave_shr:1 row_mask:0xf bank_mask:0xf bound_ctrl:0\n\t" \
+	"v_add_f32_dpp v121, v121, %[di] wave_shr:1 row_mask:0xf bank_mask:0xf bound_ctrl:0\n\t" \
+	"s_nop 0\n\t" \
+	"v_add_f32_dpp v120, v120, %[di] wave_shr:1 row_mask:0xf bank_mask:0xf bound_ctrl:0\n\t" \
+	"v_sub_f32_dpp v121, v121, %[dr] wave_shr:1 row_mask:0xf bank_mask:0xf bound_ctrl:0\n\t" \
+	"s_nop 0\n\t" \
+	"v_add_f32_dpp v120, v120, %[dr] wave_shr:1 row_mask:0xf bank_mask:0xf bound_ctrl:0\n\t" \
+	"v_add_f32_dpp v121, v121, %[di] wave_shr:1 row_mask:0xf bank_mask:0xf bound_ctrl:0\n\t" \
+	"s_nop 0\n\t" \
+	"v_sub_f32_dpp v120, v120, %[di] wave_shr:1 row_mask:0xf bank_mask:0xf bound_ctrl:0\n\t" \
+	"v_add_f32_dpp v121, v121, %[dr] wave_shr:1 row_mask:0xf bank_mask:0xf bound_ctrl:0\n\t" \
+	"s_nop 0\n\t" \
+	"v_add_f32_dpp v120, v120, %[dr] wave_shr:1 row_mask:0xf bank_mask:0xf bound_ctrl:0\n\t" \
+	"v_add_f32_dpp v121, v121, %[di] wave_shr:1 row_mask:0xf bank_mask:0xf bound_ctrl:0\n\t" \
+	"s_nop 0\n\t" \
+	"v_sub_f32_dpp v120, v120, %[di] wave_shr:1 row_mask:0xf bank_mask:0xf bound_ctrl:0\n\t" \
+	"v_add_f32_dpp v121, v121, %[dr] wave_shr:1 row_mask:0xf bank_mask:0xf bound_ctrl:0\n\t" \
+	"s_nop 0\n\t" \
+	"v_sub_f32_dpp v120, v120, %[dr] wave_shr:1 row_mask:0xf bank_mask:0xf bound_ctrl:0\n\t" \
+	"v_sub_f32_dpp v121, v121, %[di] wave_shr:1 row_mask:0xf bank_mask:0xf bound_ctrl:0\n\t" \
+	"s_nop 0\n\t" \
+	"v_add_f32_dpp v120, v120, %[di] wave_shr:1 row_mask:0xf bank_mask:0xf bound_ctrl:0\n\t" \
+	"v_sub_f32_dpp v121, v121, %[dr] wave_shr:1 row_mask:0xf bank_mask:0xf bound_ctrl:0\n\t" \
+	"s_nop 0\n\t" \
+	"v_sub_f32_dpp v120, v120, %[dr] wave_shr:1 row_mask:0xf bank_mask:0xf bound_ctrl:0\n\t" \
+	"v_sub_f32_dpp v121, v121, %[di] wave_shr:1 row_mask:0xf bank_mask:0xf bound_ctrl:0\n\t" \
+	"s_nop 0\n\t" \
+	"v_sub_f32_dpp v120, v120, %[di] wave_shr:1 row_mask:0xf bank_mask:0xf bound_ctrl:0\n\t" \
+	"v_add_f32_dpp v121, v121, %[dr] wave_shr:1 row_mask:0xf bank_mask:0xf bound_ctrl:0\n\t" \
+	"s_nop 0\n\t" \
+	"v_sub_f32_dpp v120, v120, %[dr] wave_shr:1 row_mask:0xf bank_mask:0xf bound_ctrl:0\n\t" \
+	"v_sub_f32_dpp v121, v121, %[di] wave_shr:1 row_mask:0xf bank_mask:0xf bound_ctrl:0\n\t" \
+	"s_nop 0\n\t" \
+	"v_add_f32_dpp v120, v120, %[di] wave_shr:1 row_mask:0xf bank_mask:0xf bound_ctrl:0\n\t" \
+	"v_sub_f32_dpp v121, v121, %[dr] wave_shr:1 row_mask:0xf bank_mask:0xf bound_ctrl:0\n\t" \
+	"s_nop 0\n\t" \
+	"v_sub_f32_dpp v120, v120, %[dr] wave_shr:1 row_mask:0xf bank_mask:0xf bound_ctrl:0\n\t" \
+	"v_sub_f32_dpp v121, v121, %[di] wave_shr:1 row_mask:0xf bank_mask:0xf bound_ctrl:0\n\t" \
+	"s_nop 0\n\t" \
+	"v_sub_f32_dpp v120, v120, %[di] wave_shr:1 row_mask:0xf bank_mask:0xf bound_ctrl:0\n\t" \
+	"v_add_f32_dpp v121, v121, %[dr] wave_shr:1 row_mask:0xf bank_mask:0xf bound_ctrl:0\n\t" \
+	"s_branch .Lnb_corrr_join\n\t" \
+	".Lnb_corrr_v4:\n\t" \
+	"v_add_f32_e32 v120, 0, %[dr]\n\t" \
+	"v_add_f32_e32 v121, 0, %[di]\n\t" \
+	"s_nop 0\n\t" \
+	"v_sub_f32_dpp v120, v120, %[di] wave_shr:1 row_mask:0xf bank_mask:0xf bound_ctrl:0\n\t" \
+	"v_add_f32_dpp v121, v121, %[dr] wave_shr:1 row_mask:0xf bank_mask:0xf bound_ctrl:0\n\t" \
+	"s_nop 0\n\t" \
+	"v_sub_f32_dpp v120, v120, %[dr] wave_shr:1 row_mask:0xf bank_mask:0xf bound_ctrl:0\n\t" \
+	"v_sub_f32_dpp v121, v121, %[di] wave_shr:1 row_mask:0xf bank_mask:0xf bound_ctrl:0\n\t" \
+	"s_nop 0\n\t" \
+	"v_add_f32_dpp v120, v120, %[di] wave_shr:1 row_mask:0xf bank_mask:0xf bound_ctrl:0\n\t" \
+	"v_sub_f32_dpp v121, v121, %[dr] wave_shr:1 row_mask:0xf bank_mask:0xf bound_ctrl:0\n\t" \
+	"s_nop 0\n\t" \
+	"v_sub_f32_dpp v120, v120, %[dr] wave_shr:1 row_mask:0xf bank_mask:0xf bound_ctrl:0\n\t" \
+	"v_sub_f32_dpp v121, v121, %[di] wave_shr:1 row_mask:0xf bank_mask:0xf bound_ctrl:0\n\t" \
+	"s_nop 0\n\t" \
+	"v_sub_f32_dpp v120, v120, %[di] wave_shr:1 row_mask:0xf bank_mask:0xf bound_ctrl:0\n\t" \
+	"v_add_f32_dpp v121, v121, %[dr] wave_shr:1 row_mask:0xf bank_mask:0xf bound_ctrl:0\n\t" \
+	"s_nop 0\n\t" \
+	"v_sub_f32_dpp v120, v120, %[dr] wave_shr:1 row_mask:0xf bank_mask:0xf bound_ctrl:0\n\t" \
+	"v_sub_f32_dpp v121, v121, %[di] wave_shr:1 row_mask:0xf bank_mask:0xf bound_ctrl:0\n\t" \
+	"s_nop 0\n\t" \
+	"v_sub_f32_dpp v120, v120, %[di] wave_shr:1 row_mask:0xf bank_mask:0xf bound_ctrl:0\n\t" \
+	"v_add_f32_dpp v121, v121, %[dr] wave_shr:1 row_mask:0xf bank_mask:0xf bound_ctrl:0\n\t" \
+	"s_nop 0\n\t" \
+	"v_sub_f32_dpp v120, v120, %[dr] wave_shr:1 row_mask:0xf bank_mask:0xf bound_ctrl:0\n\t" \
+	"v_sub_f32_dpp v121, v121, %[di] wave_shr:1 row_mask:0xf bank_mask:0xf bound_ctrl:0\n\t" \
+	"s_nop 0\n\t" \
+	"v_add_f32_dpp v120, v120, %[di] wave_shr:1 row_mask:0xf bank_mask:0xf bound_ctrl:0\n\t" \
+	"v_sub_f32_dpp v121, v121, %[dr] wave_shr:1 row_mask:0xf bank_mask:0xf bound_ctrl:0\n\t" \
+	"s_nop 0\n\t" \
+	"v_sub_f32_dpp v120, v120, %[dr] wave_shr:1 row_mask:0xf bank_mask:0xf bound_ctrl:0\n\t" \
+	"v_sub_f32_dpp v121, v121, %[di] wave_shr:1 row_mask:0xf bank_mask:0xf bound_ctrl:0\n\t" \
+	"s_nop 0\n\t" \
+	"v_sub_f32_dpp v120, v120, %[di] wave_shr:1 row_mask:0xf bank_mask:0xf bound_ctrl:0\n\t" \
+	"v_add_f32_dpp v121, v121, %[dr] wave_shr:1 row_mask:0xf bank_mask:0xf bound_ctrl:0\n\t" \
+	"s_nop 0\n\t" \
+	"v_add_f32_dpp v120, v120, %[dr] wave_shr:1 row_mask:0xf bank_mask:0xf bound_ctrl:0\n\t" \
+	"v_add_f32_dpp v121, v121, %[di] wave_shr:1 row_mask:0xf bank_mask:0xf bound_ctrl:0\n\t" \
+	"s_nop 0\n\t" \
+	"v_add_f32_dpp v120, v120, %[di] wave_shr:1 row_mask:0xf bank_mask:0xf bound_ctrl:0\n\t" \
+	"v_sub_f32_dpp v121, v121, %[dr] wave_shr:1 row_mask:0xf bank_mask:0xf bound_ctrl:0\n\t" \
+	"s_nop 0\n\t" \
+	"v_add_f32_dpp v120, v120, %[dr] wave_shr:1 row_mask:0xf bank_mask:0xf bound_ctrl:0\n\t" \
+	"v_add_f32_dpp v121, v121, %[di] wave_shr:1 row_mask:0xf bank_mask:0xf bound_ctrl:0\n\t" \
+	"s_nop 0\n\t" \
+	"v_add_f32_dpp v120, v120, %[di] wave_shr:1 row_mask:0xf bank_mask:0xf bound_ctrl:0\n\t" \
+	"v_sub_f32_dpp v121, v121, %[dr] wave_shr:1 row_mask:0xf bank_mask:0xf bound_ctrl:0\n\t" \
+	"s_branch .Lnb_corrr_join\n\t" \
+	".Lnb_corrr_v5:\n\t" \
+	"v_sub_f32_e32 v120, 0, %[dr]\n\t" \
+	"v_sub_f32_e32 v121, 0, %[di]\n\t" \
+	"s_nop 0\n\t" \
+	"v_sub_f32_dpp v120, v120, %[di] wave_shr:1 row_mask:0xf bank_mask:0xf bound_ctrl:0\n\t" \
+	"v_add_f32_dpp v121, v121, %[dr] wave_shr:1 row_mask:0xf bank_mask:0xf bound_ctrl:0\n\t" \
+	"s_nop 0\n\t" \
+	"v_sub_f32_dpp v120, v120, %[dr] wave_shr:1 row_mask:0xf bank_mask:0xf bound_ctrl:0\n\t" \
+	"v_sub_f32_dpp v121, v121, %[di] wave_shr:1 row_mask:0xf bank_mask:0xf bound_ctrl:0\n\t" \
+	"s_nop 0\n\t" \
+	"v_add_f32_dpp v120, v120, %[di] wave_shr:1 row_mask:0xf bank_mask:0xf bound_ctrl:0\n\t" \
+	"v_sub_f32_dpp v121, v121, %[dr] wave_shr:1 row_mask:0xf bank_mask:0xf bound_ctrl:0\n\t" \
+	"s_nop 0\n\t" \
+	"v_add_f32_dpp v120, v120, %[dr] wave_shr:1 row_mask:0xf bank_mask:0xf bound_ctrl:0\n\t" \
+	"v_add_f32_dpp v121, v121, %[di] wave_shr:1 row_mask:0xf bank_mask:0xf bound_ctrl:0\n\t" \
+	"s_nop 0\n\t" \
+	"v_sub_f32_dpp v120, v120, %[di] wave_shr:1 row_mask:0xf bank_mask:0xf bound_ctrl:0\n\t" \
+	"v_add_f32_dpp v121, v121, %[dr] wave_shr:1 row_mask:0xf bank_mask:0xf bound_ctrl:0\n\t" \
+	"s_nop 0\n\t" \
+	"v_add_f32_dpp v120, v120, %[dr] wave_shr:1 row_mask:0xf bank_mask:0xf bound_ctrl:0\n\t" \
+	"v_add_f32_dpp v121, v121, %[di] wave_shr:1 row_mask:0xf bank_mask:0xf bound_ctrl:0\n\t" \
+	"s_nop 0\n\t" \
+	"v_sub_f32_dpp v120, v120, %[di] wave_shr:1 row_mask:0xf bank_mask:0xf bound_ctrl:0\n\t" \
+	"v_add_f32_dpp v121, v121, %[dr] wave_shr:1 row_mask:0xf bank_mask:0xf bound_ctrl:0\n\t" \
+	"s_nop 0\n\t" \
+	"v_add_f32_dpp v120, v120, %[dr] wave_shr:1 row_mask:0xf bank_mask:0xf bound_ctrl:0\n\t" \
+	"v_add_f32_dpp v121, v121, %[di] wave_shr:1 row_mask:0xf bank_mask:0xf bound_ctrl:0\n\t" \
+	"s_nop 0\n\t" \
+	"v_add_f32_dpp v120, v120, %[di] wave_shr:1 row_mask:0xf bank_mask:0xf bound_ctrl:0\n\t" \
+	"v_sub_f32_dpp v121, v121, %[dr] wave_shr:1 row_mask:0xf bank_mask:0xf bound_ctrl:0\n\t" \
+	"s_nop 0\n\t" \
+	"v_sub_f32_dpp v120, v120, %[dr] wave_shr:1 row_mask:0xf bank_mask:0xf bound_ctrl:0\n\t" \
+	"v_sub_f32_dpp v121, v121, %[di] wave_shr:1 row_mask:0xf bank_mask:0xf bound_ctrl:0\n\t" \
+	"s_nop 0\n\t" \
+	"v_sub_f32_dpp v120, v120, %[di] wave_shr:1 row_mask:0xf bank_mask:0xf bound_ctrl:0\n\t" \
+	"v_add_f32_dpp v121, v121, %[dr] wave_shr:1 row_mask:0xf bank_mask:0xf bound_ctrl:0\n\t" \
+	"s_nop 0\n\t" \
+	"v_sub_f32_dpp v120, v120, %[dr] wave_shr:1 row_mask:0xf bank_mask:0xf bound_ctrl:0\n\t" \
+	"v_sub_f32_dpp v121, v121, %[di] wave_shr:1 row_mask:0xf bank_mask:0xf bound_ctrl:0\n\t" \
+	"s_nop 0\n\t" \
+	"v_add_f32_dpp v120, v120, %[di] wave_shr:1 row_mask:0xf bank_mask:0xf bound_ctrl:0\n\t" \
+	"v_sub_f32_dpp v121, v121, %[dr] wave_shr:1 row_mask:0xf bank_mask:0xf bound_ctrl:0\n\t" \
+	"s_nop 0\n\t" \
+	"v_sub_f32_dpp v120, v120, %[dr] wave_shr:1 row_mask:0xf bank_mask:0xf bound_ctrl:0\n\t" \
+	"v_sub_f32_dpp v121, v121, %[di] wave_shr:1 row_mask:0xf bank_mask:0xf bound_ctrl:0\n\t" \
+	"s_nop 0\n\t" \
+	"v_add_f32_dpp v120, v120, %[di] wave_shr:1 row_mask:0xf bank_mask:0xf bound_ctrl:0\n\t" \
+	"v_sub_f32_dpp v121, v121, %[dr] wave_shr:1 row_mask:0xf bank_mask:0xf bound_ctrl:0\n\t" \
+	"s_branch .Lnb_corrr_join\n\t" \
+	".Lnb_corrr_v6:\n\t" \
+	"v_sub_f32_e32 v120, 0, %[dr]\n\t" \
+	"v_sub_f32_e32 v121, 0, %[di]\n\t" \
+	"s_nop 0\n\t" \
+	"v_sub_f32_dpp v120, v120, %[di] wave_shr:1 row_mask:0xf bank_mask:0xf bound_ctrl:0\n\t" \
+	"v_add_f32_dpp v121, v121, %[dr] wave_shr:1 row_mask:0xf bank_mask:0xf bound_ctrl:0\n\t" \
+	"s_nop 0\n\t" \
+	"v_add_f32_dpp v120, v120, %[dr] wave_shr:1 row_mask:0xf bank_mask:0xf bound_ctrl:0\n\t" \
+	"v_add_f32_dpp v121, v121, %[di] wave_shr:1 row_mask:0xf bank_mask:0xf bound_ctrl:0\n\t" \
+	"s_nop 0\n\t" \
+	"v_add_f32_dpp v120, v120, %[di] wave_shr:1 row_mask:0xf bank_mask:0xf bound_ctrl:0\n\t" \
+	"v_sub_f32_dpp v121, v121, %[dr] wave_shr:1 row_mask:0xf bank_mask:0xf bound_ctrl:0\n\t" \
+	"s_nop 0\n\t" \
+	"v_sub_f32_dpp v120, v120, %[dr] wave_shr:1 row_mask:0xf bank_mask:0xf bound_ctrl:0\n\t" \
+	"v_sub_f32_dpp v121, v121, %[di] wave_shr:1 row_mask:0xf bank_mask:0xf bound_ctrl:0\n\t" \
+	"s_nop 0\n\t" \
+	"v_add_f32_dpp v120, v120, %[di] wave_shr:1 row_mask:0xf bank_mask:0xf bound_ctrl:0\n\t" \
+	"v_sub_f32_dpp v121, v121, %[dr] wave_shr:1 row_mask:0xf bank_mask:0xf bound_ctrl:0\n\t" \
+	"s_nop 0\n\t" \
+	"v_add_f32_dpp v120, v120, %[dr] wave_shr:1 row_mask:0xf bank_mask:0xf bound_ctrl:0\n\t" \
+	"v_add_f32_dpp v121, v121, %[di] wave_shr:1 row_mask:0xf bank_mask:0xf bound_ctrl:0\n\t" \
+	"s_nop 0\n\t" \
+	"v_add_f32_dpp v120, v120, %[di] wave_shr:1 row_mask:0xf bank_mask:0xf bound_ctrl:0\n\t" \
+	"v_sub_f32_dpp v121, v121, %[dr] wave_shr:1 row_mask:0xf bank_mask:0xf bound_ctrl:0\n\t" \
+	"s_nop 0\n\t" \
+	"v_add_f32_dpp v120, v120, %[dr] wave_shr:1 row_mask:0xf bank_mask:0xf bound_ctrl:0\n\t" \
+	"v_add_f32_dpp v121, v121, %[di] wave_shr:1 row_mask:0xf bank_mask:0xf bound_ctrl:0\n\t" \
+	"s_nop 0\n\t" \
+	"v_add_f32_dpp v120, v120, %[di] wave_shr:1 row_mask:0xf bank_mask:0xf bound_ctrl:0\n\t" \
+	"v_sub_f32_dpp v121, v121, %[dr] wave_shr:1 row_mask:0xf bank_mask:0xf bound_ctrl:0\n\t" \
+	"s_nop 0\n\t" \
+	"v_sub_f32_dpp v120, v120, %[dr] wave_shr:1 row_mask:0xf bank_mask:0xf bound_ctrl:0\n\t" \
+	"v_sub_f32_dpp v121, v121, %[di] wave_shr:1 row_mask:0xf bank_mask:0xf bound_ctrl:0\n\t" \
+	"s_nop 0\n\t" \
+	"v_add_f32_dpp v120, v120, %[di] wave_shr:1 row_mask:0xf bank_mask:0xf bound_ctrl:0\n\t" \
+	"v_sub_f32_dpp v121, v121, %[dr] wave_shr:1 row_mask:0xf bank_mask:0xf bound_ctrl:0\n\t" \
+	"s_nop 0\n\t" \
+	"v_add_f32_dpp v120, v120, %[dr] wave_shr:1 row_mask:0xf bank_mask:0xf bound_ctrl:0\n\t" \
+	"v_add_f32_dpp v121, v121, %[di] wave_shr:1 row_mask:0xf bank_mask:0xf bound_ctrl:0\n\t" \
+	"s_nop 0\n\t" \
+	"v_sub_f32_dpp v120, v120, %[di] wave_shr:1 row_mask:0xf bank_mask:0xf bound_ctrl:0\n\t" \
+	"v_add_f32_dpp v121, v121, %[dr] wave_shr:1 row_mask:0xf bank_mask:0xf bound_ctrl:0\n\t" \
+	"s_nop 0\n\t" \
+	"v_sub_f32_dpp v120, v120, %[dr] wave_shr:1 row_mask:0xf bank_mask:0xf bound_ctrl:0\n\t" \
+	"v_sub_f32_dpp v121, v121, %[di] wave_shr:1 row_mask:0xf bank_mask:0xf bound_ctrl:0\n\t" \
+	"s_nop 0\n\t" \
+	"v_sub_f32_dpp v120, v120, %[di] wave_shr:1 row_mask:0xf bank_mask:0xf bound_ctrl:0\n\t" \
+	"v_add_f32_dpp v121, v121, %[dr] wave_shr:1 row_mask:0xf bank_mask:0xf bound_ctrl:0\n\t" \
+	"s_branch .Lnb_corrr_join\n\t" \
+	".Lnb_corrr_v7:\n\t" \
+	"v_sub_f32_e32 v120, 0, %[dr]\n\t" \
+	"v_sub_f32_e32 v121, 0, %[di]\n\t" \
+	"s_nop 0\n\t" \
+	"v_sub_f32_dpp v120, v120, %[di] wave_shr:1 row_mask:0xf bank_mask:0xf bound_ctrl:0\n\t" \
+	"v_add_f32_dpp v121, v121, %[dr] wave_shr:1 row_mask:0xf bank_mask:0xf bound_ctrl:0\n\t" \
+	"s_nop 0\n\t" \
+	"v_add_f32_dpp v120, v120, %[dr] wave_shr:1 row_mask:0xf bank_mask:0xf bound_ctrl:0\n\t" \
+	"v_add_f32_dpp v121, v121, %[di] wave_shr:1 row_mask:0xf bank_mask:0xf bound_ctrl:0\n\t" \
+	"s_nop 0\n\t" \
+	"v_sub_f32_dpp v120, v120, %[di] wave_shr:1 row_mask:0xf bank_mask:0xf bound_ctrl:0\n\t" \
+	"v_add_f32_dpp v121, v121, %[dr] wave_shr:1 row_mask:0xf bank_mask:0xf bound_ctrl:0\n\t" \
+	"s_nop 0\n\t" \
+	"v_add_f32_dpp v120, v120, %[dr] wave_shr:1 row_mask:0xf bank_mask:0xf bound_ctrl:0\n\t" \
+	"v_add_f32_dpp v121, v121, %[di] wave_shr:1 row_mask:0xf bank_mask:0xf bound_ctrl:0\n\t" \
+	"s_nop 0\n\t" \
+	"v_add_f32_dpp v120, v120, %[di] wave_shr:1 row_mask:0xf bank_mask:0xf bound_ctrl:0\n\t" \
+	"v_sub_f32_dpp v121, v121, %[dr] wave_shr:1 row_mask:0xf bank_mask:0xf bound_ctrl:0\n\t" \
+	"s_nop 0\n\t" \
+	"v_add_f32_dpp v120, v120, %[dr] wave_shr:1 row_mask:0xf bank_mask:0xf bound_ctrl:0\n\t" \
+	"v_add_f32_dpp v121, v121, %[di] wave_shr:1 row_mask:0xf bank_mask:0xf bound_ctrl:0\n\t" \
+	"s_nop 0\n\t" \
+	"v_sub_f32_dpp v120, v120, %[di] wave_shr:1 row_mask:0xf bank_mask:0xf bound_ctrl:0\n\t" \
+	"v_add_f32_dpp v121, v121, %[dr] wave_shr:1 row_mask:0xf bank_mask:0xf bound_ctrl:0\n\t" \
+	"s_nop 0\n\t" \
+	"v_add_f32_dpp v120, v120, %[dr] wave_shr:1 row_mask:0xf bank_mask:0xf bound_ctrl:0\n\t" \
+	"v_add_f32_dpp v121, v121, %[di] wave_shr:1 row_mask:0xf bank_mask:0xf bound_ctrl:0\n\t" \
+	"s_nop 0\n\t" \
+	"v_sub_f32_dpp v120, v120, %[di] wave_shr:1 row_mask:0xf bank_mask:0xf bound_ctrl:0\n\t" \
+	"v_add_f32_dpp v121, v121, %[dr] wave_shr:1 row_mask:0xf bank_mask:0xf bound_ctrl:0\n\t" \
+	"s_nop 0\n\t" \
+	"v_sub_f32_dpp v120, v120, %[dr] wave_shr:1 row_mask:0xf bank_mask:0xf bound_ctrl:0\n\t" \
+	"v_sub_f32_dpp v121, v121, %[di] wave_shr:1 row_mask:0xf bank_mask:0xf bound_ctrl:0\n\t" \
+	"s_nop 0\n\t" \
+	"v_add_f32_dpp v120, v120, %[di] wave_shr:1 row_mask:0xf bank_mask:0xf bound_ctrl:0\n\t" \
+	"v_sub_f32_dpp v121, v121, %[dr] wave_shr:1 row_mask:0xf bank_mask:0xf bound_ctrl:0\n\t" \
+	"s_nop 0\n\t" \
+	"v_sub_f32_dpp v120, v120, %[dr] wave_shr:1 row_mask:0xf bank_mask:0xf bound_ctrl:0\n\t" \
+	"v_sub_f32_dpp v121, v121, %[di] wave_shr:1 row_mask:0xf bank_mask:0xf bound_ctrl:0\n\t" \
+	"s_nop 0\n\t" \
+	"v_sub_f32_dpp v120, v120, %[di] wave_shr:1 row_mask:0xf bank_mask:0xf bound_ctrl:0\n\t" \
+	"v_add_f32_dpp v121, v121, %[dr] wave_shr:1 row_mask:0xf bank_mask:0xf bound_ctrl:0\n\t" \
+	"s_nop 0\n\t" \
+	"v_sub_f32_dpp v120, v120, %[dr] wave_shr:1 row_mask:0xf bank_mask:0xf bound_ctrl:0\n\t" \
+	"v_sub_f32_dpp v121, v121, %[di] wave_shr:1 row_mask:0xf bank_mask:0xf bound_ctrl:0\n\t" \
+	"s_nop 0\n\t" \
+	"v_add_f32_dpp v120, v120, %[di] wave_shr:1 row_mask:0xf bank_mask:0xf bound_ctrl:0\n\t" \
+	"v_sub_f32_dpp v121, v121, %[dr] wave_shr:1 row_mask:0xf bank_mask:0xf bound_ctrl:0\n\t" \
+	"s_branch .Lnb_corrr_join\n\t" \
+	".Lnb_corrr_join:\n\t" \
+	"s_bfm_b64 exec, 12, 0\n\t" \
+	"ds_write_b64 v64, v[122:123]\n\t" \
+	"s_bfm_b64 exec, %[len], 19\n\t" \
+	"ds_write_b64 %[vczm], v[120:121]\n\t" \
+	"v_pk_mul_f32 v[124:125], v[120:121], v[120:121]\n\t" \
+	"s_nop 0\n\t" \
+	"v_add_f32_e32 %[nrm], v125, v124\n\t" \
+	"s_mov_b64 exec, -1\n\t" \
+	"s_waitcnt lgkmcnt(0)\n\t" \
+	"s_branch .Lnb_corr_end\n\t" \
+	".Lnb_corrr_mul:\n\t" \
+	"s_bfm_b64 exec, %[len], 19\n\t" \
+	"ds_read_b64 v[88:89], %[vdm] offset:0\n\t" \
+	"ds_read_b64 v[90:91], %[vdm] offset:8\n\t" \
+	"ds_read_b64 v[92:93], %[vdm] offset:16\n\t" \
+	"ds_read_b64 v[94:95], %[vdm] offset:24\n\t" \
+	"ds_read_b64 v[96:97], %[vdm] offset:32\n\t" \
+	"ds_read_b64 v[98:99], %[vdm] offset:40\n\t" \
+	"ds_read_b64 v[100:101], %[vdm] offset:48\n\t" \
+	"ds_read_b64 v[102:103], %[vdm] offset:56\n\t" \
+	"ds_read_b64 v[104:105], %[vdm] offset:64\n\t" \
+	"ds_read_b64 v[106:107], %[vdm] offset:72\n\t" \
+	"ds_read_b64 v[108:109], %[vdm] offset:80\n\t" \
+	"ds_read_b64 v[110:111], %[vdm] offset:88\n\t" \
+	"ds_read_b64 v[112:113], %[vdm] offset:96\n\t" \
+	"ds_read_b64 v[114:115], %[vdm] offset:104\n\t" \
+	"ds_read_b64 v[116:117], %[vdm] offset:112\n\t" \
+	"ds_read_b64 v[118:119], %[vdm] offset:120\n\t" \
+	"s_lshl_b32 s90, %[tsc], 7\n\t" \
+	"v_mov_b32_e32 v64, s90\n\t" \
+	"ds_read_b128 v[66:69], v64 offset:32848\n\t" \
+	"ds_read_b128 v[70:73], v64 offset:32864\n\t" \
+	"ds_read_b128 v[74:77], v64 offset:32880\n\t" \
+	"ds_read_b128 v[78:81], v64 offset:32896\n\t" \
+	"s_waitcnt lgkmcnt(0)\n\t" \
+	"v_pk_mul_f32 v[82:83], v[88:89], v[66:67] op_sel:[0,0] op_sel_hi:[0,1]\n\t" \
+	"v_pk_mul_f32 v[84:85], v[88:89], v[66:67] op_sel:[1,1] op_sel_hi:[1,0]\n\t" \
+	"s_nop 0\n\t" \
+	"v_pk_add_f32 v[86:87], v[82:83], v[84:85] neg_lo:[0,1] neg_hi:[0,0]\n\t" \
+	"s_nop 0\n\t" \
+	"v_pk_add_f32 v[120:121], v[120:121], v[86:87]\n\t" \
+	"v_pk_mul_f32 v[82:83], v[90:91], v[68:69] op_sel:[0,0] op_sel_hi:[0,1]\n\t" \
+	"v_pk_mul_f32 v[84:85], v[90:91], v[68:69] op_sel:[1,1] op_sel_hi:[1,0]\n\t" \
+	"s_nop 0\n\t" \
+	"v_pk_add_f32 v[86:87], v[82:83], v[84:85] neg_lo:[0,1] neg_hi:[0,0]\n\t" \
+	"s_nop 0\n\t" \
+	"v_pk_add_f32 v[120:121], v[120:121], v[86:87]\n\t" \
+	"v_pk_mul_f32 v[82:83], v[92:93], v[70:71] op_sel:[0,0] op_sel_hi:[0,1]\n\t" \
+	"v_pk_mul_f32 v[84:85], v[92:93], v[70:71] op_sel:[1,1] op_sel_hi:[1,0]\n\t" \
+	"s_nop 0\n\t" \
+	"v_pk_add_f32 v[86:87], v[82:83], v[84:85] neg_lo:[0,1] neg_hi:[0,0]\n\t" \
+	"s_nop 0\n\t" \
+	"v_pk_add_f32 v[120:121], v[120:121], v[86:87]\n\t" \
+	"v_pk_mul_f32 v[82:83], v[94:95], v[72:73] op_sel:[0,0] op_sel_hi:[0,1]\n\t" \
+	"v_pk_mul_f32 v[84:85], v[94:95], v[72:73] op_sel:[1,1] op_sel_hi:[1,0]\n\t" \
+	"s_nop 0\n\t" \
+	"v_pk_add_f32 v[86:87], v[82:83], v[84:85] neg_lo:[0,1] neg_hi:[0,0]\n\t" \
+	"s_nop 0\n\t" \
+	"v_pk_add_f32 v[120:121], v[120:121], v[86:87]\n\t" \
+	"v_pk_mul_f32 v[82:83], v[96:97], v[74:75] op_sel:[0,0] op_sel_hi:[0,1]\n\t" \
+	"v_pk_mul_f32 v[84:85], v[96:97], v[74:75] op_sel:[1,1] op_sel_hi:[1,0]\n\t" \
+	"s_nop 0\n\t" \
+	"v_pk_add_f32 v[86:87], v[82:83], v[84:85] neg_lo:[0,1] neg_hi:[0,0]\n\t" \
+	"s_nop 0\n\t" \
+	"v_pk_add_f32 v[120:121], v[120:121], v[86:87]\n\t" \
+	"v_pk_mul_f32 v[82:83], v[98:99], v[76:77] op_sel:[0,0] op_sel_hi:[0,1]\n\t" \
+	"v_pk_mul_f32 v[84:85], v[98:99], v[76:77] op_sel:[1,1] op_sel_hi:[1,0]\n\t" \
+	"s_nop 0\n\t" \
+	"v_pk_add_f32 v[86:87], v[82:83], v[84:85] neg_lo:[0,1] neg_hi:[0,0]\n\t" \
+	"s_nop 0\n\t" \
+	"v_pk_add_f32 v[120:121], v[120:121], v[86:87]\n\t" \
+	"v_pk_mul_f32 v[82:83], v[100:101], v[78:79] op_sel:[0,0] op_sel_hi:[0,1]\n\t" \
+	"v_pk_mul_f32 v[84:85], v[100:101], v[78:79] op_sel:[1,1] op_sel_hi:[1,0]\n\t" \
+	"s_nop 0\n\t" \
+	"v_pk_add_f32 v[86:87], v[82:83], v[84:85] neg_lo:[0,1] neg_hi:[0,0]\n\t" \
+	"s_nop 0\n\t" \
+	"v_pk_add_f32 v[120:121], v[120:121], v[86:87]\n\t" \
+	"v_pk_mul_f32 v[82:83], v[102:103], v[80:81] op_sel:[0,0] op_sel_hi:[0,1]\n\t" \
+	"v_pk_mul_f32 v[84:85], v[102:103], v[80:81] op_sel:[1,1] op_sel_hi:[1,0]\n\t" \
+	"s_nop 0\n\t" \
+	"v_pk_add_f32 v[86:87], v[82:83], v[84:85] neg_lo:[0,1] neg_hi:[0,0]\n\t" \
+	"s_nop 0\n\t" \
+	"v_pk_add_f32 v[120:121], v[120:121], v[86:87]\n\t" \
+	"ds_read_b128 v[66:69], v64 offset:32912\n\t" \
+	"ds_read_b128 v[70:73], v64 offset:32928\n\t" \
+	"ds_read_b128 v[74:77], v64 offset:32944\n\t" \
+	"ds_read_b128 v[78:81], v64 offset:32960\n\t" \
+	"s_waitcnt lgkmcnt(0)\n\t" \
+	"v_pk_mul_f32 v[82:83], v[104:105], v[66:67] op_sel:[0,0] op_sel_hi:[0,1]\n\t" \
+	"v_pk_mul_f32 v[84:85], v[104:105], v[66:67] op_sel:[1,1] op_sel_hi:[1,0]\n\t" \
+	"s_nop 0\n\t" \
+	"v_pk_add_f32 v[86:87], v[82:83], v[84:85] neg_lo:[0,1] neg_hi:[0,0]\n\t" \
+	"s_nop 0\n\t" \
+	"v_pk_add_f32 v[120:121], v[120:121], v[86:87]\n\t" \
+	"v_pk_mul_f32 v[82:83], v[106:107], v[68:69] op_sel:[0,0] op_sel_hi:[0,1]\n\t" \
+	"v_pk_mul_f32 v[84:85], v[106:107], v[68:69] op_sel:[1,1] op_sel_hi:[1,0]\n\t" \
+	"s_nop 0\n\t" \
+	"v_pk_add_f32 v[86:87], v[82:83], v[84:85] neg_lo:[0,1] neg_hi:[0,0]\n\t" \
+	"s_nop 0\n\t" \
+	"v_pk_add_f32 v[120:121], v[120:121], v[86:87]\n\t" \
+	"v_pk_mul_f32 v[82:83], v[108:109], v[70:71] op_sel:[0,0] op_sel_hi:[0,1]\n\t" \
+	"v_pk_mul_f32 v[84:85], v[108:109], v[70:71] op_sel:[1,1] op_sel_hi:[1,0]\n\t" \
+	"s_nop 0\n\t" \
+	"v_pk_add_f32 v[86:87], v[82:83], v[84:85] neg_lo:[0,1] neg_hi:[0,0]\n\t" \
+	"s_nop 0\n\t" \
+	"v_pk_add_f32 v[120:121], v[120:121], v[86:87]\n\t" \
+	"v_pk_mul_f32 v[82:83], v[110:111], v[72:73] op_sel:[0,0] op_sel_hi:[0,1]\n\t" \
+	"v_pk_mul_f32 v[84:85], v[110:111], v[72:73] op_sel:[1,1] op_sel_hi:[1,0]\n\t" \
+	"s_nop 0\n\t" \
+	"v_pk_add_f32 v[86:87], v[82:83], v[84:85] neg_lo:[0,1] neg_hi:[0,0]\n\t" \
+	"s_nop 0\n\t" \
+	"v_pk_add_f32 v[120:121], v[120:121], v[86:87]\n\t" \
+	"v_pk_mul_f32 v[82:83], v[112:113], v[74:75] op_sel:[0,0] op_sel_hi:[0,1]\n\t" \
+	"v_pk_mul_f32 v[84:85], v[112:113], v[74:75] op_sel:[1,1] op_sel_hi:[1,0]\n\t" \
+	"s_nop 0\n\t" \
+	"v_pk_add_f32 v[86:87], v[82:83], v[84:85] neg_lo:[0,1] neg_hi:[0,0]\n\t" \
+	"s_nop 0\n\t" \
+	"v_pk_add_f32 v[120:121], v[120:121], v[86:87]\n\t" \
+	"v_pk_mul_f32 v[82:83], v[114:115], v[76:77] op_sel:[0,0] op_sel_hi:[0,1]\n\t" \
+	"v_pk_mul_f32 v[84:85], v[114:115], v[76:77] op_sel:[1,1] op_sel_hi:[1,0]\n\t" \
+	"s_nop 0\n\t" \
+	"v_pk_add_f32 v[86:87], v[82:83], v[84:85] neg_lo:[0,1] neg_hi:[0,0]\n\t" \
+	"s_nop 0\n\t" \
+	"v_pk_add_f32 v[120:121], v[120:121], v[86:87]\n\t" \
+	"v_pk_mul_f32 v[82:83], v[116:117], v[78:79] op_sel:[0,0] op_sel_hi:[0,1]\n\t" \
+	"v_pk_mul_f32 v[84:85], v[116:117], v[78:79] op_sel:[1,1] op_sel_hi:[1,0]\n\t" \
+	"s_nop 0\n\t" \
+	"v_pk_add_f32 v[86:87], v[82:83], v[84:85] neg_lo:[0,1] neg_hi:[0,0]\n\t" \
+	"s_nop 0\n\t" \
+	"v_pk_add_f32 v[120:121], v[120:121], v[86:87]\n\t" \
+	"v_pk_mul_f32 v[82:83], v[118:119], v[80:81] op_sel:[0,0] op_sel_hi:[0,1]\n\t" \
+	"v_pk_mul_f32 v[84:85], v[118:119], v[80:81] op_sel:[1,1] op_sel_hi:[1,0]\n\t" \
+	"s_nop 0\n\t" \
+	"v_pk_add_f32 v[86:87], v[82:83], v[84:85] neg_lo:[0,1] neg_hi:[0,0]\n\t" \
+	"s_nop 0\n\t" \
+	"v_pk_add_f32 v[120:121], v[120:121], v[86:87]\n\t" \
+	"s_branch .Lnb_corrr_join\n\t" \
+	".Lnb_corr_wide:\n\t" \
 	"v_mov_b64_e32 v[120:121], 0\n\t" \
 	"s_bfm_b64 exec, %[len], 0\n\t" \
 	"ds_read_b64 v[88:89], %[vd] offset:0\n\t" \
@@ -85,16 +702,16 @@
 	"ds_read_b64 v[116:117], %[vd] offset:112\n\t" \
 	"ds_read_b64 v[118:119], %[vd] offset:120\n\t" \
 	"s_cmp_lg_u64 %[bad], 0\n\t" \
-	"s_cbranch_scc1 .Lnb_corr_mul\n\t" \
+	"s_cbranch_scc1 .Lnb_corrw_mul\n\t" \
 	"s_getpc_b64 s[88:89]\n\t" \
-	".Lnb_corr_pc:\n\t" \
-	"s_mul_i32 s90, %[tsc], .Lnb_corr_v1-.Lnb_corr_v0\n\t" \
+	".Lnb_corrw_pc:\n\t" \
+	"s_mul_i32 s90, %[tsc], .Lnb_corrw_v1-.Lnb_corrw_v0\n\t" \
 	"s_add_u32 s88, s88, s90\n\t" \
 	"s_addc_u32 s89, s89, 0\n\t" \
-	"s_add_u32 s88, s88, .Lnb_corr_v0-.Lnb_corr_pc\n\t" \
+	"s_add_u32 s88, s88, .Lnb_corrw_v0-.Lnb_corrw_pc\n\t" \
 	"s_addc_u32 s89, s89, 0\n\t" \
 	"s_setpc_b64 s[88:89]\n\t" \
-	".Lnb_corr_v0:\n\t" \
+	".Lnb_corrw_v0:\n\t" \
 	"s_waitcnt lgkmcnt(15)\n\t" \
 	"v_pk_add_f32 v[120:121], v[120:121], v[88:89] neg_lo:[0,1] neg_hi:[0,1]\n\t" \
 	"s_waitcnt lgkmcnt(14)\n\t" \
@@ -127,8 +744,8 @@
 	"v_pk_add_f32 v[120:121], v[120:121], v[116:117] neg_lo:[0,1] neg_hi:[0,1]\n\t" \
 	"s_waitcnt lgkmcnt(0)\n\t" \
 	"v_pk_add_f32 v[120:121], v[120:121], v[118:119] op_sel:[0,1] op_sel_hi:[1,0] neg_lo:[0,1] neg_hi:[0,0]\n\t" \
-	"s_branch .Lnb_corr_join\n\t" \
-	".Lnb_corr_v1:\n\t" \
+	"s_branch .Lnb_corrw_join\n\t" \
+	".Lnb_corrw_v1:\n\t" \
 	"s_waitcnt lgkmcnt(15)\n\t" \
 	"v_pk_add_f32 v[120:121], v[120:121], v[88:89] neg_lo:[0,1] neg_hi:[0,1]\n\t" \
 	"s_waitcnt lgkmcnt(14)\n\t" \
@@ -161,8 +778,8 @@
 	"v_pk_add_f32 v[120:121], v[120:121], v[116:117] neg_lo:[0,1] neg_hi:[0,1]\n\t" \
 	"s_waitcnt lgkmcnt(0)\n\t" \
 	"v_pk_add_f32 v[120:121], v[120:121], v[118:119] op_sel:[0,1] op_sel_hi:[1,0] neg_lo:[0,0] neg_hi:[0,1]\n\t" \
-	"s_branch .Lnb_corr_join\n\t" \
-	".Lnb_corr_v2:\n\t" \
+	"s_branch .Lnb_corrw_join\n\t" \
+	".Lnb_corrw_v2:\n\t" \
 	"s_waitcnt lgkmcnt(15)\n\t" \
 	"v_pk_add_f32 v[120:121], v[120:121], v[88:89]\n\t" \
 	"s_waitcnt lgkmcnt(14)\n\t" \
@@ -195,8 +812,8 @@
 	"v_pk_add_f32 v[120:121], v[120:121], v[116:117] neg_lo:[0,1] neg_hi:[0,1]\n\t" \
 	"s_waitcnt lgkmcnt(0)\n\t" \
 	"v_pk_add_f32 v[120:121], v[120:121], v[118:119] op_sel:[0,1] op_sel_hi:[1,0] neg_lo:[0,1] neg_hi:[0,0]\n\t" \
-	"s_branch .Lnb_corr_join\n\t" \
-	".Lnb_corr_v3:\n\t" \
+	"s_branch .Lnb_corrw_join\n\t" \
+	".Lnb_corrw_v3:\n\t" \
 	"s_waitcnt lgkmcnt(15)\n\t" \
 	"v_pk_add_f32 v[120:121], v[120:121], v[88:89] neg_lo:[0,1] neg_hi:[0,1]\n\t" \
 	"s_waitcnt lgkmcnt(14)\n\t" \
@@ -229,8 +846,8 @@
 	"v_pk_add_f32 v[120:121], v[120:121], v[116:117] neg_lo:[0,1] neg_hi:[0,1]\n\t" \
 	"s_waitcnt lgkmcnt(0)\n\t" \
 	"v_pk_add_f32 v[120:121], v[120:121], v[118:119] op_sel:[0,1] op_sel_hi:[1,0] neg_lo:[0,1] neg_hi:[0,0]\n\t" \
-	"s_branch .Lnb_corr_join\n\t" \
-	".Lnb_corr_v4:\n\t" \
+	"s_branch .Lnb_corrw_join\n\t" \
+	".Lnb_corrw_v4:\n\t" \
 	"s_waitcnt lgkmcnt(15)\n\t" \
 	"v_pk_add_f32 v[120:121], v[120:121], v[88:89]\n\t" \
 	"s_waitcnt lgkmcnt(14)\n\t" \
@@ -263,8 +880,8 @@
 	"v_pk_add_f32 v[120:121], v[120:121], v[116:117]\n\t" \
 	"s_waitcnt lgkmcnt(0)\n\t" \
 	"v_pk_add_f32 v[120:121], v[120:121], v[118:119] op_sel:[0,1] op_sel_hi:[1,0] neg_lo:[0,0] neg_hi:[0,1]\n\t" \
-	"s_branch .Lnb_corr_join\n\t" \
-	".Lnb_corr_v5:\n\t" \
+	"s_branch .Lnb_corrw_join\n\t" \
+	".Lnb_corrw_v5:\n\t" \
 	"s_waitcnt lgkmcnt(15)\n\t" \
 	"v_pk_add_f32 v[120:121], v[120:121], v[88:89] neg_lo:[0,1] neg_hi:[0,1]\n\t" \
 	"s_waitcnt lgkmcnt(14)\n\t" \
@@ -297,8 +914,8 @@
 	"v_pk_add_f32 v[120:121], v[120:121], v[116:117] neg_lo:[0,1] neg_hi:[0,1]\n\t" \
 	"s_waitcnt lgkmcnt(0)\n\t" \
 	"v_pk_add_f32 v[120:121], v[120:121], v[118:119] op_sel:[0,1] op_sel_hi:[1,0] neg_lo:[0,0] neg_hi:[0,1]\n\t" \
-	"s_branch .Lnb_corr_join\n\t" \
-	".Lnb_corr_v6:\n\t" \
+	"s_branch .Lnb_corrw_join\n\t" \
+	".Lnb_corrw_v6:\n\t" \
 	"s_waitcnt lgkmcnt(15)\n\t" \
 	"v_pk_add_f32 v[120:121], v[120:121], v[88:89] neg_lo:[0,1] neg_hi:[0,1]\n\t" \
 	"s_waitcnt lgkmcnt(14)\n\t" \
@@ -331,8 +948,8 @@
 	"v_pk_add_f32 v[120:121], v[120:121], v[116:117] neg_lo:[0,1] neg_hi:[0,1]\n\t" \
 	"s_waitcnt lgkmcnt(0)\n\t" \
 	"v_pk_add_f32 v[120:121], v[120:121], v[118:119] op_sel:[0,1] op_sel_hi:[1,0] neg_lo:[0,1] neg_hi:[0,0]\n\t" \
-	"s_branch .Lnb_corr_join\n\t" \
-	".Lnb_corr_v7:\n\t" \
+	"s_branch .Lnb_corrw_join\n\t" \
+	".Lnb_corrw_v7:\n\t" \
 	"s_waitcnt lgkmcnt(15)\n\t" \
 	"v_pk_add_f32 v[120:121], v[120:121], v[88:89] neg_lo:[0,1] neg_hi:[0,1]\n\t" \
 	"s_waitcnt lgkmcnt(14)\n\t" \
@@ -365,8 +982,8 @@
 	"v_pk_add_f32 v[120:121], v[120:121], v[116:117] neg_lo:[0,1] neg_hi:[0,1]\n\t" \
 	"s_waitcnt lgkmcnt(0)\n\t" \
 	"v_pk_add_f32 v[120:121], v[120:121], v[118:119] op_sel:[0,1] op_sel_hi:[1,0] neg_lo:[0,0] neg_hi:[0,1]\n\t" \
-	"s_branch .Lnb_corr_join\n\t" \
-	".Lnb_corr_join:\n\t" \
+	"s_branch .Lnb_corrw_join\n\t" \
+	".Lnb_corrw_join:\n\t" \
 	"s_add_u32 s90, %[len], 12\n\t" \
 	"s_bfm_b64 exec, s90, 0\n\t" \
 	"ds_write_b64 %[vcz], v[120:121]\n\t" \
@@ -375,7 +992,7 @@
 	"s_waitcnt lgkmcnt(0)\n\t" \
 	"v_add_f32_e32 %[nrm], v123, v122\n\t" \
 	"s_branch .Lnb_corr_end\n\t" \
-	".Lnb_corr_mul:\n\t" \
+	".Lnb_corrw_mul:\n\t" \
 	"s_lshl_b32 s90, %[tsc], 7\n\t" \
 	"v_mov_b32_e32 v64, s90\n\t" \
 	"ds_read_b128 v[66:69], v64 offset:32848\n\t" \
@@ -484,7 +1101,7 @@
 	"v_pk_add_f32 v[86:87], v[82:83], v[84:85] neg_lo:[0,1] neg_hi:[0,0]\n\t" \
 	"s_nop 0\n\t" \
 	"v_pk_add_f32 v[120:121], v[120:121], v[86:87]\n\t" \
-	"s_branch .Lnb_corr_join\n\t" \
+	"s_branch .Lnb_corrw_join\n\t" \
 	".Lnb_corr_end:\n\t"
 #define NB_ASM_DETA \
 	"s_mov_b32 %[st], 0\n\t" \
```

Result: faster. 1066, median of 6 (+1.7%).
